# yuz1wan/video_distillation

Hardware: AMD Instinct MI355X
Metric: distillation steps/sec (DM, miniUCF101 IPC=1) (higher is better)
Workload: dtype f16

## Files before the change

### include/vd_hip.h

```cpp
#ifndef VD_HIP_H
#define VD_HIP_H

#include <stdint.h>

#ifdef __cplusplus
extern "C" {
#endif

#define VD_ABI_VERSION 5

#define VD_PREC_BF16   0
#define VD_PREC_F16    1
#define VD_PREC_BF16X3 2
#define VD_PREC_F16X3  3
#define VD_F16X3_WSHIFT 8
#define VD_PREC_F16C8  4

#define VD_EPI_POOL_CL   0
#define VD_EPI_POOL_FEAT 1
#define VD_EPI_ROWS      2
#define VD_EPI_POS_FEAT  3

typedef struct VdConvParams {
    const void* src;
    int64_t src_plane_stride4;
    int64_t src_clip_stride4;
    int64_t src_chunk_stride4;
    const void* wpk;
    int64_t w_plane_stride;
    int64_t w_box_stride;
    const float* bias;
    void* dst;
    int64_t dst_plane_stride;
    uint8_t* argmax;
    const int32_t* col_off;
    const float* out_scale;
    const int32_t* type_desc;
    const int32_t* tables;
    const int32_t* boxes;
    const int32_t* gather;
    int64_t gather_stride;
    const void* zero_slot;
    int32_t nbox, nclips, ncl;
    int32_t CC, S, NT, MW, MTW;
    int32_t epi, pool_t, relu, n_out, n_stride;
    int64_t out_clip_stride;
    int32_t out_chunk_stride, out_t_stride;
    int32_t lds_plane_bytes;
    int32_t prec;
    int32_t dbg;
    int32_t ntypes;
    int32_t tab_ofs[3];
    int32_t atomic;
    int32_t select;
    int32_t src_split_cc;
    int64_t src_split_off4;
    int32_t NTW;
    const int64_t* clip_index;
    int32_t mt_valid;
    int32_t persist;
    uint64_t* stamps;
    int32_t w_set_clips;
    int32_t replica_stride;
    int32_t emit_lo;
    int32_t src_planes, src_rows;
    int32_t pair_flip;
    uint32_t* range_stats;
} VdConvParams;

int vd_abi_version(void);

int vd_conv_mfma(const VdConvParams* params, void* stream);
int vd_conv_mfma_multi(const VdConvParams* const* params, int n, void* stream);

int vd_conv0_breg(const VdConvParams* p, void* stream);

int vd_pack_weights(const float* w, const int32_t* widx, int64_t n, void* out_hi, void* out_lo,
                    int prec, void* stream);

#define VD_PACK_MAX 24
typedef struct {
    const float* w; const int32_t* widx; int64_t n; void* out_hi; void* out_lo; int32_t prec; int32_t first_block;
} VdPackSeg;
typedef struct { int32_t nseg; int32_t reserved; VdPackSeg seg[VD_PACK_MAX]; } VdPackBatch;
int vd_pack_weights_multi(const VdPackBatch* batch, void* stream);
int vd_pack_weights_c8(const float* w, int64_t w_elems, const int32_t* widx, int CC, int S, int NT, void* out_hi, void* out_c8,
                       float* scales6, void* stream);
int vd_pack_weights_dither(const float* w, const int32_t* widx, int64_t n, int groups, void* out, int prec, void* stream);

int vd_round_operand(const float* w, int64_t n, int prec, float* out, void* stream);

int vd_pix2rows(const float* x, const int64_t* clip_index, int64_t nclips, int T, int H, int W,
                void* out_hi, void* out_lo, int prec, void* stream);

int vd_unpool_relu_bwd(const float* g, const uint8_t* argmax, int64_t nclips, int C, int To, int Ho, int Wo,
                       int pool_t, int T, int OH, int OW, int g_layout, void* out_hi, void* out_lo,
                       int prec, const float* scale, void* stream);

int vd_absmax_scale(const float* g, int64_t n, float target, float* out, void* stream);

int vd_dm_loss(const float* feat_real, const float* feat_syn, int nclass, int nreal, int nsyn, int dim,
               float* loss_per_class, float* g_syn, void* stream);

int vd_group_sum(const float* x, int groups, int per, int dim, float scale, float* out, void* stream);

int vd_sgd_momentum(float* x, float* buf, const float* g, int64_t n, float lr, float momentum, int first,
                    void* stream);

int vd_hallucinator_fwd(const float* stat, const float* dyn, const int64_t* sidx, const int64_t* didx,
                        const float* w, const float* b, int n, int T, int H, int W, float* out, void* stream);

int vd_hallucinator_bwd(const float* g_out, const float* stat, const float* dyn, const int64_t* sidx,
                        const int64_t* didx, const float* w, int n, int T, int H, int W,
                        float* g_dyn, float* g_stat, float* g_w, float* g_b, void* stream);

int vd_match_rows_fwd(const float* gr, const float* gs, int64_t rows, int len, float* acc, void* stream);
int vd_match_rows_bwd(const float* gr, const float* gs, int64_t rows, int len, int mode, const float* acc,
                      const float* gout, float* g_gs, void* stream);

#define VD_MATCH_MAX_SEG 16
typedef struct VdMatchSeg {
    const float* gr;
    const float* gs;
    float* g;
    int64_t rows;
    int32_t len;
    int32_t reserved;
} VdMatchSeg;
typedef struct VdMatchBatch {
    int32_t nseg;
    int32_t reserved;
    VdMatchSeg seg[VD_MATCH_MAX_SEG];
} VdMatchBatch;
int vd_match_rows_fwd_multi(const VdMatchBatch* batch, float* acc, void* stream);
int vd_match_rows_bwd_multi(const VdMatchBatch* batch, int mode, const float* acc, const float* gout, void* stream);

int vd_clip_minor_cl(const void* src, int64_t src_plane_slots, int planes, int64_t nclips, int C, int64_t npos,
                     void* dst, int64_t dst_plane_slots, void* stream);
int vd_clip_minor_pix(const float* x, int64_t nclips, int T, int H, int W, void* dst_hi, void* dst_lo, int prec,
                      void* stream);
int vd_pack_dy(const void* dy, int64_t dy_plane_slots, int planes, int64_t nclips, int N, int T, int OH, int OW,
               int nt, int noh, int now, void* dst, int64_t dst_plane_elems, void* stream);
int vd_unpool_relu_bwd_packed(const float* g, const uint8_t* argmax, int64_t nclips, int C, int To, int Ho, int Wo,
                              int pool_t, int T, int OH, int OW, int g_layout, int nt, int noh, int now,
                              void* dst_hi, void* dst_lo, int prec, const float* scale, void* stream);

int vd_bias_grad_pooled(const float* g, const uint8_t* argmax, int64_t nclips, int C, int64_t npos, int g_layout, float* db,
                        void* stream);
int64_t vd_bias_grad_pooled_scratch_floats(int64_t nclips, int C, int64_t npos);
int vd_bias_grad_pooled_ordered(const float* g, const uint8_t* argmax, int64_t nclips, int C, int64_t npos, int g_layout,
                                float* scratch, float* db, void* stream);
int vd_bias_grad(const void* dy, int64_t dy_plane_slots, int planes, int64_t nclips, int N, int64_t npos, int prec,
                 const float* scale_inv, float* db, void* stream);

int vd_head_fwd(const float* feats, const float* w, const float* b, int64_t nclips, int C, int To, int Ho, int Wo,
                int kt, int kh, int kw, int K, float* out, void* stream);

int vd_standardize(const float* x, int64_t n, double* scratch2, float* out, void* stream);
int vd_head_train_fwd(const float* feats, const float* mask, const float* w, const float* b, int64_t nclips, int C, int To,
                      int Ho, int Wo, int kt, int kh, int kw, int K, float* dropped, float* logits, int32_t* amax_t, void* stream);
int vd_ce_loss(const float* logits, const int64_t* labels, int B, int K, float* loss_per_clip, float* dlogits, void* stream);
int vd_head_train_bwd(const float* dlogits, const int32_t* amax_t, const float* dropped, const float* mask, const float* w,
                      int64_t nclips, int C, int To, int Ho, int Wo, int kt, int kh, int kw, int K, float* g_w, float* g_b,
                      float* g_feats, void* stream);
int vd_standardize_ordered(const float* x, int64_t n, double* scratch, float* out, void* stream);
int vd_head_train_bwd_ordered(const float* dlogits, const int32_t* amax_t, const float* dropped, const float* mask, const float* w,
                              int64_t nclips, int C, int To, int Ho, int Wo, int kt, int kh, int kw, int K, float* g_w, float* g_b,
                              float* g_feats, void* stream);
int vd_set_deterministic(int on);
int vd_get_deterministic(void);
int vd_resplit_slots(const void* src_hi, const void* src_lo, int64_t n_elems, int src_prec, void* dst_hi, void* dst_lo,
                     int dst_prec, void* stream);
int vd_split_scaled(const float* src, int64_t n_elems, const float* scale, void* dst_hi, void* dst_lo, int prec, void* stream);
int vd_scale_combine(const float* a, const float* b, int mode, float* out, void* stream);
const char* vd_sources_hash(void);

int vd_head_second_order(const float* logits, const float* dlogits, const int32_t* amax_t, const float* dropped,
                         const float* mask, const float* w, const float* v_w, const float* v_b, const float* gbar_feats,
                         int64_t nclips, int C, int To, int Ho, int Wo, int kt, int kh, int kw, int K, float* abar_feats,
                         float* wbar, float* bbar, float* dlogbar_out, void* stream);
int vd_program_build(int layer, int frames, int height, int width, int prec, int batch_hint, void** blob, int64_t* nbytes);
int vd_program_build_dgrad(int layer, int parity_class, int frames, int height, int width, int batch_hint, void** blob,
                           int64_t* nbytes);
int vd_program_build_wgrad(int layer, int frames, int height, int width, int nclips, int planes, void** blob, int64_t* nbytes,
                           int* block3, int* replicas);
void vd_blob_free(void* blob);

typedef struct VdEmbed VdEmbed;
int vd_embed_create(int frames, int height, int width, int prec, int batch_hint, VdEmbed** out);
int vd_embed_create_ex(int frames, int height, int width, int prec, int prec_bwd, int batch_hint, VdEmbed** out);
int64_t vd_embed_argmax_bytes(const VdEmbed* e, int64_t nclips);
int64_t vd_embed_backward_workspace_bytes(const VdEmbed* e, int64_t nclips);
int vd_embed_forward_keep(VdEmbed* e, const float* clips, const int64_t* clip_index, int64_t nclips, void* workspace,
                          int64_t workspace_bytes, float* features, uint8_t* argmax, void* stream);
int vd_embed_backward(VdEmbed* e, const float* g_features, const uint8_t* argmax, int64_t nclips, void* workspace,
                      int64_t workspace_bytes, float* g_clips, void* stream);
int64_t vd_embed_num_features(const VdEmbed* e);
int64_t vd_embed_workspace_bytes(const VdEmbed* e, int64_t nclips);
int vd_embed_set_weights(VdEmbed* e, const float* w0, const float* b0, const float* w1, const float* b1, const float* w2,
                         const float* b2, void* stream);
int vd_embed_forward(VdEmbed* e, const float* clips, const int64_t* clip_index, int64_t nclips, void* workspace,
                     int64_t workspace_bytes, float* features, void* stream);
void vd_embed_free(VdEmbed* e);

int vd_mfma_peak(int blocks, int iters, int shape, float* out, void* stream);
int vd_sgd_momentum_wd(float* x, float* buf, const float* g, int64_t n, float lr, float momentum, float wd, int first,
                       void* stream);

int vd_replica_sum(float* rep, int replicas, int rows, int cols, float* out, void* stream);

int vd_frames_normalize(const void* src_u8, float* dst, int64_t nframes, int height, int width, const float* mean3,
                        const float* std3, void* stream);

int vd_clips_sample(const void* frames_u8, int64_t store_frames, int src_h, int src_w, const int64_t* frame_row,
                    const int32_t* crop_yx, const uint8_t* flip, int64_t nclips, int T, int out_h, int out_w, float* dst,
                    const float* mean3, const float* std3, void* stream);

typedef struct VdProgram VdProgram;
int vd_program_load(const void* blob, int64_t nbytes, int prec, VdProgram** out);
int vd_program_pack_weights(VdProgram* prog, const float* w, void* stream);
int vd_program_run(VdProgram* prog, const void* src, int64_t src_plane_slots, const float* bias, void* dst,
                   int64_t dst_plane_stride, uint8_t* argmax, const int64_t* clip_index, int nclips, void* stream);
int vd_program_run_scaled(VdProgram* prog, const void* src, int64_t src_plane_slots, const float* bias, void* dst,
                          int64_t dst_plane_stride, uint8_t* argmax, const int64_t* clip_index, int nclips,
                          const float* out_scale, void* stream);
int vd_program_run_wgrad(VdProgram* prog, const void* x_clip_minor, int64_t x_plane_slots, const void* packed_dy,
                         int64_t packed_plane_elems, float* copies, int64_t copy_elems, int cin, const float* out_scale,
                         void* stream);
int64_t vd_program_info(const VdProgram* prog, int what);
void vd_program_free(VdProgram* prog);

typedef struct VdTrain VdTrain;
int vd_train_create(int frames, int height, int width, int num_classes, int prec, int prec_bwd, int64_t nclips, VdTrain** out);
int64_t vd_train_workspace_bytes(const VdTrain* t);
int vd_train_step(VdTrain* t, float* const* params, float* const* momentum, const float* clips, const int64_t* labels,
                  const float* dropout_mask, float lr, float momentum_coef, float weight_decay, int first, void* workspace,
                  int64_t workspace_bytes, float* loss_per_clip, float* logits, void* stream);
void vd_train_free(VdTrain* t);

typedef struct VdComm VdComm;
typedef struct { char internal[128]; } VdCommId;
int vd_comm_unique_id(VdCommId* id);
int vd_comm_create(const VdCommId* id, int nranks, int rank, VdComm** out);
int vd_comm_size(const VdComm* c);
int vd_comm_version(int* version);
int vd_comm_rank(const VdComm* c);
int vd_comm_allreduce_f32(VdComm* c, const float* send, float* recv, int64_t n, void* stream);
int vd_comm_allgather_f32(VdComm* c, const float* send, float* recv, int64_t n_per_rank, void* stream);
void vd_comm_free(VdComm* c);

#define VD_CORESET_HERDING   0
#define VD_CORESET_KCENTER   1
#define VD_CORESET_MAX_COUNT 4096
#define VD_CORESET_MAX_DIM   8192
int64_t vd_coreset_workspace_bytes(int nclass, int max_count);
int vd_coreset_select(const float* feats, int dim, const int64_t* offsets, const int32_t* counts, int nclass, int max_count,
                      int ipc, int method, int64_t* out_idx, void* workspace, int64_t workspace_bytes, void* stream);

#ifdef __cplusplus
}
// ... 3 lines not shown
```

### video_distillation_amd/csrc/aux_kernels.hip

```cpp
#include <hip/hip_runtime.h>
#include <stdint.h>
#include <stdlib.h>

#include "../../include/vd_hip.h"
#include "frame_norm.h"

typedef __bf16 bf16_t;

__device__ __forceinline__ void split16p(int prec, float v, uint16_t& hi, uint16_t& lo) {
    if (prec == VD_PREC_BF16 || prec == VD_PREC_BF16X3) {
        __bf16 h = (__bf16)v;
        __bf16 l = (__bf16)(v - (float)h);
        hi = __builtin_bit_cast(uint16_t, h);
        lo = __builtin_bit_cast(uint16_t, l);
    } else {
        _Float16 h = (_Float16)v;
        _Float16 l = (_Float16)(v - (float)h);
        hi = __builtin_bit_cast(uint16_t, h);
        lo = __builtin_bit_cast(uint16_t, l);
    }
}

__device__ __forceinline__ float wave_sum(float v) {
#pragma unroll
// ... 358 lines not shown
                           reinterpret_cast<hipStream_t>(stream), g, argmax, nwin, C, To, Ho, Wo, pool_t, T, OH, OW,
                           (uint4*)out_hi, (uint4*)out_lo, prec, scale);
        return (int)hipGetLastError();
    }
    hipLaunchKernelGGL(unpool_relu_bwd_kernel, dim3((unsigned)((nslots + bs - 1) / bs)), dim3(bs), 0,
                       reinterpret_cast<hipStream_t>(stream), g, argmax, nslots, C, To, Ho, Wo, pool_t, T, OH, OW,
                       g_layout, (uint4*)out_hi, (uint4*)out_lo, prec, scale);
    return (int)hipGetLastError();
}

__global__ void absmax_kernel(const float* __restrict__ g, int64_t n, unsigned int* __restrict__ bits) {
    __shared__ float red[16];
    float m = 0.f;
    for (int64_t i = (int64_t)blockIdx.x * blockDim.x + threadIdx.x; i < n; i += (int64_t)gridDim.x * blockDim.x)
        m = fmaxf(m, fabsf(g[i]));
#pragma unroll
    for (int o = 32; o > 0; o >>= 1) m = fmaxf(m, __shfl_xor(m, o, 64));
    const int lane = threadIdx.x & 63, w = threadIdx.x >> 6;
    if (lane == 0) red[w] = m;
    __syncthreads();
    if (threadIdx.x == 0) {
        for (int i = 1; i < (int)(blockDim.x >> 6); ++i) m = fmaxf(m, red[i]);
        atomicMax(bits, __float_as_uint(m));
    }
}

__device__ __forceinline__ void float_decompose(unsigned int bits, int& e, unsigned int& mant) {
    e = (int)(bits >> 23);
    mant = bits & 0x7fffffu;
    if (e == 0) {
        const int sh = __clz(mant) - 8;
        mant <<= sh;
        e = 1 - sh;
    } else {
        mant |= 0x800000u;
    }
    e -= 127;
}

__global__ void scale_from_absmax_kernel(const unsigned int* __restrict__ bits, float target, float* __restrict__ out) {
    const unsigned int mb = bits[0], tb = __float_as_uint(target);
    int k = 0;
    if (mb != 0u && mb < 0x7f800000u && tb != 0u && tb < 0x7f800000u) {
        int em, et;
        unsigned int mm, mt;
        float_decompose(mb, em, mm);
        float_decompose(tb, et, mt);
        k = et - em - (mt > mm ? 0 : 1);
        k = k < -126 ? -126 : (k > 126 ? 126 : k);
    }
    out[0] = __uint_as_float((unsigned int)(127 + k) << 23);
    out[1] = __uint_as_float((unsigned int)(127 - k) << 23);
}

extern "C" int vd_absmax_scale(const float* g, int64_t n, float target, float* out, void* stream) {
    hipStream_t st = reinterpret_cast<hipStream_t>(stream);
    unsigned int* bits = reinterpret_cast<unsigned int*>(out + 2);
    hipError_t e = hipMemsetAsync(bits, 0, sizeof(unsigned int), st);
    if (e != hipSuccess) return (int)e;
    if (n > 0) {
        int64_t blocks = (n + 256 * 8 - 1) / (256 * 8);
        if (blocks > 1024) blocks = 1024;
        hipLaunchKernelGGL(absmax_kernel, dim3((unsigned)blocks), dim3(256), 0, st, g, n, bits);
    }
    hipLaunchKernelGGL(scale_from_absmax_kernel, dim3(1), dim3(1), 0, st, bits, target, out);
    return (int)hipGetLastError();
}

__global__ __launch_bounds__(1024) void dm_loss_kernel(const float* __restrict__ fr, const float* __restrict__ fs,
                                                        int nreal, int nsyn, int dim, float* __restrict__ loss,
                                                        float* __restrict__ gsyn) {
    __shared__ float red[16];
    const int c = blockIdx.x;
    const float* r = fr + (int64_t)c * nreal * dim;
    const float* s = fs + (int64_t)c * nsyn * dim;
    const float inv_r = 1.f / (float)nreal, inv_s = 1.f / (float)nsyn;
    float part = 0.f;
    for (int d = threadIdx.x; d < dim; d += blockDim.x) {
        float m[8] = {0.f, 0.f, 0.f, 0.f, 0.f, 0.f, 0.f, 0.f};
        int b = 0;
        for (; b + 8 <= nreal; b += 8) {
#pragma unroll
            for (int k = 0; k < 8; ++k) m[k] += r[(int64_t)(b + k) * dim + d];
        }
        for (; b < nreal; ++b) m[0] += r[(int64_t)b * dim + d];
        const float mr = ((m[0] + m[1]) + (m[2] + m[3])) + ((m[4] + m[5]) + (m[6] + m[7]));
        float ms = 0.f;
        for (int k = 0; k < nsyn; ++k) ms += s[(int64_t)k * dim + d];
        const float diff = mr * inv_r - ms * inv_s;
        part += diff * diff;
        if (gsyn != nullptr) {
            const float gv = -2.f * diff * inv_s;
            for (int k = 0; k < nsyn; ++k) gsyn[((int64_t)c * nsyn + k) * dim + d] = gv;
        }
    }
    const float tot = block_sum(part, red);
    if (threadIdx.x == 0) loss[c] = tot;
}

extern "C" int vd_dm_loss(const float* feat_real, const float* feat_syn, int nclass, int nreal, int nsyn, int dim,
                          float* loss_per_class, float* g_syn, void* stream) {
    if (nclass <= 0) return 0;
    if (nreal <= 0 || nsyn <= 0 || dim <= 0) return -2;
    hipLaunchKernelGGL(dm_loss_kernel, dim3(nclass), dim3(1024), 0, reinterpret_cast<hipStream_t>(stream), feat_real,
                       feat_syn, nreal, nsyn, dim, loss_per_class, g_syn);
    return (int)hipGetLastError();
}

__global__ void group_sum_kernel(const float* __restrict__ x, int per, int dim, float scale, float* __restrict__ out) {
    const int g = blockIdx.y;
    const int d = blockIdx.x * blockDim.x + threadIdx.x;
    if (d >= dim) return;
    const float* r = x + (int64_t)g * per * dim + d;
    float m[4] = {0.f, 0.f, 0.f, 0.f};
    int b = 0;
    for (; b + 4 <= per; b += 4) {
#pragma unroll
        for (int k = 0; k < 4; ++k) m[k] += r[(int64_t)(b + k) * dim];
    }
    for (; b < per; ++b) m[0] += r[(int64_t)b * dim];
    out[(int64_t)g * dim + d] = ((m[0] + m[1]) + (m[2] + m[3])) * scale;
}

extern "C" int vd_group_sum(const float* x, int groups, int per, int dim, float scale, float* out, void* stream) {
    if (groups <= 0 || dim <= 0) return 0;
    if (per <= 0) return -2;
    hipLaunchKernelGGL(group_sum_kernel, dim3((dim + 255) / 256, groups), dim3(256), 0,
                       reinterpret_cast<hipStream_t>(stream), x, per, dim, scale, out);
    return (int)hipGetLastError();
}

__global__ void sgd_momentum_kernel(float* __restrict__ x, float* __restrict__ buf, const float* __restrict__ g,
                                    int64_t n, float lr, float mu, int first) {
    const int64_t stride = (int64_t)gridDim.x * blockDim.x;
    for (int64_t i = (int64_t)blockIdx.x * blockDim.x + threadIdx.x; i < n; i += stride) {
#pragma clang fp contract(off)
        const float gv = g[i];
        const float prev = buf[i] * mu;
        const float b = first ? gv : prev + gv;
        buf[i] = b;
        const float step = lr * b;
        x[i] = x[i] - step;
    }
}

extern "C" int vd_sgd_momentum(float* x, float* buf, const float* g, int64_t n, float lr, float momentum, int first,
                               void* stream) {
    if (n <= 0) return 0;
    const int bs = 256;
    int64_t blocks = (n + bs - 1) / bs;
    if (blocks > 8192) blocks = 8192;
    hipLaunchKernelGGL(sgd_momentum_kernel, dim3((unsigned)blocks), dim3(bs), 0, reinterpret_cast<hipStream_t>(stream),
                       x, buf, g, n, lr, momentum, first);
    return (int)hipGetLastError();
}

#define HAL_W(co, ci, kt, kh, kw) w[(((co) * 4 + (ci)) * 3 + (kt)) * 9 + (kh) * 3 + (kw)]

__global__ __launch_bounds__(256) void hal_fwd_kernel(const float* __restrict__ stat, const float* __restrict__ dyn,
                                                       const int64_t* __restrict__ sidx, const int64_t* __restrict__ didx,
                                                       const float* __restrict__ w, const float* __restrict__ b,
                                                       int n, int T, int H, int W, float* __restrict__ out) {
    const int64_t total = (int64_t)n * H * W;
    const int64_t i = (int64_t)blockIdx.x * blockDim.x + threadIdx.x;
    if (i >= total) return;
    const int x = (int)(i % W);
    const int y = (int)((i / W) % H);
    const int64_t clip = i / ((int64_t)W * H);
    const int64_t si = sidx ? sidx[clip] : clip, di = didx ? didx[clip] : clip;
    const float* sp = stat + si * 3 * H * W;
    const float* dp = dyn + di * (int64_t)T * H * W;
    bool ok[9];
    int off[9];
#pragma unroll
    for (int a = 0; a < 3; ++a)
#pragma unroll
        for (int c = 0; c < 3; ++c) {
            const int yy = y + a - 1, xx = x + c - 1;
            ok[a * 3 + c] = yy >= 0 && yy < H && xx >= 0 && xx < W;
            off[a * 3 + c] = yy * W + xx;
        }
    float S[3][3];
#pragma unroll
    for (int kt = 0; kt < 3; ++kt)
#pragma unroll
        for (int co = 0; co < 3; ++co) S[kt][co] = 0.f;
#pragma unroll
    for (int ci = 0; ci < 3; ++ci)
#pragma unroll
        for (int k = 0; k < 9; ++k) {
            const float v = ok[k] ? sp[(int64_t)ci * H * W + off[k]] : 0.f;
#pragma unroll
            for (int kt = 0; kt < 3; ++kt)
#pragma unroll
                for (int co = 0; co < 3; ++co) S[kt][co] += HAL_W(co, ci, kt, k / 3, k % 3) * v;
        }
    const float b0 = b[0], b1 = b[1], b2 = b[2];
    float d[3][9];
#pragma unroll
    for (int k = 0; k < 9; ++k) { d[0][k] = 0.f; d[1][k] = ok[k] ? dp[off[k]] : 0.f; }
    const int64_t HW = (int64_t)H * W;
    for (int t = 0; t < T; ++t) {
        const bool nxt = t + 1 < T;
#pragma unroll
        for (int k = 0; k < 9; ++k) d[2][k] = (nxt && ok[k]) ? dp[(int64_t)(t + 1) * HW + off[k]] : 0.f;
        float a0 = b0 + S[1][0], a1 = b1 + S[1][1], a2 = b2 + S[1][2];
        if (t > 0) { a0 += S[0][0]; a1 += S[0][1]; a2 += S[0][2]; }
        if (nxt) { a0 += S[2][0]; a1 += S[2][1]; a2 += S[2][2]; }
#pragma unroll
        for (int kt = 0; kt < 3; ++kt)
#pragma unroll
            for (int k = 0; k < 9; ++k) {
                const float v = d[kt][k];
                a0 += HAL_W(0, 3, kt, k / 3, k % 3) * v;
                a1 += HAL_W(1, 3, kt, k / 3, k % 3) * v;
                a2 += HAL_W(2, 3, kt, k / 3, k % 3) * v;
            }
        float* op = out + ((clip * T + t) * 3) * HW + (int64_t)y * W + x;
        op[0] = a0;
        op[HW] = a1;
        op[2 * HW] = a2;
#pragma unroll
        for (int k = 0; k < 9; ++k) { d[0][k] = d[1][k]; d[1][k] = d[2][k]; }
    }
}

extern "C" int vd_hallucinator_fwd(const float* stat, const float* dyn, const int64_t* sidx, const int64_t* didx,
                                   const float* w, const float* b, int n, int T, int H, int W, float* out, void* stream) {
    const int64_t total = (int64_t)n * H * W;
    if (total <= 0 || T <= 0) return 0;
    hipLaunchKernelGGL(hal_fwd_kernel, dim3((unsigned)((total + 255) / 256)), dim3(256), 0,
                       reinterpret_cast<hipStream_t>(stream), stat, dyn, sidx, didx, w, b, n, T, H, W, out);
    return (int)hipGetLastError();
}

__global__ __launch_bounds__(256) void hal_bwd_data_kernel(const float* __restrict__ go, const int64_t* __restrict__ sidx,
                                                            const int64_t* __restrict__ didx, const float* __restrict__ w,
                                                            int n, int T, int H, int W, float* __restrict__ g_dyn,
                                                            float* __restrict__ g_stat) {
    const int64_t total = (int64_t)n * H * W;
    const int64_t i = (int64_t)blockIdx.x * blockDim.x + threadIdx.x;
    if (i >= total) return;
    const int x = (int)(i % W);
    const int y = (int)((i / W) % H);
    const int64_t clip = i / ((int64_t)W * H);
    const int64_t HW = (int64_t)H * W;
    bool ok[9];
    int off[9];
#pragma unroll
    for (int a = 0; a < 3; ++a)
#pragma unroll
        for (int c = 0; c < 3; ++c) {
            const int yy = y + a - 1, xx = x + c - 1;
            ok[a * 3 + c] = yy >= 0 && yy < H && xx >= 0 && xx < W;
            off[a * 3 + c] = yy * W + xx;
        }
    const float* gp = go + clip * (int64_t)T * 3 * HW;
    float nb[3][3][9], sum[3][9], first[3][9];
#pragma unroll
    for (int co = 0; co < 3; ++co)
#pragma unroll
        for (int k = 0; k < 9; ++k) {
            nb[0][co][k] = 0.f;
            const float v = ok[k] ? gp[(int64_t)co * HW + off[k]] : 0.f;
            nb[1][co][k] = v; first[co][k] = v; sum[co][k] = 0.f;
        }
    const int64_t di = didx ? didx[clip] : clip;
    float* gd = g_dyn + di * (int64_t)T * HW + (int64_t)y * W + x;
    for (int t = 0; t < T; ++t) {
        const bool nxt = t + 1 < T;
#pragma unroll
        for (int co = 0; co < 3; ++co)
#pragma unroll
            for (int k = 0; k < 9; ++k) {
                nb[2][co][k] = (nxt && ok[k]) ? gp[((int64_t)(t + 1) * 3 + co) * HW + off[k]] : 0.f;
                sum[co][k] += nb[1][co][k];
            }
        float acc = 0.f;
#pragma unroll
        for (int f = 0; f < 3; ++f)
#pragma unroll
            for (int co = 0; co < 3; ++co)
#pragma unroll
                for (int k = 0; k < 9; ++k) acc += nb[f][co][k] * HAL_W(co, 3, 2 - f, 2 - k / 3, 2 - k % 3);
        atomicAdd(gd + (int64_t)t * HW, acc);
        if (nxt) {
#pragma unroll
            for (int co = 0; co < 3; ++co)
#pragma unroll
                for (int k = 0; k < 9; ++k) { nb[0][co][k] = nb[1][co][k]; nb[1][co][k] = nb[2][co][k]; }
        }
    }
    if (g_stat != nullptr) {
        const int64_t si = sidx ? sidx[clip] : clip;
#pragma unroll
        for (int ci = 0; ci < 3; ++ci) {
            float acc = 0.f;
#pragma unroll
            for (int co = 0; co < 3; ++co)
#pragma unroll
                for (int k = 0; k < 9; ++k) {
                    const int kh = 2 - k / 3, kw = 2 - k % 3;
                    const float sm = sum[co][k];
                    acc += HAL_W(co, ci, 1, kh, kw) * sm + HAL_W(co, ci, 0, kh, kw) * (sm - first[co][k]) +
                           HAL_W(co, ci, 2, kh, kw) * (sm - nb[1][co][k]);
                }
// ... 1672 lines not shown
```

### video_distillation_amd/csrc/conv_mfma.hip

```cpp
#include <hip/hip_runtime.h>
#include <mutex>
#include <stdint.h>
#include <stdlib.h>
#include <string.h>
#include <type_traits>
#include <utility>

#include "../../include/vd_hip.h"

#ifndef VD_DB_X1
#define VD_DB_X1 3
#endif
#ifdef VD_NO_SCHED_BARRIER
#define VD_SCHED_BARRIER()
#else
#define VD_SCHED_BARRIER() __builtin_amdgcn_sched_barrier(0)
#endif
#ifndef VD_NO_SETPRIO_LOOP
#define VD_PRIO_LOOP(x) __builtin_amdgcn_s_setprio(x)
#else
#define VD_PRIO_LOOP(x)
#endif
#ifdef VD_SETPRIO
#define VD_PRIO(x) __builtin_amdgcn_s_setprio(x)
// ... 12 lines not shown
#define VD_C8_SA_LO (127 - VD_C8_ALO_SHIFT)
#define VD_C8_SA_HI (127 + 2)
__device__ __forceinline__ uint32_t vd_c8_hi_byte(uint16_t h16) {
    const _Float16 h = __builtin_bit_cast(_Float16, h16);
    const f16x2 hh = {h, h};
    i16x2 r = {0, 0};
    r = __builtin_amdgcn_cvt_scalef32_pk_fp8_f16(r, hh, 4.0f, false);
    return (uint32_t)__builtin_bit_cast(int, r) & 0xffu;
}
__device__ __forceinline__ void vd_c8_image(const uint4& a, int& w0, int& w1, const float div) {
    i16x2 r0, r1;
#pragma clang diagnostic push
#pragma clang diagnostic ignored "-Wuninitialized"
    r0 = __builtin_amdgcn_cvt_scalef32_pk_fp8_f16(r0, __builtin_bit_cast(f16x2, a.x), div, false);
    r0 = __builtin_amdgcn_cvt_scalef32_pk_fp8_f16(r0, __builtin_bit_cast(f16x2, a.y), div, true);
    r1 = __builtin_amdgcn_cvt_scalef32_pk_fp8_f16(r1, __builtin_bit_cast(f16x2, a.z), div, false);
    r1 = __builtin_amdgcn_cvt_scalef32_pk_fp8_f16(r1, __builtin_bit_cast(f16x2, a.w), div, true);
#pragma clang diagnostic pop
    w0 = __builtin_bit_cast(int, r0); w1 = __builtin_bit_cast(int, r1);
}
__device__ __forceinline__ uint32_t vd_c8_lo_byte(float v) {
    float r = (v - (float)(_Float16)v) * (float)(1 << VD_C8_ALO_SHIFT);
    r = fminf(fmaxf(r, -448.f), 448.f);
    return (uint32_t)__builtin_amdgcn_cvt_pk_fp8_f32(r, r, 0, false) & 0xffu;
}

struct VdDevCache {
    std::mutex mu;
    bool done[64] = {};
    int ncu[64] = {};
};
static int vd_dev_prepare(const void* kern, VdDevCache& c, int& ncu) {
    int dev = 0;
    hipError_t e = hipGetDevice(&dev);
    if (e != hipSuccess) return (int)e;
    if (dev < 0 || dev >= 64) return -4;
    std::lock_guard<std::mutex> lk(c.mu);
    if (!c.done[dev]) {
        e = hipDeviceGetAttribute(&c.ncu[dev], hipDeviceAttributeMultiprocessorCount, dev);
        if (e != hipSuccess || c.ncu[dev] <= 0) return e != hipSuccess ? (int)e : -4;
        e = hipFuncSetAttribute(kern, hipFuncAttributeMaxDynamicSharedMemorySize, 160 * 1024);
        if (e != hipSuccess) return (int)e;
        c.done[dev] = true;
    }
    ncu = c.ncu[dev];
    return 0;
}

template <int PREC>
__device__ __forceinline__ f32x16 mfma16(const uint4& a, const uint4& b, f32x16 c) {
    if constexpr (PREC == VD_PREC_BF16 || PREC == VD_PREC_BF16X3) {
        return __builtin_amdgcn_mfma_f32_32x32x16_bf16(__builtin_bit_cast(bf16x8, a), __builtin_bit_cast(bf16x8, b), c, 0, 0, 0);
    } else {
        return __builtin_amdgcn_mfma_f32_32x32x16_f16(__builtin_bit_cast(f16x8, a), __builtin_bit_cast(f16x8, b), c, 0, 0, 0);
    }
}

typedef uint32_t u32x4 __attribute__((ext_vector_type(4)));
template <int PREC>
__device__ __forceinline__ f32x16 mfma16(const uint4& a, const u32x4& b, f32x16 c) {
    if constexpr (PREC == VD_PREC_BF16 || PREC == VD_PREC_BF16X3) {
        return __builtin_amdgcn_mfma_f32_32x32x16_bf16(__builtin_bit_cast(bf16x8, a), __builtin_bit_cast(bf16x8, b), c, 0, 0, 0);
    } else {
        return __builtin_amdgcn_mfma_f32_32x32x16_f16(__builtin_bit_cast(f16x8, a), __builtin_bit_cast(f16x8, b), c, 0, 0, 0);
    }
}

template <int PREC>
__device__ __forceinline__ void split16(float v, uint16_t& hi, uint16_t& lo) {
    if constexpr (PREC == VD_PREC_BF16 || PREC == VD_PREC_BF16X3) {
        __bf16 h = (__bf16)v;
        __bf16 l = (__bf16)(v - (float)h);
        hi = __builtin_bit_cast(uint16_t, h);
        lo = __builtin_bit_cast(uint16_t, l);
    } else {
        _Float16 h = (_Float16)v;
        _Float16 l = (_Float16)(v - (float)h);
        hi = __builtin_bit_cast(uint16_t, h);
        lo = __builtin_bit_cast(uint16_t, l);
    }
}

#ifndef VD_DBG_HOOKS
#define VD_DBG_HOOKS 0
#endif
#if VD_DBG_HOOKS
#define VD_DBG(p) ((p).dbg)
#else
#define VD_DBG(p) 0
#endif
#ifndef VD_OCC_SMALL
#define VD_OCC_SMALL 2
#endif
#define VD_OCC(PREC, MTW, NTW, BAL) \
    ((((MTW) * (NTW) + (BAL)) <= 4 && ((PREC) == VD_PREC_BF16 || (PREC) == VD_PREC_F16)) ? VD_OCC_SMALL : 2)
template <int I> struct VdIC { static constexpr int v = I; };
template <class F, int... Is>
__device__ __forceinline__ void vd_static_for_impl(F&& f, std::integer_sequence<int, Is...>) { (f(VdIC<Is>{}), ...); }
template <int N, class F>
__device__ __forceinline__ void vd_static_for(F&& f) { vd_static_for_impl(f, std::make_integer_sequence<int, N>{}); }

template <int PREC, int MTW, bool SO = false, int NTW = 1, int BAL = 0, bool SQ = false>
__device__ __forceinline__ void conv_mfma_body(const VdConvParams& p, const int boxes_per_wg, const int total_boxes, const int block_id, const int nblocks) {
    constexpr bool C8 = (PREC == VD_PREC_F16C8);
    constexpr bool X3 = (PREC == VD_PREC_BF16X3 || PREC == VD_PREC_F16X3 || C8);
    static_assert(!C8 || (MTW == 4 && NTW == 1 && BAL == 0 && !SO && !SQ), "VD_PREC_F16C8: the last level's 4 x 1-tile layout only");
    constexpr bool EXT = SO || MTW == 5;
    constexpr bool SEQ = X3 && SQ;
    constexpr int LPL = (X3 && !SEQ) ? 2 : 1;
    constexpr bool ALT = X3 && !C8;
    constexpr int TILES = MTW * NTW + BAL;
    constexpr int MA = MTW + BAL;
    static_assert(BAL == 0 || (NTW == 2 && !X3 && !SO), "balanced layout: single-pass formats, two N tiles per wave");
    constexpr int H0 = (MTW + 1) / 2;
    constexpr int H1 = MTW - H0;
    constexpr int AD = 1;
    constexpr int DB = C8 ? 3 : X3 ? (TILES <= 2 ? 5 : ((SEQ && NTW == 1) ? 3 : 2)) : VD_DB_X1;
    static_assert(X3 || (DB + 1) % (AD + 1) == 0, "ring sizes must divide the unroll factor");
    constexpr int LU = C8 ? 6 : (TILES <= 4) ? 14 : 17;
    extern __shared__ __attribute__((aligned(16))) char smem[];

    const int tid = threadIdx.x;
    const int nthreads = blockDim.x;
    const int lane = tid & 63;
    const int wave = __builtin_amdgcn_readfirstlane(tid >> 6);
    const int ncols = p.NT / NTW;
    const int wn = wave % ncols;
    const int wm = wave / ncols;
    bool short_row = false;
    if constexpr (NTW == 2) short_row = p.mt_valid > 0 && (wm + 1) * MTW > p.mt_valid;
    const int half = lane >> 5;

    int wgid;
    {
        const int nwg = nblocks, q = nwg >> 3, r = nwg & 7;
        const int xcd = block_id & 7, k = block_id >> 3;
        wgid = (xcd < r ? xcd * (q + 1) : r * (q + 1) + (xcd - r) * q) + k;
    }
    unsigned long long t_stamp[8];
    auto stamp = [&](int k) { if (VD_DBG(p) & 8) { unsigned long long t; asm volatile("s_memtime %0\n\ts_waitcnt lgkmcnt(0)" : "=s"(t) :: "memory"); t_stamp[k] = t; } };
    auto finish = [&]() {
        if ((VD_DBG(p) & 8) && tid == 0 && p.stamps != nullptr) {
            stamp(7);
            unsigned long long* o = reinterpret_cast<unsigned long long*>(p.stamps) + (size_t)block_id * 8;
            for (int k = 0; k < 8; ++k) o[k] = t_stamp[k];
        }
    };
    const int ngroups = (int)(p.gather_stride >> 6);
    const int nwaves = nthreads >> 6;
    const int plane_bytes = p.lds_plane_bytes;
    int* lds_tap = reinterpret_cast<int*>(smem + LPL * plane_bytes);
    int* lds_otab = lds_tap + 2 * p.S;
    int* lds_skip = lds_otab + (p.MW * MTW + BAL) * 4;
    const bool one_type = (p.ntypes == 1);
    const uint32_t* zslot = reinterpret_cast<const uint32_t*>(p.zero_slot);
    const uint32_t* src = reinterpret_cast<const uint32_t*>(p.src);
    const uint4* wbase = reinterpret_cast<const uint4*>(p.wpk);
    const int64_t w_lo = p.w_plane_stride >> 3;
    const int wstep = p.NT * 64;
    const int S = p.S;
    int a_off[MA];
    const int mt_tot = p.MW * MTW + BAL;
    auto tile_of = [&](int i) { return (BAL && i == MTW) ? p.MW * MTW : wm * MTW + i; };
    if (one_type) {
        const int32_t* a_tab0 = p.tables + p.tab_ofs[0];
        const int32_t* o_tab0 = p.tables + p.tab_ofs[1];
        const int32_t* t_tab0 = p.tables + p.tab_ofs[2];
        for (int k = tid; k < 2 * p.S; k += nthreads) lds_tap[k] = t_tab0[k];
        if constexpr (C8)
            for (int k = tid; k < (p.S >> 2); k += nthreads) lds_skip[k] = t_tab0[2 * p.S + k];
        if (p.epi != VD_EPI_ROWS)
            for (int k = tid; k < mt_tot * 4; k += nthreads) lds_otab[k] = o_tab0[k];
#pragma unroll
        for (int i = 0; i < MA; ++i) a_off[i] = a_tab0[tile_of(i) * 32 + (lane & 31)];
    }

  constexpr bool LOOPED = (TILES <= 4);
  const int nbit = LOOPED ? boxes_per_wg : 1;
  for (int bit = 0; bit < nbit; ++bit) {
    const int bid = wgid * nbit + bit;
    if (bid >= total_boxes) break;
    stamp(0);
    int grp = bid / p.nbox;
    int bi = bid - grp * p.nbox;
    if constexpr (EXT) {
        if (p.w_box_stride != 0) {
            const int ngrp = total_boxes / p.nbox;
            bi = bid / ngrp;
            grp = bid - bi * ngrp;
        }
    }
    if constexpr (C8) {
        if (p.persist & 0x80000) {
            const int ngrp = total_boxes / p.nbox;
            bi = bid / ngrp;
            grp = bid - bi * ngrp;
        }
    }
    const int clip0 = grp * p.ncl;

    const int32_t* gtab = p.gather + (int64_t)bi * p.gather_stride;
    constexpr bool HOIST = (TILES < 8);
#ifndef VD_C8_HOIST
#define VD_C8_HOIST 1
#endif
    const bool hoist = HOIST && (!C8 || (VD_C8_HOIST && ngroups <= nwaves * LU));
    uint32_t goff[HOIST ? LU : 1];
#pragma unroll
    for (int u = 0; u < (HOIST ? LU : 1); ++u) {
        const int gi = wave + u * nwaves;
        const int e = gtab[((gi < ngroups) ? gi : ngroups - 1) * 64 + lane];
        const int ci = e >> 24;
        const bool ok = (e >= 0) && (clip0 + ci < p.nclips);
        goff[u] = ok ? ((uint32_t)ci * (uint32_t)p.src_clip_stride4 + (uint32_t)(e & 0xFFFFFF)) : 0xFFFFFFFFu;
    }
    const int32_t* box = p.boxes + bi * 8;
    const int32_t* o_tab = p.tables + (one_type ? p.tab_ofs[1] : box[1]);
    const int out_rel = box[3];
    if (!one_type) {
        const int32_t* a_tab = p.tables + box[0];
        const int32_t* t_tab = p.tables + box[2];
        __syncthreads();
        for (int k = tid; k < 2 * p.S; k += nthreads) lds_tap[k] = t_tab[k];
        if constexpr (C8)
            for (int k = tid; k < (p.S >> 2); k += nthreads) lds_skip[k] = t_tab[2 * p.S + k];
        if (p.epi != VD_EPI_ROWS)
            for (int k = tid; k < mt_tot * 4; k += nthreads) lds_otab[k] = o_tab[k];
#pragma unroll
        for (int i = 0; i < MA; ++i) a_off[i] = a_tab[tile_of(i) * 32 + (lane & 31)];
    }
#pragma unroll
    for (int u = 0; u < (HOIST ? LU : 1); ++u) asm volatile("" : "+v"(goff[u]));

    f32x16 acc[TILES];
#pragma unroll
    for (int i = 0; i < TILES; ++i)
#pragma unroll
        for (int k = 0; k < 16; ++k) acc[i][k] = 0.f;

    for (int cc = 0; cc < p.CC; ++cc) {
      vd_static_for<SEQ ? 2 : 1>([&](auto PHC) __attribute__((always_inline)) {
        constexpr int ph = decltype(PHC)::v;
        __syncthreads();
        const bool alt_on = ALT && !(p.persist & 0x100000);
        if constexpr (ALT) {
            if (alt_on && ph == 0 && cc > 0) {
#pragma unroll
                for (int i = 0; i < TILES; ++i)
#pragma unroll
                    for (int k = 0; k < 16; ++k) acc[i][k] = -acc[i][k];
            }
        }
        const uint32_t bsgn = (alt_on && (cc & 1)) ? 0x80008000u : 0u;
        const int64_t wset = (!X3 && !EXT && p.w_set_clips > 0) ? (int64_t)(clip0 / p.w_set_clips) * w_lo : (int64_t)0;
        const uint4* wp = wbase + wset + ((EXT || C8) ? (((int64_t)bi * p.w_box_stride) >> 3) : (int64_t)0) + ((int64_t)cc * S * p.NT + wn * NTW) * 64 + lane;
        auto load_b = [&](int s, uint4* bh, uint4* bl) {
            const int sc = (VD_DBG(p) & 16) ? 0 : ((s < S) ? s : S - 1);
#pragma unroll
            for (int j = 0; j < NTW; ++j) {
                bh[j] = wp[(int64_t)sc * wstep + j * 64];
                if constexpr (X3 && !C8 && (!SEQ || ph == 0)) bl[j] = wp[(int64_t)sc * wstep + j * 64 + w_lo];
            }
        };
        uint4 bqh[DB + 1][NTW], bql[DB + 1][NTW];
#pragma unroll
        for (int u = 0; u <= DB; ++u)
#pragma unroll
            for (int j = 0; j < NTW; ++j) bql[u][j] = make_uint4(0, 0, 0, 0);
#pragma unroll
        for (int u = 0; u < DB; ++u) load_b(u, bqh[u], bql[u]);
        const uint32_t* csrc = src + (int64_t)clip0 * p.src_clip_stride4 + (int64_t)cc * p.src_chunk_stride4;
        if constexpr (TILES <= 4) {
            if (p.clip_index != nullptr) csrc = src + p.clip_index[clip0] * (int64_t)p.src_clip_stride4;
        }
        if constexpr (SO) {
            if (p.src_split_cc > 0 && cc >= p.src_split_cc)
                csrc = src + (int64_t)clip0 * p.src_clip_stride4 + p.src_split_off4 +
                       (int64_t)(cc - p.src_split_cc) * p.src_chunk_stride4;
        }
        if (cc == 0 && ph == 0) stamp(1);
        if (hoist && !(VD_DBG(p) & 4)) {
            int gi = wave;
#pragma unroll
            for (int u = 0; u < LU; ++u) {
                asm volatile("" : "+s"(gi));
                if (gi < ngroups) {
                    const bool ok = goff[HOIST ? u : 0] != 0xFFFFFFFFu;
                    const uint32_t* gp = ok ? csrc + goff[HOIST ? u : 0] + (ph ? p.src_plane_stride4 : (int64_t)0) : zslot;
                    char* dst = smem + gi * 1024;
                    __builtin_amdgcn_global_load_lds((const __attribute__((address_space(1))) void*)gp,
                                                     (__attribute__((address_space(3))) void*)dst, 16, 0, 0);
                    if constexpr (X3 && !SEQ) {
                        const uint32_t* gl = ok ? csrc + goff[HOIST ? u : 0] + p.src_plane_stride4 : zslot;
                        __builtin_amdgcn_global_load_lds((const __attribute__((address_space(1))) void*)gl,
                                                         (__attribute__((address_space(3))) void*)(dst + plane_bytes), 16, 0, 0);
                    }
                }
                gi += nwaves;
            }
        }
        if (!hoist && !(VD_DBG(p) & 4)) {
            constexpr int LB = 8;
            for (int g0 = wave; g0 < ngroups; g0 += nwaves * LB) {
                uint32_t off[LB];
#pragma unroll
                for (int u = 0; u < LB; ++u) {
                    const int gi = g0 + u * nwaves;
                    const int e = gtab[((gi < ngroups) ? gi : ngroups - 1) * 64 + lane];
                    const int ci = e >> 24;
                    const bool ok = (e >= 0) && (clip0 + ci < p.nclips);
                    off[u] = ok ? ((uint32_t)ci * (uint32_t)p.src_clip_stride4 + (uint32_t)(e & 0xFFFFFF)) : 0xFFFFFFFFu;
                }
#pragma unroll
                for (int u = 0; u < LB; ++u) asm volatile("" : "+v"(off[u]));
                int gi = g0;
#pragma unroll
                for (int u = 0; u < LB; ++u) {
                    asm volatile("" : "+s"(gi));
                    if (gi < ngroups) {
                        const bool ok = off[u] != 0xFFFFFFFFu;
                        const uint32_t* gp = ok ? csrc + off[u] + (ph ? p.src_plane_stride4 : (int64_t)0) : zslot;
                        char* dst = smem + gi * 1024;
                        __builtin_amdgcn_global_load_lds((const __attribute__((address_space(1))) void*)gp,
                                                         (__attribute__((address_space(3))) void*)dst, 16, 0, 0);
                        if constexpr (X3 && !SEQ) {
                            const uint32_t* gl = ok ? csrc + off[u] + p.src_plane_stride4 : zslot;
                            __builtin_amdgcn_global_load_lds((const __attribute__((address_space(1))) void*)gl,
                                                             (__attribute__((address_space(3))) void*)(dst + plane_bytes), 16, 0, 0);
                        }
                    }
                    gi += nwaves;
                }
            }
        }
        if (cc == 0 && ph == 0) stamp(2);
        __syncthreads();
        if (cc == 0 && ph == 0) stamp(3);
        if (VD_DBG(p) & 2) return;
        if constexpr (!X3) {
            auto tap_of = [&](int st) {
                const int sc = (VD_DBG(p) & 32) ? 0 : ((st < S) ? st : S - 1);
                return lds_tap[2 * sc + half];
            };
            static_assert(AD == 1, "the refill scheme below is written for two register sets");
            uint4 A[AD + 1][MA];
#pragma unroll
            for (int d = 0; d <= AD; ++d) {
                const int tp = tap_of(d);
#pragma unroll
                for (int i = 0; i < MA; ++i) A[d][i] = *reinterpret_cast<const uint4*>(smem + a_off[i] + tp);
            }
            int tp = tap_of(AD + 1);
            VD_PRIO_LOOP(2);
            auto k_step = [&](const int u, const int s_abs) {
                load_b(s_abs + DB, bqh[(u + DB) % (DB + 1)], bql[(u + DB) % (DB + 1)]);
                const int tp_next = tap_of(s_abs + AD + 2);
                VD_SCHED_BARRIER();
                VD_PRIO(1);
#pragma unroll
                for (int i = 0; i < MTW; ++i) {
                    if (NTW == 2 && BAL == 0 && i == MTW - 1 && short_row) continue;
#pragma unroll
                    for (int j = 0; j < NTW; ++j)
                        acc[j * MTW + i] = mfma16<PREC>(A[u % (AD + 1)][i], bqh[u][j], acc[j * MTW + i]);
                    VD_SCHED_BARRIER();
                    if (i > 0 && (VD_DBG(p) & 64)) A[u % (AD + 1)][i] = A[u % (AD + 1)][0];
                    else A[u % (AD + 1)][i] = *reinterpret_cast<const uint4*>(smem + a_off[i] + tp);
                    VD_SCHED_BARRIER();
                }
                if constexpr (BAL) {
                    uint4 bx = bqh[u][0];
                    if (wm) bx = bqh[u][1];
                    acc[MTW * NTW] = mfma16<PREC>(A[u % (AD + 1)][MTW], bx, acc[MTW * NTW]);
                    VD_SCHED_BARRIER();
                    A[u % (AD + 1)][MTW] = *reinterpret_cast<const uint4*>(smem + a_off[MTW] + tp);
                }
                VD_PRIO(0);
                VD_SCHED_BARRIER();
                tp = tp_next;
            };
            int s = 0;
            for (; s + DB < S; s += DB + 1) {
#pragma unroll
                for (int u = 0; u <= DB; ++u) k_step(u, s + u);
            }
            if (s < S) {
#pragma unroll
                for (int u = 0; u <= DB; ++u) {
                    if (s + u >= S) break;
                    k_step(u, s + u);
                }
            }
            VD_PRIO_LOOP(0);
        } else if constexpr (C8) {
            const int* sc8 = reinterpret_cast<const int*>(p.out_scale);
            const int sb_hi = sc8[0], sb_lo = sc8[1];
            auto skip_of = [&](int st) { return __builtin_amdgcn_readfirstlane(lds_skip[((st < S) ? st : S - 4) >> 2]); };
            const int* tapv = lds_tap + half;
            auto taps_of = [&](int st, int* t4) {
                const int sc = (st < S) ? st : S - 4;
#pragma unroll
                for (int q = 0; q < 4; ++q) t4[q] = tapv[2 * (sc + q)];
            };
            auto rdA = [&](int i, int tap) { return *reinterpret_cast<const uint4*>(smem + a_off[i] + tap); };
            const uint4* wq = wp;
            auto piece = [&](int st) { return wq[(int64_t)st * wstep + w_lo]; };
            int skip = skip_of(0);
            int tq[4];
            taps_of(0, tq);
            uint4 Ah[MTW];
#pragma unroll
            for (int i = 0; i < MTW; ++i) {
                Ah[i] = make_uint4(0, 0, 0, 0);
                if (!((skip >> i) & 1)) Ah[i] = rdA(i, tq[0]);
            }
            const float w_div = p.out_scale[3];
            uint4 b8_2, b8_3;
            i32x8 B8hi;
            auto img_b = [&](auto UC) __attribute__((always_inline)) {
                constexpr int u = decltype(UC)::v;
                int w0, w1;
                vd_c8_image(bqh[u][0], w0, w1, w_div);
                B8hi[2 * u] = w0; B8hi[2 * u + 1] = w1;
            };
            i32x8 a8lo[2], a8hi[2];
            auto corr_lo = [&](auto IC, auto RC) __attribute__((always_inline)) {
// ... 112 lines not shown
                    corr_lo(VdIC<T1>{}, VdIC<1>{});
                    corr_hi(VdIC<0>{}, VdIC<0>{}, B8lo);
                    corr_hi(VdIC<T1>{}, VdIC<1>{}, B8lo);
                } else if constexpr (P1) {
                    rd_planes(VdIC<0>{}, VdIC<0>{}, VdIC<0>{});
                    prefetch_next();
                    __builtin_amdgcn_sched_barrier(0);
                    corr_lo(VdIC<0>{}, VdIC<0>{});
                    corr_hi(VdIC<0>{}, VdIC<0>{}, B8lo);
                } else {
                    vd_static_for<MTW>([&](auto IC) __attribute__((always_inline)) {
                        constexpr int i = decltype(IC)::v;
                        if (!((skip >> i) & 1)) {
                            rd_planes(IC, VdIC<i & 1>{}, VdIC<i & 1>{});
                            corr_lo(IC, VdIC<i & 1>{});
                            corr_hi(IC, VdIC<i & 1>{}, B8lo);
                        }
                    });
                    prefetch_next();
                }
                __builtin_amdgcn_sched_barrier(0);
            };
            int s = 0;
            auto run = [&](auto MC) __attribute__((always_inline)) {
                constexpr int MK = decltype(MC)::v;
                const int skip_n = skip_of(s + 4);
                const int tqn0 = tapv[2 * ((s + 4 < S) ? s + 4 : S - 4)];
                if (MK >= 0 || skip != 0xF) group(MC, skip_n, tqn0);
                else {
#pragma unroll
                    for (int u = 0; u < 4; ++u) bqh[(u + DB) % (DB + 1)][0] = wq[(int64_t)(u + DB) * wstep];
#pragma unroll
                    for (int i = 0; i < MTW; ++i)
                        if (!((skip_n >> i) & 1)) Ah[i] = rdA(i, tqn0);
                }
                wq += (int64_t)4 * wstep;
                skip = skip_n;
                s += 4;
                taps_of(s, tq);
            };
            while (s < S) {
                while (s < S && skip == 0) run(VdIC<0>{});
                while (s < S && skip == 0xA) run(VdIC<0xA>{});
                while (s < S && skip == 0xC) run(VdIC<0xC>{});
                while (s < S && skip == 0xE) run(VdIC<0xE>{});
                if (s < S && skip != 0 && skip != 0xA && skip != 0xC && skip != 0xE) run(VdIC<-1>{});
            }
        } else if constexpr (SEQ) {
            {
                constexpr int PH = ph;
                int tap_next = lds_tap[2 * ((1 < S) ? 1 : 0) + half];
                uint4 Ax[MTW];
                {
                    const int tap0 = lds_tap[half];
#pragma unroll
                    for (int i = 0; i < MTW; ++i) Ax[i] = *reinterpret_cast<const uint4*>(smem + a_off[i] + tap0);
                }
                for (int s = 0; s < S; s += DB + 1) {
#pragma unroll
                    for (int u = 0; u <= DB; ++u) {
                        if (s + u >= S) break;
                        load_b(s + u + DB, bqh[(u + DB) % (DB + 1)], bql[(u + DB) % (DB + 1)]);
                        uint4 bh[NTW], bl[NTW];
#pragma unroll
                        for (int j = 0; j < NTW; ++j) {
                            bh[j] = bqh[u][j]; bl[j] = bql[u][j];
                            bh[j].x ^= bsgn; bh[j].y ^= bsgn; bh[j].z ^= bsgn; bh[j].w ^= bsgn;
                            if constexpr (PH == 0) { bl[j].x ^= bsgn; bl[j].y ^= bsgn; bl[j].z ^= bsgn; bl[j].w ^= bsgn; }
                        }
                        const int sn2 = (s + u + 2 < S) ? s + u + 2 : S - 1;
                        const int tap_next2 = lds_tap[2 * sn2 + half];
                        __builtin_amdgcn_sched_barrier(0);
#pragma unroll
                        for (int i = 0; i < MTW; ++i) {
                            if (NTW == 2 && BAL == 0 && i == MTW - 1 && short_row) continue;
#pragma unroll
                            for (int j = 0; j < NTW; ++j) {
                                if constexpr (PH == 0) {
                                    acc[j * MTW + i] = mfma16<PREC>(Ax[i], bl[j], acc[j * MTW + i]);
                                    acc[j * MTW + i] = mfma16<PREC>(Ax[i], bh[j], acc[j * MTW + i]);
                                } else {
                                    acc[j * MTW + i] = mfma16<PREC>(Ax[i], bh[j], acc[j * MTW + i]);
                                }
                            }
                            __builtin_amdgcn_sched_barrier(0);
                            Ax[i] = *reinterpret_cast<const uint4*>(smem + a_off[i] + tap_next);
                            __builtin_amdgcn_sched_barrier(0);
                        }
                        tap_next = tap_next2;
                    }
                }
            }
        } else {
            int tap_next = lds_tap[2 * ((1 < S) ? 1 : 0) + half];
            uint4 Ah[MTW], Al[MTW];
            {
                const int tap0 = lds_tap[half];
#pragma unroll
                for (int i = 0; i < MTW; ++i) {
                    Ah[i] = *reinterpret_cast<const uint4*>(smem + a_off[i] + tap0);
                    Al[i] = *reinterpret_cast<const uint4*>(smem + plane_bytes + a_off[i] + tap0);
                }
            }
            for (int s = 0; s < S; s += DB + 1) {
#pragma unroll
                for (int u = 0; u <= DB; ++u) {
                    if (s + u >= S) break;
                    load_b(s + u + DB, bqh[(u + DB) % (DB + 1)], bql[(u + DB) % (DB + 1)]);
                    uint4 bh[NTW], bl[NTW];
#pragma unroll
                    for (int j = 0; j < NTW; ++j) {
                        bh[j] = bqh[u][j]; bl[j] = bql[u][j];
                        bh[j].x ^= bsgn; bh[j].y ^= bsgn; bh[j].z ^= bsgn; bh[j].w ^= bsgn;
                        bl[j].x ^= bsgn; bl[j].y ^= bsgn; bl[j].z ^= bsgn; bl[j].w ^= bsgn;
                    }
                    const int sn2 = (s + u + 2 < S) ? s + u + 2 : S - 1;
                    const int tap_next2 = lds_tap[2 * sn2 + half];
                    __builtin_amdgcn_sched_barrier(0);
#pragma unroll
                    for (int i = 0; i < MTW; ++i) {
                        if (NTW == 2 && BAL == 0 && i == MTW - 1 && short_row) continue;
#pragma unroll
                        for (int j = 0; j < NTW; ++j) {
                            acc[j * MTW + i] = mfma16<PREC>(Al[i], bh[j], acc[j * MTW + i]);
                            acc[j * MTW + i] = mfma16<PREC>(Ah[i], bl[j], acc[j * MTW + i]);
                            acc[j * MTW + i] = mfma16<PREC>(Ah[i], bh[j], acc[j * MTW + i]);
                        }
                        __builtin_amdgcn_sched_barrier(0);
                        Ah[i] = *reinterpret_cast<const uint4*>(smem + a_off[i] + tap_next);
                        Al[i] = *reinterpret_cast<const uint4*>(smem + plane_bytes + a_off[i] + tap_next);
                        __builtin_amdgcn_sched_barrier(0);
                    }
                    tap_next = tap_next2;
                }
            }
        }
      });
    }

    if constexpr (ALT) {
        if (!(p.persist & 0x100000) && !(p.CC & 1)) {
#pragma unroll
            for (int i = 0; i < TILES; ++i)
#pragma unroll
                for (int k = 0; k < 16; ++k) acc[i][k] = -acc[i][k];
        }
    }
    stamp(4);
    if (VD_DBG(p) & 1) { if (acc[0][0] == 123.456f) reinterpret_cast<float*>(p.dst)[0] = 1.f; continue; }
    const int64_t out_total = (int64_t)p.nclips * p.out_clip_stride;
    const int64_t out_base = (int64_t)clip0 * p.out_clip_stride + out_rel;
    const float asc = (PREC == VD_PREC_F16X3 && p.w_box_stride == 0) ? 1.f / (float)(1 << VD_F16X3_WSHIFT) : 1.f;

    if (p.epi == VD_EPI_ROWS) {
        float* dst = reinterpret_cast<float*>(p.dst);
        if constexpr (EXT) { if (p.atomic) dst += (int64_t)box[5] * p.replica_stride; }
        const float osc = ((p.out_scale != nullptr) ? p.out_scale[0] : 1.f) * asc;
#pragma unroll
      for (int j = 0; j < NTW + BAL; ++j) {
        const bool ex = BAL && j == NTW;
        const int n = (wn * NTW + (ex ? wm : j)) * 32 + (lane & 31);
        const bool n_ok = n < p.n_out;
        const float bias = (p.bias != nullptr && n_ok) ? p.bias[n] : 0.f;
        const int64_t coff = (p.col_off != nullptr) ? (int64_t)p.col_off[n & 31] : (int64_t)n * p.n_stride;
#pragma unroll
        for (int i = 0; i < MTW; ++i) {
            if (ex && i > 0) continue;
            const int gi = ex ? p.MW * MTW : wm * MTW + i;
            const f32x16& at = acc[ex ? MTW * NTW : j * MTW + i];
#pragma unroll
            for (int k = 0; k < 16; ++k) {
                const int row = (k & 3) + 8 * (k >> 2) + 4 * half;
                const int o = o_tab[gi * 32 + row];
                const int64_t idx = out_base + o;
                float v = at[k] * osc + bias;
                if (p.relu) v = fmaxf(v, 0.f);
                if (o >= 0 && n_ok && idx < out_total) {
                    if (EXT && p.atomic) atomicAdd(&dst[idx + coff], v);
                    else dst[idx + coff] = v;
                }
            }
        }
      }
        finish();
        continue;
    }

    if constexpr (C8) {
        if (p.epi == VD_EPI_POS_FEAT) {
            float* dstf = reinterpret_cast<float*>(p.dst);
            const int n = wn * 32 + (lane & 31);
            const bool n_ok = n < p.n_out;
            const float bias = (p.bias != nullptr && n_ok) ? p.bias[n] : 0.f;
#pragma unroll
            for (int k = 0; k < 16; k += 2) {
                float m = fmaxf(acc[0][k], acc[0][k + 1]);
#pragma unroll
                for (int i = 1; i < MTW; ++i) m = fmaxf(m, fmaxf(acc[i][k], acc[i][k + 1]));
                m += bias;
                if (p.relu) m = fmaxf(m, 0.f);
                const int row = (k & 3) + 8 * (k >> 2) + 4 * half;
                const int o = lds_otab[row >> 1];
                const int64_t idx = out_base + o + (int64_t)n * p.n_stride;
                if (o >= 0 && n_ok && idx < out_total) dstf[idx] = m;
            }
            finish();
            continue;
        }
    }

    const int64_t lim64 = out_total - out_base;
    const int lim = (int)(lim64 > 0x7fffffff ? 0x7fffffff : (lim64 < 0 ? 0 : lim64));
    const bool feat = (p.epi == VD_EPI_POOL_FEAT);
    float* dstf = reinterpret_cast<float*>(p.dst) + out_base;
    uint16_t* dst16 = reinterpret_cast<uint16_t*>(p.dst) + out_base * 8;
    uint8_t* amx = p.argmax ? p.argmax + (feat ? out_base : out_base * 8) : nullptr;
    const int nsets = (p.pool_t == 2) ? 1 : 2;
    const bool staged = !feat && amx == nullptr;
    const bool lo_out = X3 || (!EXT && p.emit_lo != 0);
    const int NCH = p.NT * 32;
    const int Q = mt_tot * 4 * nsets;
    uint16_t* stg = reinterpret_cast<uint16_t*>(smem);
    if (staged) __syncthreads();
    stamp(5);
    float rs_amax = 0.f;
    int rs_sat = 0;
#pragma unroll
  for (int j = 0; j < NTW + BAL; ++j) {
    const bool ex = BAL && j == NTW;
    const int n = (wn * NTW + (ex ? wm : j)) * 32 + (lane & 31);
    const bool n_ok = n < p.n_out;
    const float bias = (p.bias != nullptr && n_ok) ? p.bias[n] : 0.f;
    const uint32_t chan = feat ? (uint32_t)n * (uint32_t)p.n_stride
                               : (uint32_t)(n >> 3) * (uint32_t)p.out_chunk_stride * 8u + (uint32_t)(n & 7);
#pragma unroll
    for (int i = 0; i < MTW; ++i) {
        if (ex && i > 0) continue;
        const int gi = ex ? p.MW * MTW : wm * MTW + i;
        const f32x16& at = acc[ex ? MTW * NTW : j * MTW + i];
#pragma unroll
        for (int qh = 0; qh < 2; ++qh) {
            const int r0 = 8 * qh;
            if (staged) {
                float m0 = fmaxf(fmaxf(at[r0], at[r0 + 1]), fmaxf(at[r0 + 2], at[r0 + 3]));
                float m1 = fmaxf(fmaxf(at[r0 + 4], at[r0 + 5]), fmaxf(at[r0 + 6], at[r0 + 7]));
                if (p.pool_t == 2) m0 = fmaxf(m0, m1);
                if constexpr (PREC == VD_PREC_F16X3) { m0 *= asc; m1 *= asc; }
                m0 += bias; m1 += bias;
                if (p.relu) { m0 = fmaxf(m0, 0.f); m1 = fmaxf(m1, 0.f); }
                if (!X3 && !EXT && p.emit_lo == 2) {
                    const float a0 = fabsf(m0), a1 = (p.pool_t == 2) ? 0.f : fabsf(m1);
                    rs_amax = fmaxf(rs_amax, fmaxf(a0, a1));
                    rs_sat += (!(a0 <= 1792.f) ? 1 : 0) + (!(a1 <= 1792.f) ? 1 : 0);
                    m0 = fminf(fmaxf(m0, -1792.f), 1792.f); m1 = fminf(fmaxf(m1, -1792.f), 1792.f);
                }
                const int q = (gi * 4 + half + 2 * qh) * nsets;
                uint16_t hi, lo;
                split16<PREC>(m0, hi, lo);
                stg[q * NCH + n] = hi;
                const bool lo8 = !X3 && !EXT && p.emit_lo == 2;
                uint8_t* stg8 = reinterpret_cast<uint8_t*>(stg);
                const int b8 = (n >> 3) * 16 + (n & 7);
                if (lo8) { stg8[(Q + q) * NCH * 2 + b8] = (uint8_t)vd_c8_lo_byte(m0); stg8[(Q + q) * NCH * 2 + b8 + 8] = (uint8_t)vd_c8_hi_byte(hi); }
                else if (lo_out) stg[(Q + q) * NCH + n] = lo;
                if (p.pool_t != 2) {
                    split16<PREC>(m1, hi, lo);
                    stg[(q + 1) * NCH + n] = hi;
                    if (lo8) { stg8[(Q + q + 1) * NCH * 2 + b8] = (uint8_t)vd_c8_lo_byte(m1); stg8[(Q + q + 1) * NCH * 2 + b8 + 8] = (uint8_t)vd_c8_hi_byte(hi); }
                    else if (lo_out) stg[(Q + q + 1) * NCH + n] = lo;
                }
                continue;
            }
            const int o = lds_otab[gi * 4 + half + 2 * qh];
            if (o < 0 || !n_ok) continue;
            if (SO && p.select) {
                const float osc_sel = ((p.out_scale != nullptr) ? p.out_scale[0] : 1.f) * asc;
#pragma unroll
                for (int st = 0; st < 2; ++st) {
                    if (st == 1 && p.pool_t == 2) continue;
                    const int base = o + st * (((p.pair_flip >> (half + 2 * qh)) & 1) ? -p.out_t_stride : p.out_t_stride);
                    if (base >= lim) continue;
                    const uint32_t idx = feat ? (uint32_t)base + chan : (uint32_t)base * 8u + chan;
                    const int ab = amx[idx];
                    const int jsel = (p.pool_t == 2) ? (ab & 7) : (4 * st + (ab & 3));
                    float v = 0.f;
#pragma unroll
                    for (int j = 0; j < 8; ++j) v = (j == jsel) ? at[r0 + j] : v;
                    v = (ab & 0x80) ? 0.f : v * osc_sel + bias;
                    if (feat) {
                        dstf[idx] = v;
                    } else if (p.select == 2) {
                        reinterpret_cast<float*>(p.dst)[out_base * 8 + idx] = v;
                    } else {
                        uint16_t hi, lo;
                        split16<PREC>(v, hi, lo);
                        dst16[idx] = hi;
                        if constexpr (X3) dst16[idx + p.dst_plane_stride * 8] = lo;
                    }
                }
                continue;
            }
            float mv[2]; int av[2];
#pragma unroll
            for (int st = 0; st < 2; ++st) {
                float mx = at[r0 + 4 * st];
                int am = 0;
#pragma unroll
                for (int j = 1; j < 4; ++j) {
                    const float v = at[r0 + 4 * st + j];
                    if (v > mx) { mx = v; am = j; }
                }
                mv[st] = mx; av[st] = am;
            }
            if (p.pool_t == 2 && mv[1] > mv[0]) { mv[0] = mv[1]; av[0] = 4 + av[1]; }
#pragma unroll
            for (int st = 0; st < 2; ++st) {
                if (st == 1 && p.pool_t == 2) continue;
                float mx = mv[st];
                if constexpr (PREC == VD_PREC_F16X3) mx *= asc;
                mx += bias;
                if (p.relu) mx = fmaxf(mx, 0.f);
                const int base = o + st * (((p.pair_flip >> (half + 2 * qh)) & 1) ? -p.out_t_stride : p.out_t_stride);
                if (base >= lim) continue;
                const uint8_t ab = (uint8_t)(av[st] | (mx > 0.f ? 0 : 0x80));
                if (feat) {
                    const uint32_t idx = (uint32_t)base + chan;
                    dstf[idx] = mx;
                    if (amx) amx[idx] = ab;
                } else {
                    const uint32_t idx = (uint32_t)base * 8u + chan;
                    uint16_t hi, lo;
                    split16<PREC>(mx, hi, lo);
                    dst16[idx] = hi;
                    if constexpr (X3) dst16[idx + p.dst_plane_stride * 8] = lo;
                    if (amx) amx[idx] = ab;
                }
            }
        }
    }
  }
    if constexpr (!X3 && !EXT) {
        if (staged && p.emit_lo == 2 && p.range_stats != nullptr) {
#pragma unroll
            for (int o = 32; o > 0; o >>= 1) {
                rs_amax = fmaxf(rs_amax, __shfl_xor(rs_amax, o));
                rs_sat += __shfl_xor(rs_sat, o);
            }
            if (lane == 0) {
                const uint32_t bits = __float_as_uint(rs_amax);
                if (bits > __builtin_nontemporal_load(p.range_stats + 1)) atomicMax(p.range_stats + 1, bits);
                if (rs_sat) atomicAdd(p.range_stats, (uint32_t)rs_sat);
            }
        }
    }
    if (staged) {
        __syncthreads();
        stamp(6);
        const int cpq_sh = __builtin_ctz(NCH >> 3);
        const int ns_sh = nsets - 1;
        uint4* dslots = reinterpret_cast<uint4*>(p.dst) + out_base;
        for (int item = tid; item < ((Q << cpq_sh)); item += nthreads) {
            const int q = item >> cpq_sh, cc = item & ((1 << cpq_sh) - 1);
            const int g = q >> ns_sh, st = q & ns_sh;
            const int o = lds_otab[g];
            const int base = o + st * (((p.pair_flip >> (g & 3)) & 1) ? -p.out_t_stride : p.out_t_stride);
            if (o < 0 || base >= lim) continue;
            const uint32_t slot = (uint32_t)base + (uint32_t)cc * (uint32_t)p.out_chunk_stride;
            dslots[slot] = *reinterpret_cast<const uint4*>(stg + q * NCH + cc * 8);
            if (lo_out) dslots[slot + p.dst_plane_stride] = *reinterpret_cast<const uint4*>(stg + (Q + q) * NCH + cc * 8);
        }
    }
    finish();
  }
}

template <int PREC, int MTW, bool SO = false, int NTW = 1, int BAL = 0, bool SQ = false>
__global__ __launch_bounds__(256, VD_OCC(PREC, MTW, NTW, BAL)) void conv_mfma_kernel(const VdConvParams p, const int boxes_per_wg, const int total_boxes) {
    conv_mfma_body<PREC, MTW, SO, NTW, BAL, SQ>(p, boxes_per_wg, total_boxes, (int)blockIdx.x, (int)gridDim.x);
}

#define VD_MULTI_MAX 4
struct VdConvMulti {
    VdConvParams p[VD_MULTI_MAX];
    int first[VD_MULTI_MAX + 1];
    int total[VD_MULTI_MAX];
};
template <int PREC, int MTW, bool SO = false, int NTW = 1, int BAL = 0>
__global__ __launch_bounds__(256, VD_OCC(PREC, MTW, NTW, BAL)) void conv_mfma_multi_kernel(const VdConvMulti m) {
    const int b = (int)blockIdx.x;
    int k = 0;
#pragma unroll
    for (int i = 1; i < VD_MULTI_MAX; ++i) k += (b >= m.first[i]) ? 1 : 0;
    conv_mfma_body<PREC, MTW, SO, NTW, BAL>(m.p[k], 1, m.total[k], b - m.first[k], m.first[k + 1] - m.first[k]);
}

#ifndef VD_L0_D
#define VD_L0_D 6
#endif
#ifndef VD_L0_PRIO
#define VD_L0_PRIO 1
#endif
#ifndef VD_L0_TOUCH
#define VD_L0_TOUCH 0
#endif
#define VD_LDS_BARRIER() asm volatile("s_waitcnt lgkmcnt(0)\n\ts_barrier" ::: "memory")

template <int PREC, bool FS>
__global__ __launch_bounds__(512, 1) void conv0_breg_kernel(const VdConvParams p, const int boxes_per_wg) {
    constexpr int MTW = 4, S = 32, NI = 3;
    constexpr int PH = 9, PF = 189;
    extern __shared__ __attribute__((aligned(16))) char smem[];
    const int tid = threadIdx.x;
    const int lane = tid & 63;
    const int wave = __builtin_amdgcn_readfirstlane(tid >> 6);
    const int grp = wave >> 2, tg = tid & 255;
    const int wn = wave & 1, wm = (wave >> 1) & 1;
    const int half = lane >> 5;
    const int32_t* a_tab = p.tables + p.tab_ofs[0];
    const int32_t* o_tab = p.tables + p.tab_ofs[1];
    const int32_t* t_tab = p.tables + p.tab_ofs[2];
    const int plane_bytes = p.lds_plane_bytes;
    const uint32_t* src = reinterpret_cast<const uint32_t*>(p.src);
    char* patch = smem + grp * plane_bytes;
    int* lds_tap = reinterpret_cast<int*>(smem + 2 * plane_bytes);
    uint16_t* stg16 = reinterpret_cast<uint16_t*>(smem + 2 * plane_bytes + 512 + wave * 2048);
    for (int k = tid; k < 2 * S; k += 512) lds_tap[k] = t_tab[k];
    int a_off[FS ? 1 : MTW];
#pragma unroll
    for (int i = 0; i < (FS ? 1 : MTW); ++i) a_off[i] = a_tab[(wm * MTW + i) * 32 + (lane & 31)];
    int o_reg[2];
#pragma unroll
    for (int k = 0; k < 2; ++k) {
        const int ql = (lane + 64 * k) >> 2, g = ql >> 1;
        const int o = o_tab[wm * 16 + g];
        const int step = ((p.pair_flip >> (g & 3)) & 1) ? -p.out_t_stride : p.out_t_stride;
        o_reg[k] = o < 0 ? -1 : o + (ql & 1) * step;
    }
    const int ph = p.type_desc[1], pitch_h = FS ? PH : p.type_desc[3], pitch_f = FS ? PF : p.type_desc[4], nitems = 2 * p.type_desc[0] * ph;
    const int ph_magic = (65536 + ph - 1) / ph;
    const int row4 = (int)(p.src_chunk_stride4 / ((int64_t)p.src_planes * p.src_rows));
    u32x4 breg[S];
    auto load_breg = [&](int set) {
        const char* wbase = reinterpret_cast<const char*>(reinterpret_cast<const uint4*>(p.wpk) + (int64_t)set * (p.w_plane_stride >> 3) + (int64_t)wn * 64);
        uint32_t voff = (uint32_t)lane * 16u;
#define VD_L0_LD(k) "global_load_dwordx4 %" #k ", %16, %17\n\tv_add_u32 %16, 0x800, %16\n\t"
#define VD_L0_LD16 VD_L0_LD(0) VD_L0_LD(1) VD_L0_LD(2) VD_L0_LD(3) VD_L0_LD(4) VD_L0_LD(5) VD_L0_LD(6) VD_L0_LD(7) \
                   VD_L0_LD(8) VD_L0_LD(9) VD_L0_LD(10) VD_L0_LD(11) VD_L0_LD(12) VD_L0_LD(13) VD_L0_LD(14) VD_L0_LD(15)
#pragma unroll
        for (int h = 0; h < 2; ++h) {
            u32x4* b = breg + 16 * h;
            asm volatile(VD_L0_LD16 "s_waitcnt vmcnt(0)"
                         : "=&v"(b[0]), "=&v"(b[1]), "=&v"(b[2]), "=&v"(b[3]), "=&v"(b[4]), "=&v"(b[5]), "=&v"(b[6]), "=&v"(b[7]),
                           "=&v"(b[8]), "=&v"(b[9]), "=&v"(b[10]), "=&v"(b[11]), "=&v"(b[12]), "=&v"(b[13]), "=&v"(b[14]), "=&v"(b[15]),
                           "+v"(voff)
                         : "s"(wbase)
                         : "memory");
        }
#undef VD_L0_LD16
#undef VD_L0_LD
        __builtin_amdgcn_sched_barrier(0);
    };
    int cur_set = -1;
    const int n = wn * 32 + (lane & 31);
    const float bias = (p.bias != nullptr) ? p.bias[n] : 0.f;
    const int64_t out_total = (int64_t)p.nclips * p.out_clip_stride;
    const int total = p.nclips * p.nbox;
    int wgid;
    {
        const int nwg = gridDim.x, q = nwg >> 3, r = nwg & 7;
        const int xcd = blockIdx.x & 7, k = blockIdx.x >> 3;
        wgid = (xcd < r ? xcd * (q + 1) : r * (q + 1) + (xcd - r) * q) + k;
    }
    const int b_lo = wgid * boxes_per_wg;
    const int b_hi = (b_lo + boxes_per_wg < total) ? b_lo + boxes_per_wg : total;
    if (b_lo >= b_hi) return;
    const int nmine = (b_hi - b_lo + 1 - grp) >> 1;
    uint4 raw[NI][2];
    const char* rs_base = nullptr;
    int rs_f0 = 0, rs_h0 = 0, rs_w0 = 0;
    int64_t ep_base = 0;
    typedef const int32_t __attribute__((address_space(4))) * cint_p;
    typedef const int64_t __attribute__((address_space(4))) * clong_p;
    const cint_p c_boxes = (cint_p)(uintptr_t)p.boxes;
    const clong_p c_index = (clong_p)(uintptr_t)p.clip_index;
    auto prep_rows = [&](int b) {
        const int clip0 = b / p.nbox, bi = b - clip0 * p.nbox;
        const cint_p box = c_boxes + bi * 8;
        const int b6 = box[6], b7 = box[7];
        const int64_t ci = p.clip_index != nullptr ? c_index[clip0] : (int64_t)clip0;
        rs_f0 = b6 >> 16; rs_h0 = (int)(int16_t)(b6 & 0xFFFF); rs_w0 = b7;
        rs_base = reinterpret_cast<const char*>(src + ci * p.src_clip_stride4 + ((int64_t)rs_f0 * p.src_rows + rs_h0) * row4 + rs_w0);
    };
    auto prep_out = [&](int b) {
        const int clip0 = b / p.nbox, bi = b - clip0 * p.nbox;
        ep_base = (int64_t)clip0 * p.out_clip_stride + c_boxes[bi * 8 + 3];
    };
    auto load_raw = [&]() {
        const int f0 = rs_f0, h0 = rs_h0, w0 = rs_w0;
        const char* base = rs_base;
        int tv = tg;
        asm volatile("" : "+v"(tv));
        const uint32_t off_valid = (uint32_t)((((f0 < 0 ? -f0 : 0) * p.src_rows + (h0 < 0 ? -h0 : 0)) * row4) * 4);
        const uint32_t hf16 = (uint32_t)(tv & 1) * 16u;
        const bool in_row = (w0 + 4 * (tv & 1) + 8 <= row4);
#pragma unroll
        for (int k = 0; k < NI; ++k) {
            const int it = tv + 256 * k, r = it >> 1;
            const int pl = (r * ph_magic) >> 16, h = r - pl * ph;
            const bool ok = it < nitems && (unsigned)(f0 + pl) < (unsigned)p.src_planes && (unsigned)(h0 + h) < (unsigned)p.src_rows;
            const uint32_t o1 = (ok ? (uint32_t)((pl * p.src_rows + h) * row4 * 4) : off_valid) + hf16;
            const uint32_t o2 = (ok && in_row) ? o1 + 16u : o1;
            const uint4 v0 = *reinterpret_cast<const uint4*>(base + o1);
            const uint4 v1 = *reinterpret_cast<const uint4*>(base + o2);
            const uint32_t m0 = ok ? 0xffffffffu : 0u, m1 = (ok && in_row) ? 0xffffffffu : 0u;
            raw[k][0] = make_uint4(v0.x & m0, v0.y & m0, v0.z & m0, v0.w & m0);
            raw[k][1] = make_uint4(v1.x & m1, v1.y & m1, v1.z & m1, v1.w & m1);
        }
    };
    uint32_t sink = 0;
    auto touch_rows = [&]() {
        const int f0 = rs_f0, h0 = rs_h0;
        const char* base = rs_base;
        int tv = tg;
        asm volatile("" : "+v"(tv));
        const uint32_t off_valid = (uint32_t)((((f0 < 0 ? -f0 : 0) * p.src_rows + (h0 < 0 ? -h0 : 0)) * row4) * 4);
        const uint32_t hf16 = (uint32_t)(tv & 1) * 16u;
#pragma unroll
        for (int k = 0; k < NI; ++k) {
            const int it = tv + 256 * k, r = it >> 1;
            const int pl = (r * ph_magic) >> 16, h = r - pl * ph;
            const bool ok = it < nitems && (unsigned)(f0 + pl) < (unsigned)p.src_planes && (unsigned)(h0 + h) < (unsigned)p.src_rows;
            const uint32_t o1 = (ok ? (uint32_t)((pl * p.src_rows + h) * row4 * 4) : off_valid) + hf16;
            asm volatile("global_load_dword %0, %1, %2" : "+v"(sink) : "v"(o1), "s"(base) : "memory");
        }
    };
    auto expand = [&]() {
        int tv = tg;
        asm volatile("" : "+v"(tv));
#pragma unroll
        for (int k = 0; k < NI; ++k) {
            const int it = tv + 256 * k, r = it >> 1;
            if (it >= nitems) continue;
            const int pl = (r * ph_magic) >> 16, h = r - pl * ph;
            const uint4 a = raw[k][0], c = raw[k][1];
            uint4* dst = reinterpret_cast<uint4*>(patch + (pl * pitch_f + h * pitch_h + 4 * (tv & 1)) * 16);
            dst[0] = a;
            dst[1] = make_uint4(a.y, a.z, a.w, c.x);
            dst[2] = make_uint4(a.z, a.w, c.x, c.y);
            dst[3] = make_uint4(a.w, c.x, c.y, c.z);
        }
    };
    f32x16 acc[MTW];
    unsigned long long t_sum[6] = {0, 0, 0, 0, 0, 0}, t_last = 0, t_first = 0;
    auto tick = [&](int k) {
        if (VD_DBG(p) & 8) {
            unsigned long long t;
            asm volatile("s_memtime %0\n\ts_waitcnt lgkmcnt(0)" : "=s"(t) :: "memory");
            if (k >= 0) t_sum[k] += t - t_last;
            else if (k == -2) t_first = t;
            t_last = t;
        }
    };
    const int b_first = (b_lo + grp < b_hi) ? b_lo + grp : b_hi - 1;
    prep_rows(b_first);
    load_raw();
    if (grp == 0) {
        expand();
        if (FS) prep_rows(b_first + 2 < b_hi ? b_first + 2 : b_first);
    }
    {
        const int set = (p.w_set_clips > 0) ? (b_first / p.nbox) / p.w_set_clips : 0;
        cur_set = set; load_breg(set);
    }
    __syncthreads();
    tick(-2);
    const int n0 = (b_hi - b_lo + 1) >> 1;
    for (int q = 0; q <= 2 * n0; ++q) {
        const int j = (q - grp) >> 1;
        const bool k_phase = ((q + grp) & 1) == 0;
        if (k_phase) {
            if (j >= 0 && j < nmine) {
                const int b = b_lo + grp + 2 * j;
                if (p.w_set_clips > 0) {
                    const int set = (b / p.nbox) / p.w_set_clips;
                    if (set != cur_set) { cur_set = set; load_breg(set); }
                }
                prep_out(b);
                if constexpr (!FS) prep_rows(j + 1 < nmine ? b + 2 : b);
                tick(0);
#pragma unroll
                for (int i = 0; i < MTW; ++i)
#pragma unroll
                    for (int k = 0; k < 16; ++k) acc[i][k] = 0.f;
                if constexpr (FS) {
                    constexpr int D = VD_L0_D, NR = 68;
                    constexpr int FSTRIDE = 3 * PF * 16;
                    uint4 R[D];
                    const char* pa = patch + a_off[0] + half * (PH * 16);
                    const char* pb = patch + a_off[0] + half * ((PF - 6 * PH) * 16);
                    const char* pl0 = patch + a_off[0] + half * FSTRIDE;
                    const char* pl1 = patch + a_off[0];
                    auto tapq = [](int qq) constexpr { return ((qq / 7) * PF + (qq % 7) * PH) * 16; };
                    auto rd = [&](auto rc) -> uint4 {
                        constexpr int r = decltype(rc)::v;
                        if constexpr (r < 60) {
                            constexpr int jj = r / 6, f = r % 6;
                            return *reinterpret_cast<const uint4*>((jj == 3 ? pb : pa) + f * FSTRIDE + tapq(2 * jj));
                        } else {
                            constexpr int i = (r - 60) & 3, st = (r - 60) >> 2;
                            return *reinterpret_cast<const uint4*>((st ? pl1 : pl0) + (i + 2 * st) * FSTRIDE + tapq(20));
                        }
                    };
                    vd_static_for<D>([&](auto rc) { R[decltype(rc)::v] = rd(rc); });
                    if (VD_L0_PRIO) __builtin_amdgcn_s_setprio(3);
                    vd_static_for<NR>([&](auto rc) {
                        constexpr int r = decltype(rc)::v;
                        if constexpr (r < 60) {
                            constexpr int jj = r / 6, f = r % 6;
                            vd_static_for<3>([&](auto kc) {
                                constexpr int kt = decltype(kc)::v, i = f - kt;
                                if constexpr (i >= 0 && i < MTW) {
                                    acc[i] = mfma16<PREC>(R[r % D], breg[3 * jj + kt], acc[i]);
                                    __builtin_amdgcn_sched_barrier(0);
                                }
                            });
                        } else {
                            acc[(r - 60) & 3] = mfma16<PREC>(R[r % D], breg[30 + ((r - 60) >> 2)], acc[(r - 60) & 3]);
                            __builtin_amdgcn_sched_barrier(0);
                        }
                        if constexpr (r + D < NR) {
                            R[r % D] = rd(VdIC<r + D>{});
                            __builtin_amdgcn_sched_barrier(0);
                        }
                        if constexpr (r == 5 && VD_L0_TOUCH) { touch_rows(); __builtin_amdgcn_sched_barrier(0); }
                    });
                    if (VD_L0_PRIO) __builtin_amdgcn_s_setprio(0);
                } else {
                    uint4 A[2][MTW];
                    const int tp0 = lds_tap[half], tp1 = lds_tap[2 + half];
#pragma unroll
                    for (int i = 0; i < MTW; ++i) A[0][i] = *reinterpret_cast<const uint4*>(patch + a_off[i] + tp0);
#pragma unroll
                    for (int i = 0; i < MTW; ++i) A[1][i] = *reinterpret_cast<const uint4*>(patch + a_off[i] + tp1);
                    int tp2 = lds_tap[4 + half];
#pragma unroll
                    for (int s = 0; s < S; ++s) {
                        const int tp3 = lds_tap[2 * ((s + 3 < S) ? s + 3 : S - 1) + half];
#pragma unroll
                        for (int i = 0; i < MTW; ++i) {
                            acc[i] = mfma16<PREC>(A[s & 1][i], breg[s], acc[i]);
                            __builtin_amdgcn_sched_barrier(0);
                            if (s + 2 < S) A[s & 1][i] = *reinterpret_cast<const uint4*>(patch + a_off[i] + tp2);
                            __builtin_amdgcn_sched_barrier(0);
                        }
                        tp2 = tp3;
                    }
                }
                tick(1);
            }
        } else {
            const int jn = (q + 1 - grp) >> 1;
            const bool have_prev = jn - 1 >= 0 && jn - 1 < nmine;
            load_raw();
            __builtin_amdgcn_sched_barrier(0);
            if (have_prev) {
#pragma unroll
                for (int i = 0; i < MTW; ++i) {
#pragma unroll
                    for (int qh = 0; qh < 2; ++qh) {
                        const int r0 = 8 * qh;
                        float m0 = fmaxf(fmaxf(acc[i][r0], acc[i][r0 + 1]), fmaxf(acc[i][r0 + 2], acc[i][r0 + 3]));
                        float m1 = fmaxf(fmaxf(acc[i][r0 + 4], acc[i][r0 + 5]), fmaxf(acc[i][r0 + 6], acc[i][r0 + 7]));
                        m0 = fmaxf(m0 + bias, 0.f); m1 = fmaxf(m1 + bias, 0.f);
                        const int ql = (i * 4 + half + 2 * qh) * 2;
                        uint16_t hi, lo;
                        split16<PREC>(m0, hi, lo);
                        stg16[ql * 32 + (lane & 31)] = hi;
                        split16<PREC>(m1, hi, lo);
                        stg16[(ql + 1) * 32 + (lane & 31)] = hi;
                    }
                }
            }
            __builtin_amdgcn_sched_barrier(0);
            tick(3);
            expand();
            __builtin_amdgcn_sched_barrier(0);
            tick(4);
            if (have_prev) {
                const int64_t out_base = ep_base;
                const int64_t lim64 = out_total - out_base;
                const int lim = (int)(lim64 > 0x7fffffff ? 0x7fffffff : (lim64 < 0 ? 0 : lim64));
                uint4* dslots = reinterpret_cast<uint4*>(p.dst) + out_base;
                const uint4* stg4 = reinterpret_cast<const uint4*>(stg16);
#pragma unroll
                for (int k = 0; k < 2; ++k) {
                    const int item = lane + 64 * k;
                    const int ch = item & 3;
                    const uint4 v = stg4[item];
                    const int base = o_reg[k];
                    if (base >= 0 && base < lim)
                        dslots[(uint32_t)base + (uint32_t)(wn * 4 + ch) * (uint32_t)p.out_chunk_stride] = v;
                }
            }
            if constexpr (FS) {
                const int bn = b_lo + grp + 2 * (jn + 1 < nmine ? jn + 1 : (jn < nmine ? jn : (nmine > 0 ? nmine - 1 : 0)));
                prep_rows(bn < b_hi ? bn : b_hi - 1);
            }
        }
        tick(k_phase ? -1 : 5);
        VD_LDS_BARRIER();
        tick(k_phase ? 2 : 5);
    }
    if ((VD_DBG(p) & 8) && p.stamps != nullptr && (tid & 255) == 0) {
        unsigned long long* o = reinterpret_cast<unsigned long long*>(p.stamps) + ((size_t)wgid * 2 + grp) * 8;
        for (int k = 0; k < 6; ++k) o[k] = t_sum[k];
        o[6] = (unsigned long long)nmine;
        o[7] = t_last - t_first;
    }
    asm volatile("s_waitcnt vmcnt(0)" :: "v"(sink) : "memory");
}

template <int PREC, bool FS>
static int launch_conv0_breg(const VdConvParams& p, hipStream_t st) {
    const int64_t total = (int64_t)p.nclips * p.nbox;
    if (total <= 0) return 0;
    auto kern = conv0_breg_kernel<PREC, FS>;
    static VdDevCache cache;
    int ncu = 0;
    if (int rc = vd_dev_prepare(reinterpret_cast<const void*>(kern), cache, ncu)) return rc;
    const size_t lds = (size_t)2 * p.lds_plane_bytes + 512 + 8 * 2048;
    if (lds > 160 * 1024) return -3;
    const int64_t slots = (int64_t)ncu;
    const int gens = p.persist > 0 ? p.persist : 4;
    int per = (int)((total + slots * gens - 1) / (slots * gens));
    if (per < 2) per = 2;
    per += per & 1;
    const int64_t grid = (total + per - 1) / per;
    hipLaunchKernelGGL(kern, dim3((unsigned)grid), dim3(512), lds, st, p, per);
    return (int)hipGetLastError();
}

extern "C" int vd_conv0_breg(const VdConvParams* pp, void* stream) {
    if (pp == nullptr) return -1;
    const VdConvParams& p = *pp;
    if (p.NT != 2 || p.MW != 2 || p.MTW != 4 || (p.NTW != 0 && p.NTW != 1) || p.S != 32 || p.CC != 1 || p.ncl != 1 ||
        p.ntypes != 1 || p.epi != VD_EPI_POOL_CL || p.pool_t != 1 || p.argmax != nullptr || !p.relu ||
        8 * 1024 > p.lds_plane_bytes || p.src_planes <= 0 || p.src_rows <= 0 || p.type_desc == nullptr)
        return -2;
    hipStream_t st = reinterpret_cast<hipStream_t>(stream);
    VdConvParams q = p;
    q.persist = p.persist & 0xFFFF;
    const bool fs = (p.pair_flip & 0xF) != 0 && (p.pair_flip >> 8) == (9 | (189 << 8)) && !(p.persist & 0x80000);
    if (p.prec == VD_PREC_F16) return fs ? launch_conv0_breg<VD_PREC_F16, true>(q, st) : launch_conv0_breg<VD_PREC_F16, false>(q, st);
    if (p.prec == VD_PREC_BF16) return fs ? launch_conv0_breg<VD_PREC_BF16, true>(q, st) : launch_conv0_breg<VD_PREC_BF16, false>(q, st);
    return -2;
}

template <int PREC, int MTW, bool SO = false, int NTW = 1, int BAL = 0, bool SQ = false>
static int launch(const VdConvParams& p, hipStream_t st) {
    constexpr bool X3 = (PREC == VD_PREC_BF16X3 || PREC == VD_PREC_F16X3 || PREC == VD_PREC_F16C8);
    const int groups = (p.nclips + p.ncl - 1) / p.ncl;
    const int64_t total = (int64_t)groups * p.nbox;
    if (total <= 0) return 0;
    size_t lds = (size_t)((X3 && !SQ) ? 2 : 1) * p.lds_plane_bytes +
                 (size_t)(2 * p.S + (p.MW * MTW + BAL) * 4 + (PREC == VD_PREC_F16C8 ? p.S / 4 : 0)) * sizeof(int) + 16;
    if (lds > 160 * 1024) return -3;
    if ((p.dbg & 0x100) && lds < 100 * 1024) lds = 100 * 1024;
    auto kern = conv_mfma_kernel<PREC, MTW, SO, NTW, BAL, SQ>;
    if (p.NT % NTW != 0) return -2;
    const int ncols = p.NT / NTW;
    static VdDevCache cache;
    int ncu = 0;
    if (int rc = vd_dev_prepare(reinterpret_cast<const void*>(kern), cache, ncu)) return rc;
    int occ = (int)((160 * 1024) / lds);
    const int waves_per_simd = VD_OCC(PREC, MTW, NTW, BAL);
    const int wg_waves = ncols * p.MW;
    const int by_regs = (waves_per_simd * 4) / wg_waves;
    if (occ > by_regs) occ = by_regs;
    if (occ < 1) occ = 1;
    const int64_t slots = (int64_t)ncu * occ;
    const int gens = p.persist & 0xFFFF;
    int per = (gens > 0 && MTW * NTW <= 4) ? (int)((total + slots * gens - 1) / (slots * gens)) : 1;
    if (per < 1) per = 1;
    const int64_t grid = (total + per - 1) / per;
    hipLaunchKernelGGL(kern, dim3((unsigned)grid), dim3(64 * ncols * p.MW), lds, st, p, per, (int)total);
    return (int)hipGetLastError();
}

static bool vd_first_level_seq_enabled() {
    static const bool on = [] { const char* e = getenv("VD_X3_SEQ"); return !(e && e[0] == '0'); }();
    return on;
}

extern "C" int vd_conv_mfma(const VdConvParams* pp, void* stream) {
    if (pp == nullptr) return -1;
    const VdConvParams& p = *pp;
    hipStream_t st = reinterpret_cast<hipStream_t>(stream);
    const int ntw = p.NTW > 0 ? p.NTW : 1;
    if (p.NT % ntw != 0) return -2;
    const int wgw = (p.NT / ntw) * p.MW;
    if (wgw < 1 || wgw > 4 || p.lds_plane_bytes % 16 != 0) return -2;
    if (p.ncl * 65536 <= 0 || p.S <= 0 || p.CC <= 0) return -2;
    if (p.MTW * ntw < 8 && (p.gather_stride >> 6) > (int64_t)wgw * (p.MTW * ntw <= 4 ? 14 : 17)) return -2;
    if (p.clip_index != nullptr && (p.ncl != 1 || p.CC != 1 || p.MTW * ntw > 4)) return -2;
    if (p.prec == VD_PREC_F16C8) {
        if (ntw != 1 || p.MTW != 4 || p.S % 4 != 0 || (p.epi != VD_EPI_POOL_FEAT && p.epi != VD_EPI_POS_FEAT) || p.out_scale == nullptr ||
            p.select || p.atomic || p.src_split_cc > 0 || p.emit_lo != 0)
            return -2;
        if (p.epi == VD_EPI_POS_FEAT && (p.MW != 1 || p.NT != 4 || p.pool_t != 2 || p.argmax != nullptr || p.w_box_stride <= 0)) return -2;
        if (p.epi != VD_EPI_POS_FEAT && p.w_box_stride != 0) return -2;
        return launch<VD_PREC_F16C8, 4>(p, st);
    }
    if (p.emit_lo != 0) {
        const int mt_tot = p.MW * p.MTW + ((ntw == 2 && p.MTW == 3) ? 1 : 0);
        if (p.prec > VD_PREC_F16 || p.epi != VD_EPI_POOL_CL || p.argmax != nullptr || p.dst_plane_stride <= 0 ||
            (int64_t)2 * mt_tot * 4 * (p.pool_t == 2 ? 1 : 2) * p.NT * 32 * 2 > p.lds_plane_bytes)
            return -2;
    }
    if (ntw == 2 && p.MTW == 3) {
        if (p.MW != 2 || p.NT != 4 || p.select || p.src_split_cc > 0 || p.atomic || p.w_box_stride != 0) return -2;
        if ((p.gather_stride >> 6) > (int64_t)4 * 17) return -2;
        if (p.prec == VD_PREC_F16) return launch<VD_PREC_F16, 3, false, 2, 1>(p, st);
        if (p.prec == VD_PREC_BF16) return launch<VD_PREC_BF16, 3, false, 2, 1>(p, st);
        return -2;
    }
    if (ntw == 2) {
        if ((p.MTW != 4 && p.MTW != 2) || p.select || p.src_split_cc > 0 || p.atomic || p.w_box_stride != 0) return -2;
        switch (p.prec) {
            case VD_PREC_BF16: return p.MTW == 4 ? launch<VD_PREC_BF16, 4, false, 2>(p, st) : launch<VD_PREC_BF16, 2, false, 2>(p, st);
            case VD_PREC_F16: return p.MTW == 4 ? launch<VD_PREC_F16, 4, false, 2>(p, st) : launch<VD_PREC_F16, 2, false, 2>(p, st);
            case VD_PREC_BF16X3: return p.MTW == 4 ? launch<VD_PREC_BF16X3, 4, false, 2>(p, st) : launch<VD_PREC_BF16X3, 2, false, 2>(p, st);
            case VD_PREC_F16X3: return p.MTW == 4 ? launch<VD_PREC_F16X3, 4, false, 2>(p, st) : launch<VD_PREC_F16X3, 2, false, 2>(p, st);
            default: return -2;
        }
    }
    if (ntw != 1) return -2;
    if (p.MTW != 5 && (p.atomic || p.w_box_stride != 0 || p.select || p.src_split_cc > 0)) {
        if (p.select == 2 && (p.epi != VD_EPI_POOL_CL || p.argmax == nullptr)) return -2;
        if (p.prec == VD_PREC_F16X3) {
            if (p.MTW == 2) return launch<VD_PREC_F16X3, 2, true>(p, st);
            if (p.MTW == 4) return launch<VD_PREC_F16X3, 4, true>(p, st);
            if (p.MTW == 7) return launch<VD_PREC_F16X3, 7, true>(p, st);
            if (p.MTW == 8) return launch<VD_PREC_F16X3, 8, true>(p, st);
            return -2;
        }
        if (p.prec != VD_PREC_BF16X3) return -2;
        if (p.MTW == 2) return launch<VD_PREC_BF16X3, 2, true>(p, st);
        if (p.MTW == 4) return launch<VD_PREC_BF16X3, 4, true>(p, st);
        if (p.MTW == 7) return launch<VD_PREC_BF16X3, 7, true>(p, st);
        if (p.MTW == 8) return launch<VD_PREC_BF16X3, 8, true>(p, st);
        return -2;
    }
    const int64_t sq_stage = (p.epi == VD_EPI_POOL_CL && p.argmax == nullptr)
        ? (int64_t)2 * p.MW * p.MTW * 4 * (p.pool_t == 2 ? 1 : 2) * p.NT * 32 * 2 : 0;
    if (p.MTW == 4 && p.CC == 1 && p.ncl == 1 && sq_stage <= p.lds_plane_bytes && vd_first_level_seq_enabled()) {
        if (p.prec == VD_PREC_BF16X3) return launch<VD_PREC_BF16X3, 4, false, 1, 0, true>(p, st);
        if (p.prec == VD_PREC_F16X3) return launch<VD_PREC_F16X3, 4, false, 1, 0, true>(p, st);
    }
#define VD_DISPATCH(PR)                                                   \
    case PR:                                                              \
        if (p.MTW == 2) return launch<PR, 2>(p, st);                      \
        if (p.MTW == 4) return launch<PR, 4>(p, st);                      \
        if (p.MTW == 5) return launch<PR, 5>(p, st);                      \
        if (p.MTW == 7) return launch<PR, 7>(p, st);                      \
        if (p.MTW == 8) return launch<PR, 8>(p, st);                      \
        return -2;
    switch (p.prec) {
        VD_DISPATCH(VD_PREC_BF16)
        VD_DISPATCH(VD_PREC_F16)
        VD_DISPATCH(VD_PREC_BF16X3)
        VD_DISPATCH(VD_PREC_F16X3)
        default: return -2;
    }
#undef VD_DISPATCH
}

template <int PREC, int MTW, bool SO = false>
static int launch_multi(const VdConvParams* const* pp, int n, hipStream_t st) {
    constexpr bool X3 = (PREC == VD_PREC_BF16X3 || PREC == VD_PREC_F16X3);
    VdConvMulti m;
    ::memset(&m, 0, sizeof(m));
    size_t lds = 0;
    int64_t grid = 0;
    int used = 0;
    const int threads = 64 * pp[0]->NT * pp[0]->MW;
    for (int k = 0; k < n; ++k) {
        const VdConvParams& p = *pp[k];
        const int groups = (p.nclips + p.ncl - 1) / p.ncl;
        const int64_t total = (int64_t)groups * p.nbox;
        if (total <= 0) continue;
        if (total > 0x3fffffff) return -2;
        const size_t l = (size_t)(X3 ? 2 : 1) * p.lds_plane_bytes + (size_t)(2 * p.S + p.MW * MTW * 4) * sizeof(int) + 16;
        if (l > lds) lds = l;
        m.p[used] = p;
        m.first[used] = (int)grid;
        m.total[used] = (int)total;
        grid += (total + 7) & ~(int64_t)7;
        ++used;
    }
    if (used == 0) return 0;
    if (lds > 160 * 1024 || grid > 0x7fffffff) return -3;
    for (int k = used; k <= VD_MULTI_MAX; ++k) m.first[k] = (int)grid;
    auto kern = conv_mfma_multi_kernel<PREC, MTW, SO>;
    static VdDevCache cache;
    int ncu = 0;
    if (int rc = vd_dev_prepare(reinterpret_cast<const void*>(kern), cache, ncu)) return rc;
    hipLaunchKernelGGL(kern, dim3((unsigned)grid), dim3(threads), lds, st, m);
    return (int)hipGetLastError();
}

extern "C" int vd_conv_mfma_multi(const VdConvParams* const* pp, int n, void* stream) {
    if (pp == nullptr || n < 1 || n > VD_MULTI_MAX) return -1;
    for (int k = 0; k < n; ++k)
        if (pp[k] == nullptr) return -1;
    if (n == 1) return vd_conv_mfma(pp[0], stream);
    hipStream_t st = reinterpret_cast<hipStream_t>(stream);
    const VdConvParams& a = *pp[0];
    bool so = false;
    const bool so0 = a.atomic || a.select || a.src_split_cc > 0;
    for (int k = 0; k < n; ++k) {
        const VdConvParams& p = *pp[k];
        if ((p.atomic || p.select || p.src_split_cc > 0) != so0) return -2;
        if (p.prec != a.prec || p.MTW != a.MTW || p.NT != a.NT || p.MW != a.MW || (p.NTW != 0 && p.NTW != 1)) return -2;
        const int wgw = p.NT * p.MW;
        if (wgw < 1 || wgw > 4 || p.lds_plane_bytes % 16 != 0 || p.ncl * 65536 <= 0 || p.S <= 0 || p.CC <= 0) return -2;
        if (p.MTW < 8 && (p.gather_stride >> 6) > (int64_t)wgw * (p.MTW <= 4 ? 14 : 17)) return -2;
        if (p.clip_index != nullptr || p.emit_lo != 0 || p.w_box_stride != 0 || p.MTW == 5) return -2;
        so = so || p.atomic || p.select || p.src_split_cc > 0;
    }
    if (so) {
        if (a.prec == VD_PREC_F16X3) {
            if (a.MTW == 2) return launch_multi<VD_PREC_F16X3, 2, true>(pp, n, st);
            if (a.MTW == 4) return launch_multi<VD_PREC_F16X3, 4, true>(pp, n, st);
            if (a.MTW == 7) return launch_multi<VD_PREC_F16X3, 7, true>(pp, n, st);
            if (a.MTW == 8) return launch_multi<VD_PREC_F16X3, 8, true>(pp, n, st);
            return -2;
        }
        if (a.prec != VD_PREC_BF16X3) return -2;
        if (a.MTW == 2) return launch_multi<VD_PREC_BF16X3, 2, true>(pp, n, st);
        if (a.MTW == 4) return launch_multi<VD_PREC_BF16X3, 4, true>(pp, n, st);
        if (a.MTW == 7) return launch_multi<VD_PREC_BF16X3, 7, true>(pp, n, st);
        if (a.MTW == 8) return launch_multi<VD_PREC_BF16X3, 8, true>(pp, n, st);
        return -2;
    }
#define VD_DISPATCH_MULTI(PR)                                                \
    case PR:                                                                 \
        if (a.MTW == 2) return launch_multi<PR, 2>(pp, n, st);               \
        if (a.MTW == 4) return launch_multi<PR, 4>(pp, n, st);               \
        if (a.MTW == 7) return launch_multi<PR, 7>(pp, n, st);               \
        if (a.MTW == 8) return launch_multi<PR, 8>(pp, n, st);               \
        return -2;
    switch (a.prec) {
        VD_DISPATCH_MULTI(VD_PREC_BF16)
        VD_DISPATCH_MULTI(VD_PREC_F16)
        VD_DISPATCH_MULTI(VD_PREC_BF16X3)
        VD_DISPATCH_MULTI(VD_PREC_F16X3)
        default: return -2;
    }
#undef VD_DISPATCH_MULTI
}
```

### video_distillation_amd/distill.py

```python
from __future__ import annotations

import ctypes
import math
import collections
import os
from typing import Dict, List, Optional, Sequence, Tuple

import numpy as np
import torch

from . import plan as P

PARAM_SHAPES = ((64, 3, 3, 7, 7), (64,), (128, 64, 3, 7, 7), (128,), (128, 128, 3, 7, 7), (128,))


COLLECTIVE_CALLS = {"all_reduce": 0, "all_gather": 0, "bytes": 0, "control_all_reduce": 0}


def _all_reduce(t: torch.Tensor) -> None:
    import torch.distributed as dist
    COLLECTIVE_CALLS["all_reduce"] += 1
    COLLECTIVE_CALLS["bytes"] += t.numel() * t.element_size()
    dist.all_reduce(t, op=dist.ReduceOp.SUM)

# ... 105 lines not shown
        if self.two_streams:
            pr, ps = (int(v) for v in os.environ.get("VD_STREAM_PRIO", "0,-1").split(","))
            self.s_real = torch.cuda.Stream(device=self.device, priority=pr)
            self.s_syn = torch.cuda.Stream(device=self.device, priority=ps)
        self._ev_real = None
        self.s_prep = None
        self._real_done: Dict[int, "torch.cuda.Event"] = {}
        self._prep_slot: Optional[int] = None
        self.weight_format = prec_real if (prec_real in ("f16", "bf16") and prec_syn == prec_real + "x3"
                                           and os.environ.get("VD_VALUE_PASS", "1") == "1") else None
        self.prec_real = prec_real
        self.dither_enabled = True
        self._dither = 0
        self.resident_rows = os.environ.get("VD_RESIDENT_ROWS", "1") == "1"
        self._pool_rows = None

    def new_network(self, seed: int):
        return fresh_network_weights(seed, self.device)

    def embed_syn(self, x: torch.Tensor, weights):
        eng = self.eng_syn
        eng.set_weights(weights)
        feats, handle = eng.forward(x, keep=True)
        if self.weight_format is not None and not self._dither:
            eng.set_weights(weights, quantize=self.weight_format, quantize_levels=(0, 1) if self.real_last in ("x3", "c8") else (0, 1, 2))
            feats = eng.forward(x)
        return feats, handle

    def set_weights(self, weights, per_class: int = 0) -> None:
        self.set_real_weights(weights, per_class)
        if self.eng_syn is not self.eng_real:
            self.eng_syn.set_weights(weights)

    def set_real_weights(self, weights, per_class: int = 0, slot: Optional[int] = None) -> None:
        from . import engine
        self._dither = engine.dither_groups(int(per_class), self.prec_real) if (self.dither_enabled and self.eng_syn is not self.eng_real) else 0
        self.eng_real.set_weights(weights, dither=self._dither, slot=slot)

    def prepare_real_weights(self, weights, per_class: int, step: int, nclips: Optional[int] = None) -> None:
        if not self.two_streams or os.environ.get("VD_PREP_STREAM", "1") != "1" or \
                (nclips is not None and nclips < int(os.environ.get("VD_PREP_MIN_CLIPS", "1600"))):
            self._prep_slot = None
            return self.set_real_weights(weights, per_class)
        if self.s_prep is None:
            self.s_prep = torch.cuda.Stream(device=self.device, priority=-1)
        k = step % 2
        cur = torch.cuda.current_stream(self.device)
        self.s_prep.wait_stream(torch.cuda.default_stream(self.device))
        prev = self._real_done.get(k)
        if prev is not None:
            self.s_prep.wait_event(prev)
        for w in weights:
            w.record_stream(self.s_prep)
        with torch.cuda.stream(self.s_prep):
            self.set_real_weights(weights, per_class, slot=k)
            ev = torch.cuda.Event()
            ev.record(self.s_prep)
        cur.wait_event(ev)
        self._prep_slot = k

    def real_launches_done(self) -> None:
        if self.s_prep is not None and self._prep_slot is not None:
            ev = torch.cuda.Event()
            ev.record(torch.cuda.current_stream(self.device))
            self._real_done[self._prep_slot] = ev

    def fork(self):
        if self.two_streams:
            cur = torch.cuda.current_stream(self.device)
            self.s_real.wait_stream(cur)
            self.s_syn.wait_stream(cur)

    def on_real(self):
        return torch.cuda.stream(self.s_real) if self.two_streams else _NullCtx()

    def on_syn(self):
        return torch.cuda.stream(self.s_syn) if self.two_streams else _NullCtx()

    def real_to_syn(self, *tensors):
        if self.two_streams:
            self.s_syn.wait_stream(self.s_real)
            for t in tensors:
                t.record_stream(self.s_syn)

    C8_MIN_ABSMAX = 0.25

    def real_range(self, reset: bool = True) -> Optional[dict]:
        st = getattr(self.eng_real.fwd[1], "range_stats", None) if self.real_last == "c8" else None
        if st is None:
            return None
        sat, bits = (int(v) for v in st.cpu().numpy().view(np.uint32))
        if reset:
            st.zero_()
        return {"saturated": sat, "absmax": float(np.array([bits], dtype=np.uint32).view(np.float32)[0])}

    def check_real_range(self, force_fallback: bool = False) -> Optional[dict]:
        r = self.real_range()
        if r is None or not (self.range_is_bad(r) or force_fallback):
            return r
        return self.fall_back_to_hi_lo(r)

    def range_is_bad(self, r: Optional[dict]) -> bool:
        return r is not None and (r["saturated"] > 0 or not np.isfinite(r["absmax"]) or (0.0 < r["absmax"] < self.C8_MIN_ABSMAX))

    def fall_back_to_hi_lo(self, r: Optional[dict] = None) -> dict:
        r = dict(r or {"saturated": 0, "absmax": 0.0})
        import warnings
        warnings.warn("fp8-corrected last level outside its validated activation range (%d outputs of level 1 saturated at 1792, "
                      "max |output| %.3g): the real side's last level runs in fp16 hi+lo pairs from now on" % (r["saturated"], r["absmax"]))
        from . import engine
        old = self.eng_real
        self.eng_real = engine.EmbedEngine(self.geo, prec=old.prec_name, device=self.device, chunk=old.chunk, last_hilo=True)
        self.real_last = "x3"
        self._pool_rows = None
        self._prep_slot = None
        self._real_done = {}
        r["fallback"] = "x3"
        return r

    def join(self, *tensors):
        if self.two_streams:
            cur = torch.cuda.current_stream(self.device)
            cur.wait_stream(self.s_real)
            cur.wait_stream(self.s_syn)
            for t in tensors:
                t.record_stream(cur)

    def embed_pool(self, pool: torch.Tensor, index: torch.Tensor, per_class: int = 0) -> torch.Tensor:
        segs = [(index.numel() // per_class, per_class)] if (per_class and index.numel() % per_class == 0) else None
        return self.embed_pool_segments(pool, index, segs)

    def embed_pool_segments(self, pool: torch.Tensor, index: torch.Tensor, segments) -> torch.Tensor:
        rows = None
        if self.resident_rows:
            key = (pool.data_ptr(), tuple(pool.shape))
            if self._pool_rows is None or self._pool_rows[0] != key:
                self._pool_rows = (key, self.eng_real.pool_rows(pool))
            rows = self._pool_rows[1]
        G = self._dither
        if G and segments and all(per % G == 0 for _, per in segments) and sum(n * per for n, per in segments) == index.numel():
            key = (tuple(segments), G, str(index.device))
            perm = self._seg_perm.get(key) if hasattr(self, "_seg_perm") else None
            if perm is None:
                pos, parts = 0, [[] for _ in range(G)]
                for n, per in segments:
                    blk = torch.arange(pos, pos + n * per).view(n, per // G, G)
                    for g in range(G):
                        parts[g].append(blk[:, :, g].reshape(-1))
                    pos += n * per
                perm = torch.cat([torch.cat(pg) for pg in parts]).to(index.device)
                if not hasattr(self, "_seg_perm"):
                    self._seg_perm = {}
                self._seg_perm[key] = perm
            f = self.eng_real.forward_sets(pool, index[perm], rows=rows)
            out = torch.empty_like(f)
            out[perm] = f
            return out
        return self.eng_real.forward(pool, index=index, rows=rows)

    def embed_keep(self, x: torch.Tensor):
        return self.eng_syn.forward(x, keep=True)

    def embed_backward(self, handle, g: torch.Tensor) -> torch.Tensor:
        return self.eng_syn.backward(handle, g)

    def dm_loss(self, f_real: torch.Tensor, f_syn: torch.Tensor, nclass: int):
        nreal, nsyn, dim = f_real.shape[0] // max(nclass, 1), f_syn.shape[0] // max(nclass, 1), self.num_feat
        loss = torch.empty(nclass, dtype=torch.float32, device=self.device)
        g = torch.empty_like(f_syn)
        hip = self.hip
        hip.check(hip.lib().vd_dm_loss(hip.ptr(f_real), hip.ptr(f_syn), nclass, nreal, nsyn, dim, hip.ptr(loss),
                                       hip.ptr(g), hip.stream_ptr(self.device)), "vd_dm_loss")
        return loss, g

    def group_sum(self, x: torch.Tensor, groups: int, per: int, scale: float) -> torch.Tensor:
        hip = self.hip
        out = torch.empty((groups, x.shape[1]), dtype=torch.float32, device=self.device)
        hip.check(hip.lib().vd_group_sum(hip.ptr(x), groups, per, x.shape[1], ctypes.c_float(scale), hip.ptr(out),
                                         hip.stream_ptr(self.device)), "vd_group_sum")
        return out

    def sgd(self, x: torch.Tensor, buf: torch.Tensor, g: torch.Tensor, lr: float, mu: float, first: bool) -> None:
        hip = self.hip
        hip.check(hip.lib().vd_sgd_momentum(hip.ptr(x), hip.ptr(buf), hip.ptr(g), ctypes.c_int64(x.numel()),
                                            ctypes.c_float(lr), ctypes.c_float(mu), int(first),
                                            hip.stream_ptr(self.device)), "vd_sgd_momentum")

    def hallucinate(self, static, dynamic, sidx, didx, w, b):
        hip = self.hip
        n, T, H, W = int(sidx.numel()), dynamic.shape[-4], dynamic.shape[-2], dynamic.shape[-1]
        out = torch.empty((n, T, 3, H, W), dtype=torch.float32, device=self.device)
        hip.check(hip.lib().vd_hallucinator_fwd(hip.ptr(static), hip.ptr(dynamic), hip.ptr(sidx), hip.ptr(didx),
                                                hip.ptr(w), hip.ptr(b), n, T, H, W, hip.ptr(out),
                                                hip.stream_ptr(self.device)), "vd_hallucinator_fwd")
        return out

    def hallucinate_backward(self, g_out, static, dynamic, sidx, didx, w, need_static: bool):
        hip = self.hip
        n, T, H, W = int(sidx.numel()), dynamic.shape[-4], dynamic.shape[-2], dynamic.shape[-1]
        g_dyn = torch.zeros_like(dynamic)
        g_stat = torch.zeros_like(static) if need_static else None
        g_w = torch.zeros(324, dtype=torch.float32, device=self.device)
        g_b = torch.zeros(3, dtype=torch.float32, device=self.device)
        hip.check(hip.lib().vd_hallucinator_bwd(hip.ptr(g_out), hip.ptr(static), hip.ptr(dynamic), hip.ptr(sidx),
                                                hip.ptr(didx), hip.ptr(w), n, T, H, W, hip.ptr(g_dyn),
                                                hip.ptr(g_stat), hip.ptr(g_w), hip.ptr(g_b),
                                                hip.stream_ptr(self.device)), "vd_hallucinator_bwd")
        return g_dyn, g_stat, g_w.view(3, 4, 3, 3, 3), g_b


class RealPool:

    def __init__(self, clips: torch.Tensor, counts: Sequence[int], offsets: Sequence[int]):
        self.clips, self.counts, self.offsets = clips, list(counts), list(offsets)

    @staticmethod
    def synthetic(num_classes: int, classes: Sequence[int], per_class: int, geo: P.NetGeometry, device, seed: int = 1234,
                  kind: str = "randn", noise: float = 2.0):
        assert kind in ("randn", "templates")
        n = len(classes) * per_class
        clips = torch.empty((n, geo.frames, 3, geo.height, geo.width), dtype=torch.float32, device=device)
        counts = [per_class] * num_classes
        offsets = [0] * num_classes
        for k, c in enumerate(classes):
            gen = torch.Generator(device=device)
            gen.manual_seed(int(seed) * 1000003 + int(c))
            blk = clips[k * per_class:(k + 1) * per_class]
            blk.normal_(generator=gen)
            if kind == "templates":
                t = torch.randn((geo.frames * 3, 1, geo.height, geo.width), dtype=torch.float32, device=device, generator=gen)
                t = torch.nn.functional.avg_pool2d(t, 9, 1, 4).view(1, geo.frames, 3, geo.height, geo.width) * 6.0
                blk.mul_(float(noise)).add_(t)
            mean = blk.mean(dim=(0, 1, 3, 4), keepdim=True)
            std = blk.std(dim=(0, 1, 3, 4), keepdim=True)
            blk.sub_(mean).div_(std)
            offsets[c] = k * per_class
        return RealPool(clips, counts, offsets)

    @staticmethod
    def from_dataset(dataset, num_classes: int, classes: Sequence[int], device, workers: int = 8):
        from . import dataset as D
        per_class = D.indices_class(dataset.labels, num_classes)
        order = [i for c in classes for i in per_class[c]]
        clips, _ = D.preload(dataset, device, indices=order, workers=workers)
        counts = [len(per_class[c]) for c in range(num_classes)]
        offsets, o = [0] * num_classes, 0
        for c in classes:
            offsets[c] = o
            o += counts[c]
        return RealPool(clips, counts, offsets)


def check_real_range(trainer) -> None:
    be = trainer.be
    every = int(os.environ.get("VD_RANGE_CHECK_EVERY", "1"))
    if every <= 0 or not hasattr(be, "check_real_range") or getattr(be, "real_last", None) != "c8":
        return
    trainer._range_calls = getattr(trainer, "_range_calls", 0) + 1
    if trainer._range_calls % every:
        return
    torch.cuda.synchronize(be.device)
    force = False
    if collectives_on(getattr(trainer, "world", 1)):
        flag = torch.tensor([1.0 if be.range_is_bad(be.real_range(reset=False)) else 0.0], device=be.device)
        _all_reduce_max(flag)
        force = bool(flag.item() > 0)
    r = be.check_real_range(force_fallback=force)
    if r is not None and r.get("fallback"):
        r["fallback_at_sync"] = trainer._range_calls
        r["fallback_decided_by"] = "max over ranks" if force else "this rank"
    if r is not None and (r["absmax"] > 0.0 or r["saturated"] > 0 or getattr(trainer, "real_range", None) is None):
        trainer.real_range = r


class DMTrainer:

    def __init__(self, backend, pool: RealPool, num_classes: int, ipc: int, batch_real: int, lr_img: float,
                 momentum: float = 0.5, rank: int = 0, world: int = 1, image_syn: Optional[torch.Tensor] = None,
                 shard: str = "class", exchange: str = "owner", comm=None):
        assert shard in ("class", "batch", "hybrid")
        self.shard = shard if (world > 1 or os.environ.get("VD_FORCE_BATCH_SHARD") == "1") else "class"
        if self.shard in ("batch", "hybrid") and batch_real % world != 0:
            raise ValueError("shard=%r needs batch_real (%d) divisible by the number of ranks (%d): every rank embeds the same share of a "
                             "split class batch; use shard='class' (distill.choose_shard falls back to it)" % (self.shard, batch_real, world))
        self.be, self.pool = backend, pool
        self.num_classes, self.ipc, self.batch_real = num_classes, ipc, batch_real
        self.lr_img, self.momentum = float(lr_img), float(momentum)
        self.rank, self.world = rank, world
        self.c_lo, self.c_hi = class_range(num_classes, rank, world)
        self.classes = list(range(self.c_lo, self.c_hi))
        if self.shard == "hybrid":
            self.block, self.split, self.split_owned = hybrid_partition(num_classes, rank, world)
            self.classes = self.block + self.split_owned
        if image_syn is None:
            idx = np.concatenate([pool.offsets[c] + np.arange(ipc) % pool.counts[c] for c in self.classes]) \
                if self.classes else np.zeros(0, dtype=np.int64)
            image_syn = pool.clips[torch.as_tensor(idx, device=pool.clips.device, dtype=torch.int64)].clone()
        self.image_syn = image_syn.contiguous()
        self.buf = torch.zeros_like(self.image_syn)
        self.steps_done = 0
        assert exchange in ("owner", "allreduce")
        self.exchange, self.comm = exchange, comm
        self.exchange_events = collections.deque(maxlen=512)
        self._g_full = None
        self._pending = None
        self.defer_backward = os.environ.get("VD_DEFER_BWD", "1" if getattr(backend, "real_last", None) == "c8" else "0") == "1"

    def _allreduce_pixel_grad(self, grad: torch.Tensor) -> torch.Tensor:
        if self.world == 1 and self.comm is None:
            return grad
        if self._g_full is None:
            self._g_full = torch.empty((self.num_classes * self.ipc,) + tuple(grad.shape[1:]), dtype=grad.dtype, device=grad.device)
            own = self.owned_classes()
            self._g_rows = (torch.as_tensor(own, device=grad.device, dtype=torch.int64).view(-1, 1) * self.ipc
                            + torch.arange(self.ipc, device=grad.device)).view(-1)
        full = self._g_full
        full.zero_()
        full.index_copy_(0, self._g_rows, grad)
        timed = full.is_cuda
        if timed:
            e0, e1 = torch.cuda.Event(enable_timing=True), torch.cuda.Event(enable_timing=True)
            e0.record()
        if self.comm is not None:
            COLLECTIVE_CALLS["all_reduce"] += 1
            COLLECTIVE_CALLS["bytes"] += full.numel() * full.element_size()
            self.comm.all_reduce(full)
        else:
            import torch.distributed as dist
            if dist.is_available() and dist.is_initialized():
                _all_reduce(full)
        if timed:
            e1.record()
            self.exchange_events.append((e0, e1))
        return full.index_select(0, self._g_rows)

    def owned_classes(self, rank: Optional[int] = None) -> List[int]:
        rank = self.rank if rank is None else rank
        if self.shard == "hybrid":
            block, _, owned = hybrid_partition(self.num_classes, rank, self.world)
            return block + owned
        lo, hi = class_range(self.num_classes, rank, self.world)
        return list(range(lo, hi))

    def step(self, it: int, overlap: bool = False) -> torch.Tensor:
        be, ncls = self.be, len(self.classes)
        if self.shard == "batch":
            per = self.batch_real // self.world
            idx = sample_real_indices(it, self.pool.counts, self.pool.offsets, self.batch_real, range(self.num_classes))
            idx = idx.reshape(self.num_classes, self.batch_real)[:, self.rank * per:(self.rank + 1) * per].reshape(-1)
        elif self.shard == "hybrid":
            per = self.batch_real // self.world
            idx_s = sample_real_indices(it, self.pool.counts, self.pool.offsets, self.batch_real, self.split)
            idx_s = idx_s.reshape(len(self.split), self.batch_real)[:, self.rank * per:(self.rank + 1) * per].reshape(-1)
            idx = np.concatenate([sample_real_indices(it, self.pool.counts, self.pool.offsets, self.batch_real, self.block), idx_s])
        else:
            idx = sample_real_indices(it, self.pool.counts, self.pool.offsets, self.batch_real, self.classes)
        dev = self.image_syn.device
        idx_t = torch.as_tensor(idx, device=dev)
        weights = be.new_network(seed=it)
        fork, on_real, on_syn = getattr(be, "fork", None), getattr(be, "on_real", _NullCtx), getattr(be, "on_syn", _NullCtx)
        if fork:
            fork()
        if getattr(be, "two_streams", False):
            idx_t.record_stream(be.s_real)
            for w in weights:
                w.record_stream(be.s_real)
                w.record_stream(be.s_syn)
            defer = overlap and self.defer_backward
            ev_l0 = None
            with on_real():
                if hasattr(be, "prepare_real_weights"):
                    be.prepare_real_weights(weights, self._per_class(), self.steps_done, nclips=int(idx.size))
                else:
                    be.set_real_weights(weights, self._per_class())
                if defer:
                    ev_l0 = torch.cuda.Event()
                    be.eng_real.after_first_level = lambda: ev_l0.record(be.s_real)
                try:
                    f_real = self._real_features(idx_t)
                finally:
                    be.eng_real.after_first_level = None
                if hasattr(be, "real_launches_done"):
                    be.real_launches_done()
            with on_syn():
                self._flush_backward(ev_l0 if defer else None)
                f_syn, handle = be.embed_syn(self.image_syn, weights)
                be.real_to_syn(f_real)
                f_real = self._exchange(f_real)
                loss_c, g_syn = be.dm_loss(f_real, f_syn, ncls)
                self._pending = (handle, g_syn, self.steps_done == 0)
                if not defer:
                    self._flush_backward(None)
                loss = loss_c.sum()
            if not overlap:
                be.join(loss)
            self.steps_done += 1
            return loss
        self._flush_backward(None)
        if hasattr(be, "set_real_weights"):
            be.set_weights(weights, self._per_class())
        else:
            be.set_weights(weights)
        f_real = self._exchange(self._real_features(idx_t))
        f_syn, handle = be.embed_syn(self.image_syn, weights) if hasattr(be, "embed_syn") else be.embed_keep(self.image_syn)
        loss_c, g_syn = be.dm_loss(f_real, f_syn, ncls)
        grad = be.embed_backward(handle, g_syn)
        if self.exchange == "allreduce":
            grad = self._allreduce_pixel_grad(grad)
        be.sgd(self.image_syn, self.buf, grad, self.lr_img, self.momentum, first=(self.steps_done == 0))
        self.steps_done += 1
        return loss_c.sum()

    def _flush_backward(self, after: Optional["torch.cuda.Event"]) -> None:
        if self._pending is None:
            return
        handle, g_syn, first = self._pending
        self._pending = None
        be = self.be
        if after is not None:
            torch.cuda.current_stream(self.image_syn.device).wait_event(after)
        grad = be.embed_backward(handle, g_syn)
        if self.exchange == "allreduce":
            grad = self._allreduce_pixel_grad(grad)
        be.sgd(self.image_syn, self.buf, grad, self.lr_img, self.momentum, first=first)

    def _real_features(self, idx_t: torch.Tensor) -> torch.Tensor:
        be = self.be
        if self.shard == "hybrid":
            nb, ns, per = len(self.block), len(self.split), self.batch_real // self.world
            if hasattr(be, "embed_pool_segments"):
                f = be.embed_pool_segments(self.pool.clips, idx_t, [(n, p) for n, p in ((nb, self.batch_real), (ns, per)) if n])
            else:
                f = be.embed_pool(self.pool.clips, idx_t)
            parts = []
            if nb:
                parts.append(be.group_sum(f[:nb * self.batch_real].contiguous(), nb, self.batch_real, 1.0 / self.batch_real))
            if ns:
                parts.append(be.group_sum(f[nb * self.batch_real:].contiguous(), ns, per, 1.0 / self.batch_real))
            return torch.cat(parts, 0)
        f = be.embed_pool(self.pool.clips, idx_t, self._per_class()) if hasattr(be, "set_real_weights") else \
            be.embed_pool(self.pool.clips, idx_t)
        if self.shard != "batch":
            return f
        return be.group_sum(f, self.num_classes, self.batch_real // self.world, 1.0 / self.batch_real)

    def _per_class(self) -> int:
        return self.batch_real // self.world if self.shard in ("batch", "hybrid") else self.batch_real

    def _exchange(self, x: torch.Tensor) -> torch.Tensor:
        if self.shard == "class":
            return x
        import torch.distributed as dist
        live = dist.is_available() and dist.is_initialized()
        if self.shard == "hybrid":
            nb = len(self.block)
            if not self.split:
                return x
            part = x[nb:].contiguous()
            if live:
                _all_reduce(part)
            if not self.split_owned:
                return x[:nb].contiguous()
            if getattr(self, "_own_idx", None) is None or self._own_idx.device != x.device:
                self._own_idx = torch.as_tensor([self.split.index(c) for c in self.split_owned], dtype=torch.int64, device=x.device)
            return torch.cat([x[:nb], part.index_select(0, self._own_idx)], 0)
        if live:
            _all_reduce(x)
        return x[self.c_lo:self.c_hi].contiguous()

    def global_loss(self, local_loss: torch.Tensor) -> torch.Tensor:
        be = self.be
        ctx = be.on_syn() if getattr(be, "two_streams", False) else _NullCtx()
        with ctx:
            if collectives_on(self.world):
                import torch.distributed as dist
                local_loss = local_loss.clone()
                _all_reduce(local_loss)
        return local_loss

    def sync(self) -> None:
        if getattr(self.be, "two_streams", False):
            if getattr(self, "_pending", None) is not None:
                with self.be.on_syn():
                    self._flush_backward(None)
            self.be.join()
        check_real_range(self)

    def mark(self):
        ev = torch.cuda.Event(enable_timing=True)
        ev.record(self.be.s_syn if getattr(self.be, "two_streams", False) else torch.cuda.current_stream(self.image_syn.device))
        return ev

    def gather_syn(self) -> torch.Tensor:
        if hasattr(self, "sync"):
            self.sync()
        if not collectives_on(self.world):
            return self.image_syn
        import torch.distributed as dist
        owners = [self.owned_classes(r) if hasattr(self, "owned_classes") else
                  list(range(*class_range(self.num_classes, r, self.world))) for r in range(self.world)]
        sizes = [len(o) * self.ipc for o in owners]
        mx = max(sizes)
        pad = torch.zeros((mx,) + tuple(self.image_syn.shape[1:]), dtype=self.image_syn.dtype, device=self.image_syn.device)
        pad[:self.image_syn.shape[0]] = self.image_syn
        parts = [torch.empty_like(pad) for _ in range(self.world)]
        _all_gather(parts, pad)
        out = torch.cat([p[:s] for p, s in zip(parts, sizes)], dim=0)
        order = [c for o in owners for c in o]
        if order != sorted(order):
            pos = torch.as_tensor(np.argsort(order), device=out.device)
            out = out.view(len(order), self.ipc, *out.shape[1:])[pos].reshape(out.shape)
        return out


class S2DTrainer:

    def __init__(self, backend, pool: RealPool, num_classes: int, vpc: int, spc: int, dpc: int, batch_real: int,
                 static_syn: torch.Tensor, dynamic_syn: torch.Tensor, hal_w: torch.Tensor, hal_b: torch.Tensor,
                 lr_dynamic: float, lr_hal: float, lr_static: float = 0.0, train_static: bool = False,
                 momentum: float = 0.95, rank: int = 0, world: int = 1):
        self.be, self.pool = backend, pool
        self.num_classes, self.vpc, self.spc, self.dpc, self.batch_real = num_classes, vpc, spc, dpc, batch_real
        self.rank, self.world = rank, world
        self.c_lo, self.c_hi = class_range(num_classes, rank, world)
        self.classes = list(range(self.c_lo, self.c_hi))
        self.static = static_syn[self.c_lo * spc:self.c_hi * spc].contiguous()
        self.dynamic = dynamic_syn[self.c_lo:self.c_hi].reshape((-1,) + tuple(dynamic_syn.shape[2:])).contiguous()
        self.hal_w, self.hal_b = hal_w.clone().contiguous(), hal_b.clone().contiguous()
        self.lr_dynamic, self.lr_hal, self.lr_static = float(lr_dynamic), float(lr_hal), float(lr_static)
        self.train_static, self.momentum = train_static, float(momentum)
        self.buf_d = torch.zeros_like(self.dynamic)
        self.buf_w, self.buf_b = torch.zeros_like(self.hal_w), torch.zeros_like(self.hal_b)
        self.buf_s = torch.zeros_like(self.static) if train_static else None
        self.steps_done = 0
        self._pending = None
        self.last_grads = None
        self.defer_backward = os.environ.get("VD_DEFER_BWD", "1" if getattr(backend, "real_last", None) == "c8" else "0") == "1"

    def indices(self, it: int, draws: Optional[Tuple[np.ndarray, np.ndarray]] = None):
        ncls = len(self.classes)
        label = np.repeat(np.arange(ncls), self.vpc)
        idx = np.tile(np.arange(self.vpc), ncls)
        if draws is None:
            dd = np.concatenate([np.random.default_rng([it, c, 1]).integers(0, 2, self.vpc) for c in self.classes]) if ncls else idx
            ds = np.concatenate([np.random.default_rng([it, c, 2]).integers(0, 2, self.vpc) for c in self.classes]) if ncls else idx
        else:
            dd, ds = draws[0][self.c_lo * self.vpc:self.c_hi * self.vpc], draws[1][self.c_lo * self.vpc:self.c_hi * self.vpc]
        dynamic_idx = label * self.dpc + 2 * idx + dd
        static_idx = self.spc * label + 2 * idx + ds
        return static_idx.astype(np.int64), dynamic_idx.astype(np.int64)

    def step(self, it: int, draws=None, overlap: bool = False) -> torch.Tensor:
        be, ncls = self.be, len(self.classes)
        dev = self.dynamic.device
        weights = be.new_network(seed=it)
        sidx_np, didx_np = self.indices(it, draws)
        sidx, didx = torch.as_tensor(sidx_np, device=dev), torch.as_tensor(didx_np, device=dev)
        idx = sample_real_indices(it, self.pool.counts, self.pool.offsets, self.batch_real, self.classes)
        idx_t = torch.as_tensor(idx, device=dev)
        two = getattr(be, "two_streams", False)
        on_real, on_syn = (be.on_real, be.on_syn) if two else (_NullCtx, _NullCtx)
        if two:
            be.fork()
            idx_t.record_stream(be.s_real)
            for t in (sidx, didx):
                t.record_stream(be.s_syn)
            for w in weights:
                w.record_stream(be.s_real)
                w.record_stream(be.s_syn)
            defer = overlap and self.defer_backward
            ev_l0 = None
            with on_real():
                be.prepare_real_weights(weights, self.batch_real, self.steps_done, nclips=int(idx.size))
                if defer:
                    ev_l0 = torch.cuda.Event()
                    be.eng_real.after_first_level = lambda: ev_l0.record(be.s_real)
                try:
# ... 491 lines not shown
```

### video_distillation_amd/engine.py

```python
from __future__ import annotations

import ctypes
import threading
import os
from typing import Dict, List, Optional, Sequence, Tuple

import numpy as np
import torch

from . import hip
from . import plan as P


LAUNCH_PROFILE: Optional[list] = None


class _DevPlan:

    def __init__(self, plan: P.ConvPlan, device, prec: int):
        self.plan = plan
        desc, tables = plan.flat_tables()
        self.type_desc = torch.from_numpy(desc.copy()).to(device)
        self.tables = torch.from_numpy(tables.copy()).to(device)
        self.boxes = torch.from_numpy(plan.device_boxes().copy()).to(device)
        self.widx = torch.from_numpy(plan.widx.reshape(-1).copy()).to(device)
        gt = plan.gather_table()
        self.gather = torch.from_numpy(gt.copy()).to(device)
        self.n_w = int(self.widx.numel())
        planes = 2 if hip.is_x3(prec) else 1
        self.prec = prec
        self.wpk = self._new_wpk(planes, device)
        self.wpk_d: Optional[torch.Tensor] = None
        self.range_stats: Optional[torch.Tensor] = None
        self._slots: Dict[int, tuple] = {}
        self._slot = 0
        p = hip.VdConvParams()
        p.type_desc = self.type_desc.data_ptr(); p.tables = self.tables.data_ptr(); p.boxes = self.boxes.data_ptr()
        p.gather = self.gather.data_ptr(); p.gather_stride = int(gt.shape[1])
        p.nbox = plan.nbox; p.ncl = plan.ncl
        p.CC, p.S = plan.CC, plan.S
        p.src_clip_stride4, p.src_chunk_stride4 = plan.clip_stride4, plan.chunk_stride4
        p.NT, p.MW, p.MTW, p.NTW = plan.NT, plan.MW, plan.MTW, plan.NTW
        mt_max = max(t.mt for t in plan.types)
        p.mt_valid = mt_max if (plan.NTW == 2 and mt_max < plan.MW * plan.MTW and os.environ.get("VD_SKIP_PAD", "1") == "1") else 0
        p.epi, p.pool_t, p.relu = plan.epi, plan.pool_t, int(plan.relu)
        p.n_out, p.n_stride = plan.n_out, plan.n_stride
        p.out_clip_stride = plan.out_clip_stride
        p.out_chunk_stride, p.out_t_stride = plan.out_chunk_stride, plan.out_t_stride
        p.pair_flip = plan.pair_flip
        p.lds_plane_bytes = int(gt.shape[1]) * 16
        p.ntypes = len(plan.types)
        p.persist = int(os.environ.get("VD_PERSIST", str(P.BOX_WALK_GENERATIONS)))
        if os.environ.get("VD_NO_ALT") == "1":
            p.persist |= 0x100000
        p.tab_ofs[0], p.tab_ofs[1], p.tab_ofs[2] = int(desc[0][7]), int(desc[0][8]), int(desc[0][9])
        self.zero = torch.zeros(64, dtype=torch.uint8, device=device)
        p.zero_slot = self.zero.data_ptr()
        p.prec = prec
        p.wpk = self.wpk.data_ptr(); p.w_plane_stride = self.n_w
        p.w_box_stride = plan.w_box_stride; p.atomic = int(plan.atomic)
        self.col_off = None if plan.col_off is None else torch.from_numpy(plan.col_off.copy()).to(device)
        p.col_off = 0 if self.col_off is None else self.col_off.data_ptr()
        self.params = p
        self.breg_variant = int(os.environ.get("VD_L0_BREG", "5"))
        self.breg_ok = bool(self.breg_variant in (4, 5) and not hip.is_x3(prec)
                            and plan.epi == P.EPI_POOL_CL and plan.pool_t == 1 and plan.CC == 1 and plan.ncl == 1 and plan.NTW == 1
                            and (plan.NT, plan.MW, plan.MTW, plan.S) == (2, 2, 4, 32) and len(plan.types) == 1
                            and plan.relu and plan.row_source()[1] > 0)
        if plan.row_source()[1] > 0:
            p.src_planes, p.src_rows = plan.row_source()

    def _new_wpk(self, planes: int, device) -> torch.Tensor:
        slack = 16384 if self.prec == hip.PREC["f16c8"] else 0
        flat = torch.zeros(planes * self.n_w + slack, dtype=torch.int16, device=device) if slack else \
            torch.empty(planes * self.n_w, dtype=torch.int16, device=device)
        return flat[:planes * self.n_w].view(planes, self.n_w)

    def use_slot(self, k: int) -> None:
        self._slots[self._slot] = (self.wpk, self.wpk_d)
        if k not in self._slots:
            self._slots[k] = (self._new_wpk(self.wpk.shape[0], self.wpk.device), None)
        self.wpk, self.wpk_d = self._slots[k]
        self._slot = k

    def pack(self, w: torch.Tensor) -> None:
        assert w.dtype == torch.float32 and w.is_contiguous()
        lo = self.wpk[1] if self.wpk.shape[0] == 2 else None
        if _PACK.queue is not None and self.n_w > 0:
            _PACK.queue.append((w, self.widx, self.n_w, self.wpk[0], lo, self.prec))
            return
        hip.check(hip.lib().vd_pack_weights(hip.ptr(w), hip.ptr(self.widx), ctypes.c_int64(self.n_w),
                                            hip.ptr(self.wpk[0]), hip.ptr(lo), self.prec, hip.stream_ptr(w.device)),
                  "vd_pack_weights")

    def pack_c8(self, w: torch.Tensor, scales: torch.Tensor) -> None:
        assert w.dtype == torch.float32 and w.is_contiguous() and self.wpk.shape[0] == 2
        pl = self.plan
        sets = self.n_w // (pl.CC * pl.S * pl.NT * 512)
        hip.check(hip.lib().vd_pack_weights_c8(hip.ptr(w), ctypes.c_int64(w.numel()), hip.ptr(self.widx), sets * pl.CC, pl.S, pl.NT,
                                               hip.ptr(self.wpk[0]), hip.ptr(self.wpk[1]), hip.ptr(scales), hip.stream_ptr(w.device)),
                  "vd_pack_weights_c8")

    def pack_dither(self, w: torch.Tensor, groups: int) -> None:
        assert w.dtype == torch.float32 and w.is_contiguous() and self.wpk.shape[0] == 1
        if self.wpk_d is None or self.wpk_d.shape[0] != groups:
            self.wpk_d = torch.empty((groups, self.n_w), dtype=torch.int16, device=w.device)
        hip.check(hip.lib().vd_pack_weights_dither(hip.ptr(w), hip.ptr(self.widx), ctypes.c_int64(self.n_w), int(groups),
                                                   hip.ptr(self.wpk_d), self.prec, hip.stream_ptr(w.device)), "vd_pack_weights_dither")

    def run(self, src: torch.Tensor, src_plane_slots: int, bias: Optional[torch.Tensor], dst_ptr: int,
            dst_plane_stride: int, argmax: Optional[torch.Tensor], nclips: int, out_scale: Optional[torch.Tensor] = None,
            wpk: Optional[torch.Tensor] = None, w_plane_elems: int = 0, clip_index: Optional[torch.Tensor] = None,
            group: Optional[int] = None, set_clips: int = 0, emit_lo: bool = False, launch: bool = True) -> None:
        p = self.params
        p.emit_lo = int(emit_lo)
        if int(emit_lo) == 2 and _RANGE_MONITOR:
            if self.range_stats is None:
                self.range_stats = torch.zeros(2, dtype=torch.int32, device=src.device)
            p.range_stats = self.range_stats.data_ptr()
        else:
            p.range_stats = 0
        p.clip_index = 0 if clip_index is None else clip_index.data_ptr()
        p.out_scale = 0 if out_scale is None else out_scale.data_ptr()
        p.w_set_clips = 0
        if wpk is not None:
            p.wpk = wpk.data_ptr(); p.w_plane_stride = w_plane_elems
        elif group is not None:
            p.wpk = self.wpk_d[group].data_ptr(); p.w_plane_stride = self.n_w
        elif set_clips > 0:
            assert set_clips % self.plan.ncl == 0
            p.wpk = self.wpk_d.data_ptr(); p.w_plane_stride = self.n_w; p.w_set_clips = int(set_clips)
        else:
            p.wpk = self.wpk.data_ptr(); p.w_plane_stride = self.n_w
        p.src = src.data_ptr(); p.src_plane_stride4 = src_plane_slots * 4
        p.bias = 0 if bias is None else bias.data_ptr()
        p.dst = dst_ptr; p.dst_plane_stride = dst_plane_stride
        p.argmax = 0 if argmax is None else argmax.data_ptr()
        p.nclips = nclips
        if not launch:
            return
        prof = LAUNCH_PROFILE
        if prof is not None:
            e0, e1 = torch.cuda.Event(enable_timing=True), torch.cuda.Event(enable_timing=True)
            e0.record()
        if self.breg_ok and argmax is None and (not p.dbg or os.environ.get("VD_BREG_DBG") == "1"):
            persist = p.persist
            if self.breg_variant == 4:
                p.persist = persist | 0x80000
            try:
                hip.check(hip.lib().vd_conv0_breg(ctypes.byref(p), hip.stream_ptr(src.device)), "vd_conv0_breg(%s)" % self.plan.name)
            finally:
                p.persist = persist
        else:
            hip.check(hip.lib().vd_conv_mfma(ctypes.byref(p), hip.stream_ptr(src.device)), "vd_conv_mfma(%s)" % self.plan.name)
        if prof is not None:
            e1.record()
            prof.append((self.plan.name, self.prec, 2.0 * self.plan.meta.get("macs_per_unit", 0) * nclips, e0, e1))


def GRAD_TARGET() -> float:
    return float(os.environ.get("VD_GRAD_TARGET", "1024"))


_RANGE_MONITOR = os.environ.get("VD_RANGE_MONITOR", "1") == "1"


class _PackState(threading.local):
    queue: Optional[list] = None


_PACK = _PackState()


class batched_packs:

    def __enter__(self):
        self.outer = _PACK.queue is not None or os.environ.get("VD_PACK_BATCH", "1") != "1"
        if not self.outer:
            _PACK.queue = []
        return self

    def __exit__(self, *exc):
        if self.outer:
            return False
        q, _PACK.queue = _PACK.queue, None
        if exc[0] is None:
            flush_packs(q)
        return False


def flush_packs(q) -> None:
    for i in range(0, len(q), hip.VD_PACK_MAX):
        part = q[i:i + hip.VD_PACK_MAX]
        b = hip.VdPackBatch()
        b.nseg = len(part)
        for k, (w, widx, n, hi, lo, prec) in enumerate(part):
            sg = b.seg[k]
            sg.w, sg.widx, sg.n = w.data_ptr(), widx.data_ptr(), int(n)
            sg.out_hi, sg.out_lo, sg.prec = hi.data_ptr(), (0 if lo is None else lo.data_ptr()), int(prec)
        hip.check(hip.lib().vd_pack_weights_multi(ctypes.byref(b), hip.stream_ptr(part[0][0].device)), "vd_pack_weights_multi")


def run_together(plans: Sequence["_DevPlan"], *args, **kwargs) -> None:
    plans = list(plans)
    if len(plans) < 2 or os.environ.get("VD_MULTI_LAUNCH", "1") != "1":
        for dp in plans:
            dp.run(*args, **kwargs)
        return
    groups: Dict[tuple, list] = {}
    for dp in plans:
        pl, p = dp.plan, dp.params
        so = bool(p.atomic or p.select or p.src_split_cc > 0)
        plain = pl.NTW in (0, 1) and pl.MTW in (2, 4, 7, 8) and not p.w_box_stride and not p.dbg and (not so or hip.is_x3(dp.prec))
        key = (dp.prec, pl.MTW, pl.NT, pl.MW, so) if plain else ("single", id(dp))
        groups.setdefault(key, []).append(dp)
    for key, grp in groups.items():
        for i in range(0, len(grp), 4):
            part = grp[i:i + 4]
            if len(part) == 1 or key[0] == "single":
                for dp in part:
                    dp.run(*args, **kwargs)
                continue
            for dp in part:
                dp.run(*args, launch=False, **kwargs)
            arr = (ctypes.POINTER(hip.VdConvParams) * len(part))(*[ctypes.pointer(dp.params) for dp in part])
            prof = LAUNCH_PROFILE
            if prof is not None:
                e0, e1 = torch.cuda.Event(enable_timing=True), torch.cuda.Event(enable_timing=True)
                e0.record()
            dev = part[0].tables.device
            hip.check(hip.lib().vd_conv_mfma_multi(arr, len(part), hip.stream_ptr(dev)),
                      "vd_conv_mfma_multi(%s)" % ",".join(dp.plan.name for dp in part))
            if prof is not None:
                e1.record()
                nclips = int(part[0].params.nclips)
                name = os.path.commonprefix([dp.plan.name for dp in part]).rstrip("_") + "_x%d" % len(part)
                prof.append((name, part[0].prec, sum(2.0 * dp.plan.meta.get("macs_per_unit", 0) * nclips for dp in part), e0, e1))


def dither_groups(n: int, prec: str) -> int:
    want = int(os.environ.get("VD_REAL_DITHER", "8"))
    if prec not in ("f16", "bf16") or want < 4 or n < 4:
        return 0
    g = 1
    while g * 2 <= min(want, n) and n % (g * 2) == 0:
        g *= 2
    return g if g >= 4 else 0


def round_weights(params: Sequence[torch.Tensor], prec: str, levels: Sequence[int] = (0, 1, 2)) -> List[torch.Tensor]:
    out, L = [], hip.lib()
    for i, p in enumerate(params):
        if i % 2 == 0 and p.dim() == 5 and i < 6 and (i // 2) in levels:
            p = p.detach().to(torch.float32).contiguous()
            q = torch.empty_like(p)
            hip.check(L.vd_round_operand(hip.ptr(p), ctypes.c_int64(p.numel()), hip.PREC[prec], hip.ptr(q),
                                         hip.stream_ptr(p.device)), "vd_round_operand")
            out.append(q)
        else:
            out.append(p)
    return out


class EmbedEngine:
    def __init__(self, geo: P.NetGeometry, prec: str = "bf16x3", device="cuda:0", chunk: int = 256,
                 prec_bwd: Optional[str] = None, ntw0: Optional[int] = None, batch_hint: Optional[int] = None,
                 last_hilo: bool = False, bwd0_small: bool = False):
        if not torch.cuda.is_available():
            raise RuntimeError("EmbedEngine needs a HIP device (no CPU fallback)")
        hip.lib()
        self.geo = geo
        self.prec_name = prec
        self.prec = hip.PREC[prec]
        self.planes = 2 if hip.is_x3(self.prec) else 1
        self.device = torch.device(device)
        self.chunk = int(chunk)
        self.ntw = int(os.environ.get("VD_NTW", "2"))
        if ntw0 is None:
            breg = os.environ.get("VD_L0_BREG", "5") in ("4", "5")
            ntw0 = int(os.environ.get("VD_NTW0", "1" if (hip.is_x3(self.prec) or self.ntw != 2 or breg) else "2"))
        bal = (self.ntw == 2 and not hip.is_x3(self.prec) and os.environ.get("VD_BALANCED", "1") == "1")
        self.batch_hint = batch_hint
        net = P.plan_network(geo, ntw=self.ntw, ntw0=ntw0, balanced=bal, batch_hint=batch_hint, bwd0_small=bwd0_small)
        self.dims = net["dims"]
        self.fwd = [_DevPlan(pl, self.device, self.prec) for pl in net["fwd"]]
        self.fwd2x = None
        self.last_c8 = False
        self._c8_scale_slots: Dict[int, torch.Tensor] = {}
        if last_hilo:
            if hip.is_x3(self.prec):
                raise ValueError("last_hilo is an option of the single-pass formats (%s already carries hi+lo planes)" % prec)
            import dataclasses
            pl2 = net["fwd"][2]
            if os.environ.get("VD_L2X_PLAN", "small") == "small" and pl2.NTW == 2 and pl2.MTW == 4 and pl2.ncl % 2 == 0:
                d2 = self.dims[2]
                try:
                    alt = P.plan_forward_cl("fwd2", d2[0], d2[1], d2[2], d2[3], d2[4], d2[11], feat_out=True, ntw=1, mtw_options=(4,),
                                            step_multiple=4 if last_hilo == "c8" else 1)
                    if alt.rows_total <= pl2.rows_total and 2 * alt.gather_table().shape[1] * 16 <= 72 * 1024:
                        pl2 = alt
                except ValueError:
                    pass
            self.last_c8 = (last_hilo == "c8")
            if self.last_c8:
                d2 = self.dims[2]
                pos = None
                if prec == "f16" and os.environ.get("VD_C8_POS", "1") == "1":
                    try:
                        pos = P.plan_forward_pos("fwd2_pos", d2[0], d2[1], d2[2], d2[3], d2[4], d2[11])
                    except (ValueError, AssertionError):
                        pos = None
                if pos is not None:
                    pl2 = pos
                elif prec == "f16" and pl2.NTW == 1 and pl2.MTW == 4 and pl2.S % 4 == 0:
                    pl2 = P.with_skip_table(dataclasses.replace(pl2, types=[dataclasses.replace(t) for t in pl2.types]))
                else:
                    raise ValueError("last_hilo='c8' needs the f16 format and either position tiles (frames dividing 32) or the one-clip "
                                     "4 x 1-tile last-level program (geometry %s)" % (geo,))
            self.fwd2x = _DevPlan(dataclasses.replace(pl2, name="fwd2_c8" if self.last_c8 else "fwd2_hilo"), self.device,
                                  hip.PREC["f16c8"] if self.last_c8 else hip.PREC[prec + "x3"])
            if self.last_c8:
                self.c8_scales = torch.zeros(8, dtype=torch.float32, device=self.device)
                if pl2.epi == P.EPI_POS_FEAT and os.environ.get("VD_C8_BOXMAJOR", "0") == "1":
                    self.fwd2x.params.persist |= 0x80000
        self.prec_bwd = hip.PREC[prec_bwd] if prec_bwd else self.prec
        self.planes_bwd = 2 if hip.is_x3(self.prec_bwd) else 1
        self.bwd = [[_DevPlan(pl, self.device, self.prec_bwd) for pl in layer] for layer in net["bwd"]]
        self.num_feat = geo.num_feat
        self._weights: Optional[List[torch.Tensor]] = None
        self._bwd_packed = False
        self._ws: Dict[str, torch.Tensor] = {}
        self.profile = None

    def _buf(self, name: str, shape, dtype) -> torch.Tensor:
        t = self._ws.get(name)
        n = int(np.prod(shape))
        if t is None or t.numel() < n or t.dtype != dtype:
            t = torch.empty(n, dtype=dtype, device=self.device)
            self._ws[name] = t
        return t[:n].view(*shape)

    def set_weights(self, params: Sequence[torch.Tensor], quantize: Optional[str] = None, dither: int = 0,
                    quantize_levels: Sequence[int] = (0, 1, 2), slot: Optional[int] = None) -> None:
        ws = [p.detach().to(self.device, torch.float32).contiguous() for p in params[:6]]
        if quantize is not None:
            ws = round_weights(ws, quantize, quantize_levels)
        self._weights = ws
        if slot is not None:
            for dp in self.fwd + ([self.fwd2x] if self.fwd2x is not None else []):
                dp.use_slot(slot)
            if self.last_c8:
                if slot not in self._c8_scale_slots:
                    self._c8_scale_slots[slot] = torch.zeros(8, dtype=torch.float32, device=self.device)
                self.c8_scales = self._c8_scale_slots[slot]
        with batched_packs():
            for li in range(3):
                if li == 2 and self.fwd2x is not None:
                    if self.last_c8:
                        self.fwd2x.pack_c8(ws[4], self.c8_scales)
                    else:
                        self.fwd2x.pack(ws[4])
                    continue
                self.fwd[li].pack(ws[2 * li])
                if dither >= 2:
                    self.fwd[li].pack_dither(ws[2 * li], dither)
        self._dither = int(dither) if dither >= 2 else 0
        self._bwd_packed = False

    def _pack_bwd(self) -> None:
        if not self._bwd_packed:
            with batched_packs():
                for li in range(3):
                    for dp in self.bwd[li]:
                        dp.pack(self._weights[2 * li])
            if os.environ.get("VD_BWD_X2_SIM") == "w":
                if _PACK.queue:
                    flush_packs(_PACK.queue)
                    del _PACK.queue[:]
                for li in range(3):
                    for dp in self.bwd[li]:
                        if dp.wpk.shape[0] == 2:
                            dp.wpk[1].zero_()
            self._bwd_packed = True

    def pool_rows(self, pool: torch.Tensor, step: int = 256) -> torch.Tensor:
        g = self.geo
        N = int(pool.shape[0])
        rowp = P.pix_row_pitch(g.width)
        per = g.frames * 3 * g.height * (rowp // 8)
        rows = torch.empty((self.planes, N * per, 8), dtype=torch.int16, device=self.device)
        L, st = hip.lib(), hip.stream_ptr(self.device)
        for i in range(0, N, step):
            nb = min(step, N - i)
            lo = rows[1, i * per:] if self.planes == 2 else None
            hip.check(L.vd_pix2rows(hip.ptr(pool[i:]), hip.ptr(None), ctypes.c_int64(nb), g.frames, g.height, g.width,
                                     hip.ptr(rows[0, i * per:]), hip.ptr(lo), self.prec, st), "vd_pix2rows")
        return rows

    def forward(self, x: torch.Tensor, keep: bool = False, index: Optional[torch.Tensor] = None,
                rows: Optional[torch.Tensor] = None, group: Optional[int] = None):
        assert self._weights is not None, "set_weights() first"
        assert group is None or 0 <= group < getattr(self, "_dither", 0), "set_weights(dither=G) first"
        g = self.geo
        assert x.dim() == 5 and tuple(x.shape[1:]) == (g.frames, g.channel, g.height, g.width), x.shape
        x = x.detach().to(torch.float32).contiguous()
        B = x.shape[0] if index is None else int(index.numel())
        if index is not None:
            index = index.to(self.device, torch.int64).contiguous()
        feats = torch.empty((B, self.num_feat), dtype=torch.float32, device=self.device)
        saved = []
        L = hip.lib()
        st = hip.stream_ptr(self.device)
        rowp = P.pix_row_pitch(g.width)
        per1 = int(np.prod(self.fwd[0].plan.out_shape[:-1]))
        per2 = int(np.prod(self.fwd[1].plan.out_shape[:-1]))
        for c0 in range(0, B, self.chunk):
            nb = min(self.chunk, B - c0)
            n_slots0 = nb * g.frames * 3 * g.height * (rowp // 8)
            cidx = None
            if rows is not None:
                assert index is not None and rows.shape[0] == self.planes
                slots0, n_slots0, cidx = rows, int(rows.shape[1]), index[c0:]
            else:
                slots0 = self._buf("slots0", (self.planes, n_slots0, 8), torch.int16)
                lo = slots0[1] if self.planes == 2 else None
                xin = x[c0:] if index is None else x
                hip.check(L.vd_pix2rows(hip.ptr(xin), hip.ptr(None if index is None else index[c0:]),
                                         ctypes.c_int64(nb), g.frames, g.height, g.width,
                                         hip.ptr(slots0[0]), hip.ptr(lo), self.prec, st), "vd_pix2rows")
            n1, n2 = nb * per1, nb * per2
            hilo = self.fwd2x is not None
            assert not (hilo and keep), "last_hilo engines have no kept-arg-max forward"
            act1 = self._buf("act1", (self.planes, n1, 8), torch.int16)
            act2 = self._buf("act2", (2 if hilo else self.planes, n2, 8), torch.int16)
            am0 = am1 = am2 = None
            if keep:
                am0 = torch.empty(n1 * 8, dtype=torch.uint8, device=self.device)
                am1 = torch.empty(n2 * 8, dtype=torch.uint8, device=self.device)
                am2 = torch.empty(nb * self.num_feat, dtype=torch.uint8, device=self.device)
            w = self._weights
            prof = self.profile
            ev = [torch.cuda.Event(enable_timing=True) for _ in range(4)] if prof is not None else None
            if ev: ev[0].record()
            self.fwd[0].run(slots0, n_slots0, w[1], act1.data_ptr(), n1, am0, nb, clip_index=cidx, group=group)
            if ev: ev[1].record()
            self.fwd[1].run(act1, n1, w[3], act2.data_ptr(), n2, am1, nb, group=group, emit_lo=(2 if self.last_c8 else 1) if hilo else 0)
            if ev: ev[2].record()
            if hilo:
                self.fwd2x.run(act2, n2, w[5], feats[c0:].data_ptr(), 0, None, nb, out_scale=self.c8_scales if self.last_c8 else None)
            else:
                self.fwd[2].run(act2, n2, w[5], feats[c0:].data_ptr(), 0, am2, nb, group=group)
            if ev:
                ev[3].record()
                prof += [("fwd0", nb, ev[0], ev[1]), ("fwd1", nb, ev[1], ev[2]), ("fwd2", nb, ev[2], ev[3])]
            if keep:
                saved.append((c0, nb, am0, am1, am2))
        if keep:
            return feats, saved
        return feats

    def forward_sets(self, x: torch.Tensor, index: torch.Tensor, rows: Optional[torch.Tensor] = None) -> torch.Tensor:
        G = getattr(self, "_dither", 0)
        B = int(index.numel())
        assert G >= 2 and B % G == 0 and self.planes == 1, "set_weights(dither=G) on a single-pass engine first"
        g = self.geo
        per = B // G
        index = index.to(self.device, torch.int64).contiguous()
        feats = torch.empty((B, self.num_feat), dtype=torch.float32, device=self.device)
        rowp = P.pix_row_pitch(g.width)
        per1 = int(np.prod(self.fwd[0].plan.out_shape[:-1]))
        per2 = int(np.prod(self.fwd[1].plan.out_shape[:-1]))
        n1, n2 = B * per1, B * per2
        hilo = self.fwd2x is not None
        act1 = self._buf("act1", (1, n1, 8), torch.int16)
        act2 = self._buf("act2", (2 if hilo else 1, n2, 8), torch.int16)
        w = self._weights
        if rows is None:
            n_slots0 = B * g.frames * 3 * g.height * (rowp // 8)
            slots0 = self._buf("slots0", (1, n_slots0, 8), torch.int16)
            hip.check(hip.lib().vd_pix2rows(hip.ptr(x.detach().to(torch.float32).contiguous()), hip.ptr(index), ctypes.c_int64(B),
                                            g.frames, g.height, g.width, hip.ptr(slots0[0]), hip.ptr(None), self.prec,
                                            hip.stream_ptr(self.device)), "vd_pix2rows")
        if self.fwd[0].breg_ok:
            if rows is not None:
                self.fwd[0].run(rows, int(rows.shape[1]), w[1], act1.data_ptr(), n1, None, B, clip_index=index, set_clips=per)
            else:
                self.fwd[0].run(slots0, n_slots0, w[1], act1.data_ptr(), n1, None, B, set_clips=per)
        else:
            for s in range(G):
                if rows is not None:
                    self.fwd[0].run(rows, int(rows.shape[1]), w[1], act1.data_ptr() + s * per * per1 * 16, n1, None, per,
                                    clip_index=index[s * per:], group=s)
                else:
                    per0 = g.frames * 3 * g.height * (rowp // 8)
                    self.fwd[0].run(slots0[:, s * per * per0:], n_slots0, w[1], act1.data_ptr() + s * per * per1 * 16, n1, None, per, group=s)
        if getattr(self, "after_first_level", None) is not None:
            self.after_first_level()
        for li, (src, n_src, per_src, dst_ptr, n_dst, per_dst_bytes) in enumerate((
                (act1, n1, per1, act2.data_ptr(), n2, per2 * 16), (act2, n2, per2, feats.data_ptr(), 0, self.num_feat * 4)), start=1):
            if li == 2 and hilo:
                if os.environ.get("VD_L2_X2_SIM") == "act":
                    src[1].zero_()
                self.fwd2x.run(src, n_src, w[5], dst_ptr, 0, None, B, out_scale=self.c8_scales if self.last_c8 else None)
            elif per % self.fwd[li].plan.ncl == 0:
                self.fwd[li].run(src, n_src, w[2 * li + 1], dst_ptr, n_dst, None, B, set_clips=per,
                                 emit_lo=(2 if self.last_c8 else 1) if (li == 1 and hilo) else 0)
            else:
                for s in range(G):
                    self.fwd[li].run(src[:, s * per * per_src:], n_src, w[2 * li + 1], dst_ptr + s * per * per_dst_bytes, n_dst, None,
                                     per, group=s, emit_lo=(2 if self.last_c8 else 1) if (li == 1 and hilo) else 0)
        return feats

    def backward(self, saved, g_feat: torch.Tensor) -> torch.Tensor:
        self._pack_bwd()
        g = self.geo
        g_feat = g_feat.detach().to(torch.float32).contiguous()
        B = g_feat.shape[0]
        dx = torch.empty((B, g.frames, g.channel, g.height, g.width), dtype=torch.float32, device=self.device)
        L = hip.lib()
        st = hip.stream_ptr(self.device)
        for c0, nb, am0, am1, am2 in saved:
            grad = g_feat[c0:c0 + nb]
            layout = 0
            for li, am in ((2, am2), (1, am1), (0, am0)):
                cin, cout, t, h, w, T, OH, OW, To, Ho, Wo, pt = self.dims[li]
                nslots = nb * (cout // 8) * T * OH * OW
                dy = self._buf("dy%d" % li, (self.planes_bwd, nslots, 8), torch.int16)
                lo = dy[1] if self.planes_bwd == 2 else None
                sc = inv = None
                if self.prec_bwd in (hip.PREC["f16"], hip.PREC["f16x3"]):
                    scb = self._buf("gscale%d" % li, (4,), torch.float32)
                    hip.check(L.vd_absmax_scale(hip.ptr(grad), ctypes.c_int64(grad.numel()), ctypes.c_float(GRAD_TARGET()),
                                                hip.ptr(scb), st), "vd_absmax_scale")
                    sc, inv = scb, scb[1:]
                hip.check(L.vd_unpool_relu_bwd(hip.ptr(grad), hip.ptr(am), ctypes.c_int64(nb), cout, To, Ho, Wo, pt,
                                               T, OH, OW, layout, hip.ptr(dy[0]), hip.ptr(lo), self.prec_bwd, hip.ptr(sc), st),
                          "vd_unpool_relu_bwd")
                if lo is not None and os.environ.get("VD_BWD_X2_SIM") == "g":
                    lo.zero_()
                if li == 0:
                    out = dx[c0:c0 + nb]
                else:
                    out = self._buf("dx%d" % li, (nb, t, h, w, cin), torch.float32)
                run_together(self.bwd[li], dy, nslots, None, out.data_ptr(), 0, None, nb, out_scale=inv)
                grad = out
                layout = 1
        return dx


class WgradOp:

    def __init__(self, cin: int, cout: int, t: int, h: int, w: int, nclips: int, prec: str, device, ordered: bool = False):
        self.cin, self.cout, self.t, self.h, self.w, self.nclips = cin, cout, t, h, w, nclips
        self.ordered = bool(ordered)
        self.prec = hip.PREC[prec]
        self.planes = 2 if hip.is_x3(self.prec) else 1
        self.device = torch.device(device)
        blk = os.environ.get("VD_WG_BLOCK")
        self.plan = P.plan_wgrad("wgrad%dx%d" % (cin, cout), cin, cout, t, h, w, nclips, block=tuple(int(v) for v in blk.split(",")) if blk else None,
                                 planes=self.planes, ordered=self.ordered)
        self.dp = _DevPlan(self.plan, self.device, self.prec)
        self.T, self.OH, self.OW = self.plan.meta["grid"]
        self.CCb = self.plan.CC
        self.npos_in = t * h * w
        self.xT = torch.empty((self.planes, cin * self.CCb * self.npos_in, 8), dtype=torch.int16, device=self.device)
        self.bp_elems = self.plan.nbox * self.plan.w_box_stride
        self.bp = torch.empty((self.planes, self.bp_elems), dtype=torch.int16, device=self.device)
        self.replicas = int(self.plan.meta["replicas"])
        self.rep = torch.empty((self.replicas, cin * 147, cout), dtype=torch.float32, device=self.device)

    def _stage_x(self, x_src: torch.Tensor, x_is_pixels: bool, x_plane_slots: int) -> None:
        L, st = hip.lib(), hip.stream_ptr(self.device)
        nb = self.nclips
        if x_is_pixels:
            lo = self.xT[1] if self.planes == 2 else None
            hip.check(L.vd_clip_minor_pix(hip.ptr(x_src), ctypes.c_int64(nb), self.t, self.h, self.w, hip.ptr(self.xT[0]),
                                          hip.ptr(lo), self.prec, st), "vd_clip_minor_pix")
        else:
            hip.check(L.vd_clip_minor_cl(hip.ptr(x_src), ctypes.c_int64(x_plane_slots), self.planes, ctypes.c_int64(nb), self.cin,
                                         ctypes.c_int64(self.npos_in), hip.ptr(self.xT), ctypes.c_int64(self.xT.shape[1]), st),
                      "vd_clip_minor_cl")

    def _accumulate(self, dw_out: torch.Tensor, out_scale: Optional[torch.Tensor]) -> None:
        L, st = hip.lib(), hip.stream_ptr(self.device)
        self.rep.zero_()
        self.dp.params.replica_stride = dw_out.numel()
        self.dp.run(self.xT, self.xT.shape[1], None, self.rep.data_ptr(), 0, None, self.cin, out_scale=out_scale, wpk=self.bp,
                    w_plane_elems=self.bp_elems)
        hip.check(L.vd_replica_sum(hip.ptr(self.rep), self.replicas, self.cin * 147, self.cout, hip.ptr(dw_out), st), "vd_replica_sum")

    def run(self, x_src: torch.Tensor, x_is_pixels: bool, x_plane_slots: int, dy: torch.Tensor, dy_plane_slots: int,
            dw_out: torch.Tensor, out_scale: Optional[torch.Tensor] = None) -> None:
        L, st = hip.lib(), hip.stream_ptr(self.device)
        self._stage_x(x_src, x_is_pixels, x_plane_slots)
        nt, noh, now = self.plan.meta["box"]
        hip.check(L.vd_pack_dy(hip.ptr(dy), ctypes.c_int64(dy_plane_slots), self.planes, ctypes.c_int64(self.nclips), self.cout, self.T,
                               self.OH, self.OW, nt, noh, now, hip.ptr(self.bp), ctypes.c_int64(self.bp_elems), st), "vd_pack_dy")
        self._accumulate(dw_out, out_scale)

    def run_pooled(self, x_src: torch.Tensor, x_is_pixels: bool, x_plane_slots: int, g_pooled: torch.Tensor, argmax: torch.Tensor,
                   g_layout: int, pooled: Tuple[int, int, int, int], scale: Optional[torch.Tensor], dw_out: torch.Tensor,
                   out_scale: Optional[torch.Tensor] = None) -> None:
        L, st = hip.lib(), hip.stream_ptr(self.device)
        self._stage_x(x_src, x_is_pixels, x_plane_slots)
        nt, noh, now = self.plan.meta["box"]
        To, Ho, Wo, pt = pooled
        lo = self.bp[1] if self.planes == 2 else None
        hip.check(L.vd_unpool_relu_bwd_packed(hip.ptr(g_pooled), hip.ptr(argmax), ctypes.c_int64(self.nclips), self.cout, To, Ho, Wo, pt,
                                              self.T, self.OH, self.OW, g_layout, nt, noh, now, hip.ptr(self.bp[0]), hip.ptr(lo),
                                              self.prec, hip.ptr(scale), st), "vd_unpool_relu_bwd_packed")
        self._accumulate(dw_out, out_scale)
```

### video_distillation_amd/hip.py

```python
from __future__ import annotations

import ctypes
import os
import subprocess
from typing import Optional

import torch

_HERE = os.path.dirname(os.path.abspath(__file__))
LIB_PATH = os.path.join(_HERE, "libvd_hip.so")
SOURCES = [os.path.join(_HERE, "csrc", f) for f in ("conv_mfma.hip", "aux_kernels.hip", "program.hip", "planner.cpp", "comm.cpp",
                                                         "coreset.hip", "clips_sample.hip")]
CSRC_HEADERS = [os.path.join(_HERE, "csrc", "frame_norm.h")]
STAMP_SOURCE = os.path.join(_HERE, "csrc", "stamp.cpp")
HEADER = os.path.join(_HERE, "..", "include", "vd_hip.h")

CORESET_METHOD = {"herding": 0, "k-center": 1}
PREC = {"bf16": 0, "f16": 1, "bf16x3": 2, "f16x3": 3, "f16c8": 4}
EXPORTS = ("vd_abi_version", "vd_conv_mfma", "vd_conv_mfma_multi", "vd_conv0_breg", "vd_pack_weights", "vd_round_operand", "vd_pix2rows", "vd_unpool_relu_bwd", "vd_absmax_scale", "vd_dm_loss",
           "vd_group_sum", "vd_sgd_momentum", "vd_hallucinator_fwd", "vd_hallucinator_bwd", "vd_match_rows_fwd", "vd_match_rows_bwd", "vd_match_rows_fwd_multi", "vd_match_rows_bwd_multi", "vd_head_fwd", "vd_clip_minor_cl", "vd_clip_minor_pix", "vd_pack_dy", "vd_bias_grad", "vd_bias_grad_pooled", "vd_standardize", "vd_head_train_fwd", "vd_ce_loss", "vd_head_train_bwd", "vd_head_second_order", "vd_resplit_slots", "vd_program_load", "vd_program_pack_weights",
           "vd_program_run", "vd_program_info", "vd_program_free",
           "vd_sgd_momentum_wd", "vd_frames_normalize", "vd_replica_sum", "vd_pack_weights_dither", "vd_unpool_relu_bwd_packed", "vd_mfma_peak", "vd_program_build", "vd_program_build_dgrad", "vd_program_build_wgrad", "vd_program_run_wgrad", "vd_train_create", "vd_train_workspace_bytes", "vd_train_step", "vd_train_free", "vd_blob_free", "vd_embed_create", "vd_embed_create_ex", "vd_embed_argmax_bytes", "vd_embed_backward_workspace_bytes",
           "vd_embed_forward_keep", "vd_embed_backward", "vd_program_run_scaled", "vd_embed_num_features",
           "vd_embed_workspace_bytes", "vd_embed_set_weights", "vd_embed_forward", "vd_embed_free",
           "vd_comm_unique_id", "vd_comm_create", "vd_comm_size", "vd_comm_version", "vd_comm_rank", "vd_comm_allreduce_f32", "vd_comm_allgather_f32",
           "vd_comm_free",
           "vd_bias_grad_pooled_scratch_floats", "vd_bias_grad_pooled_ordered", "vd_standardize_ordered", "vd_head_train_bwd_ordered",
           "vd_set_deterministic", "vd_get_deterministic", "vd_pack_weights_c8", "vd_pack_weights_multi",
           "vd_split_scaled", "vd_scale_combine", "vd_sources_hash", "vd_coreset_workspace_bytes", "vd_coreset_select",
           "vd_clips_sample")
F16X3_WSHIFT = 8


class VdConvParams(ctypes.Structure):
    _fields_ = [
        ("src", ctypes.c_void_p), ("src_plane_stride4", ctypes.c_int64),
        ("src_clip_stride4", ctypes.c_int64), ("src_chunk_stride4", ctypes.c_int64),
        ("wpk", ctypes.c_void_p), ("w_plane_stride", ctypes.c_int64), ("w_box_stride", ctypes.c_int64),
        ("bias", ctypes.c_void_p),
        ("dst", ctypes.c_void_p), ("dst_plane_stride", ctypes.c_int64),
        ("argmax", ctypes.c_void_p), ("col_off", ctypes.c_void_p), ("out_scale", ctypes.c_void_p),
        ("type_desc", ctypes.c_void_p), ("tables", ctypes.c_void_p), ("boxes", ctypes.c_void_p),
        ("gather", ctypes.c_void_p), ("gather_stride", ctypes.c_int64), ("zero_slot", ctypes.c_void_p),
        ("nbox", ctypes.c_int32), ("nclips", ctypes.c_int32), ("ncl", ctypes.c_int32),
        ("CC", ctypes.c_int32), ("S", ctypes.c_int32), ("NT", ctypes.c_int32), ("MW", ctypes.c_int32), ("MTW", ctypes.c_int32),
        ("epi", ctypes.c_int32), ("pool_t", ctypes.c_int32), ("relu", ctypes.c_int32),
        ("n_out", ctypes.c_int32), ("n_stride", ctypes.c_int32),
        ("out_clip_stride", ctypes.c_int64),
        ("out_chunk_stride", ctypes.c_int32), ("out_t_stride", ctypes.c_int32),
        ("lds_plane_bytes", ctypes.c_int32), ("prec", ctypes.c_int32), ("dbg", ctypes.c_int32), ("ntypes", ctypes.c_int32), ("tab_ofs", ctypes.c_int32 * 3), ("atomic", ctypes.c_int32), ("select", ctypes.c_int32), ("src_split_cc", ctypes.c_int32), ("src_split_off4", ctypes.c_int64), ("NTW", ctypes.c_int32), ("clip_index", ctypes.c_void_p), ("mt_valid", ctypes.c_int32), ("persist", ctypes.c_int32), ("stamps", ctypes.c_void_p),
        ("w_set_clips", ctypes.c_int32), ("replica_stride", ctypes.c_int32), ("emit_lo", ctypes.c_int32), ("src_planes", ctypes.c_int32), ("src_rows", ctypes.c_int32), ("pair_flip", ctypes.c_int32), ("range_stats", ctypes.c_void_p),
    ]


class VdMatchSeg(ctypes.Structure):
    _fields_ = [("gr", ctypes.c_void_p), ("gs", ctypes.c_void_p), ("g", ctypes.c_void_p), ("rows", ctypes.c_int64),
                ("len", ctypes.c_int32), ("reserved", ctypes.c_int32)]


VD_PACK_MAX = 24


class VdPackSeg(ctypes.Structure):
    _fields_ = [("w", ctypes.c_void_p), ("widx", ctypes.c_void_p), ("n", ctypes.c_int64), ("out_hi", ctypes.c_void_p),
                ("out_lo", ctypes.c_void_p), ("prec", ctypes.c_int32), ("first_block", ctypes.c_int32)]


class VdPackBatch(ctypes.Structure):
    _fields_ = [("nseg", ctypes.c_int32), ("reserved", ctypes.c_int32), ("seg", VdPackSeg * VD_PACK_MAX)]


class VdMatchBatch(ctypes.Structure):
    _fields_ = [("nseg", ctypes.c_int32), ("reserved", ctypes.c_int32), ("seg", VdMatchSeg * 16)]


def build(force: bool = False, verbose: bool = False, debug_hooks: bool = False) -> str:
    out = LIB_PATH.replace(".so", "_dbg.so") if debug_hooks else LIB_PATH
    if not force and library_stamp(out) == sources_hash():
        return out
    hipcc = os.environ.get("HIPCC", "/opt/rocm/bin/hipcc")
    objdir = os.path.join(_HERE, "csrc", "build_dbg" if debug_hooks else "build")
    os.makedirs(objdir, exist_ok=True)
    import fcntl
    lock = open(os.path.join(objdir, ".lock"), "w")
    fcntl.flock(lock, fcntl.LOCK_EX)
    try:
        return _build_locked(out, objdir, hipcc, force, verbose, debug_hooks)
    finally:
        fcntl.flock(lock, fcntl.LOCK_UN)
        lock.close()


def _file_hash(*paths: str) -> str:
    import hashlib
    h = hashlib.sha256()
    for path in paths:
        with open(path, "rb") as f:
            h.update(f.read())
    return h.hexdigest()[:16]


def _build_locked(out: str, objdir: str, hipcc: str, force: bool, verbose: bool, debug_hooks: bool) -> str:
    want = sources_hash()
    if not force and library_stamp(out) == want:
        return out
    flags = ["-O3", "--offload-arch=gfx950", "-fPIC"] + (["-DVD_DBG_HOOKS=1"] if debug_hooks else [])
    jobs, objs = [], []
    for src in SOURCES:
        obj = os.path.join(objdir, os.path.basename(src) + ".o")
        side = obj + ".srchash"
        objs.append(obj)
        key = _file_hash(src, HEADER, *CSRC_HEADERS)
        have = open(side).read().strip() if os.path.exists(side) and os.path.exists(obj) else None
        if force or have != key:
            if os.path.exists(side):
                os.remove(side)
            cmd = [hipcc] + flags + ["-c", src, "-o", obj]
            if verbose:
                print(" ".join(cmd))
            jobs.append((cmd, subprocess.Popen(cmd), side, key))
    for cmd, pr, side, key in jobs:
        if pr.wait() != 0:
            raise subprocess.CalledProcessError(pr.returncode, cmd)
        with open(side, "w") as f:
            f.write(key)
    stamp_obj = os.path.join(objdir, "stamp.cpp.o")
    cmd = [hipcc, "-O2", "-fPIC", "-DVD_SOURCES_HASH=\"%s%s\"" % (STAMP_PREFIX, want), "-c", STAMP_SOURCE, "-o", stamp_obj]
    subprocess.run(cmd, check=True)
    tmp = out + ".tmp.%d" % os.getpid()
    cmd = [hipcc, "--offload-arch=gfx950", "-shared", "-fPIC", "-o", tmp] + objs + [stamp_obj, "-ldl"]
    if verbose:
        print(" ".join(cmd))
    subprocess.run(cmd, check=True)
    os.replace(tmp, out)
    return out


STAMP_PREFIX = "VD_SOURCES_HASH="


def library_stamp(path: str = None) -> Optional[str]:
    path = path or LIB_PATH
    if not os.path.exists(path):
        return None
    import mmap
    with open(path, "rb") as f:
        with mmap.mmap(f.fileno(), 0, access=mmap.ACCESS_READ) as m:
            i = m.find(STAMP_PREFIX.encode())
            if i < 0:
                return None
            return m[i + len(STAMP_PREFIX):i + len(STAMP_PREFIX) + 16].decode("ascii", "replace")


def sources_hash() -> str:
    import hashlib
    h = hashlib.sha256()
    for path in sorted(SOURCES) + [HEADER] + CSRC_HEADERS:
        with open(path, "rb") as f:
            h.update(f.read())
    return h.hexdigest()[:16]


_lib: Optional[ctypes.CDLL] = None


def lib() -> ctypes.CDLL:
    global _lib
    if _lib is None:
        path = os.environ.get("VD_LIB_PATH", LIB_PATH)
        if os.environ.get("VD_LIB_VARIANT") == "dbg":
            path = build(debug_hooks=True)
        if not os.path.exists(path):
            raise RuntimeError(
                "libvd_hip.so not found at %s -- run `python -c 'import __graft_entry__ as g; g.build()'` "
                "(there is no CPU or eager fallback for the HIP path)" % path)
        if "VD_LIB_PATH" not in os.environ and os.environ.get("VD_LIB_VARIANT") != "dbg":
            want = sources_hash()
            if library_stamp(path) != want:
                try:
                    build()
                except (OSError, subprocess.CalledProcessError) as e:
                    raise RuntimeError("libvd_hip.so at %s was built from other sources (stamp %s, checkout %s) and could not be "
                                       "rebuilt: %s" % (path, library_stamp(path), want, e))
                if library_stamp(path) != want:
                    raise RuntimeError("libvd_hip.so at %s carries stamp %s, the checkout's kernel sources hash to %s"
                                       % (path, library_stamp(path), want))
        L = ctypes.CDLL(path)
        for name in EXPORTS:
            if not hasattr(L, name):
                if "VD_LIB_PATH" in os.environ:
                    continue
                raise RuntimeError("libvd_hip.so does not export %s" % name)
            getattr(L, name).restype = {"vd_program_info": ctypes.c_int64, "vd_program_free": None, "vd_blob_free": None, "vd_embed_free": None, "vd_train_free": None, "vd_comm_free": None, "vd_train_workspace_bytes": ctypes.c_int64, "vd_bias_grad_pooled_scratch_floats": ctypes.c_int64,
                                        "vd_embed_num_features": ctypes.c_int64, "vd_embed_workspace_bytes": ctypes.c_int64,
                                        "vd_embed_argmax_bytes": ctypes.c_int64, "vd_embed_backward_workspace_bytes": ctypes.c_int64,
                                        "vd_coreset_workspace_bytes": ctypes.c_int64}.get(name, ctypes.c_int)
        if L.vd_abi_version() != 5:
            raise RuntimeError("libvd_hip.so ABI version mismatch")
        if hasattr(L, "vd_sources_hash"):
            L.vd_sources_hash.restype = ctypes.c_char_p
        _lib = L
    return _lib


# ... 64 lines not shown
```

Baseline: 31.05.

## Fuse SGD update with pix2rows packing and add clip-order gather/scatter in conv

```diff
diff --git a/include/vd_hip.h b/include/vd_hip.h
--- a/include/vd_hip.h
+++ b/include/vd_hip.h
@@ -66,6 +66,8 @@
     int32_t src_planes, src_rows;
     int32_t pair_flip;
     uint32_t* range_stats;
+    const int64_t* clip_order;
+    const int64_t* out_clip_index;
 } VdConvParams;
 
 int vd_abi_version(void);
@@ -106,6 +108,8 @@
 
 int vd_sgd_momentum(float* x, float* buf, const float* g, int64_t n, float lr, float momentum, int first,
                     void* stream);
+int vd_sgd_momentum_pix2rows(float* x, float* buf, const float* g, int64_t nclips, int T, int H, int W, float lr, float momentum,
+                             int first, void* out_hi, void* out_lo, int prec, void* stream);
 
 int vd_hallucinator_fwd(const float* stat, const float* dyn, const int64_t* sidx, const int64_t* didx,
                         const float* w, const float* b, int n, int T, int H, int W, float* out, void* stream);
diff --git a/video_distillation_amd/csrc/aux_kernels.hip b/video_distillation_amd/csrc/aux_kernels.hip
--- a/video_distillation_amd/csrc/aux_kernels.hip
+++ b/video_distillation_amd/csrc/aux_kernels.hip
@@ -534,6 +534,116 @@
     if (blocks > 8192) blocks = 8192;
     hipLaunchKernelGGL(sgd_momentum_kernel, dim3((unsigned)blocks), dim3(bs), 0, reinterpret_cast<hipStream_t>(stream),
                        x, buf, g, n, lr, momentum, first);
+    return (int)hipGetLastError();
+}
+
+__global__ void sgd_momentum_pix2rows_kernel(float* __restrict__ x, float* __restrict__ buf, const float* __restrict__ g,
+                                             int64_t nchunks, int W, int cpr, float lr, float mu, int first,
+                                             uint4* __restrict__ hi, uint4* __restrict__ lo, int prec) {
+    const int64_t i = (int64_t)blockIdx.x * blockDim.x + threadIdx.x;
+    if (i >= nchunks) return;
+    const int j = (int)(i % cpr);
+    const int64_t base = (i / cpr) * W;
+    const int w0 = 8 * j - 3;
+    uint16_t h16[8], l16[8];
+#pragma unroll
+    for (int k = 0; k < 8; ++k) {
+#pragma clang fp contract(off)
+        const int ww = w0 + k;
+        float v = 0.f;
+        if (ww >= 0 && ww < W) {
+            const int64_t e = base + ww;
+            const float gv = g[e];
+            const float prev = buf[e] * mu;
+            const float b = first ? gv : prev + gv;
+            buf[e] = b;
+            const float step = lr * b;
+            v = x[e] - step;
+            x[e] = v;
+        }
+        split16p(prec, v, h16[k], l16[k]);
+    }
+    uint4 vh, vl;
+    vh.x = h16[0] | ((uint32_t)h16[1] << 16); vh.y = h16[2] | ((uint32_t)h16[3] << 16);
+    vh.z = h16[4] | ((uint32_t)h16[5] << 16); vh.w = h16[6] | ((uint32_t)h16[7] << 16);
+    hi[i] = vh;
+    if (lo != nullptr) {
+        vl.x = l16[0] | ((uint32_t)l16[1] << 16); vl.y = l16[2] | ((uint32_t)l16[3] << 16);
+        vl.z = l16[4] | ((uint32_t)l16[5] << 16); vl.w = l16[6] | ((uint32_t)l16[7] << 16);
+        lo[i] = vl;
+    }
+}
+
+__global__ void sgd_momentum_pix2rows_vec_kernel(float* __restrict__ x, float* __restrict__ buf, const float* __restrict__ g,
+                                                 int64_t nrows, int W, int cpr, int rpw, float lr, float mu, int first,
+                                                 uint4* __restrict__ hi, uint4* __restrict__ lo, int prec) {
+    const int lane = threadIdx.x & 63;
+    const int64_t wave = ((int64_t)blockIdx.x * blockDim.x + threadIdx.x) >> 6;
+    const int rr = lane / cpr, j = lane - rr * cpr;
+    const int64_t row = wave * rpw + rr;
+    const bool active = rr < rpw && row < nrows;
+    float nv[8];
+#pragma unroll
+    for (int q = 0; q < 2; ++q) {
+#pragma clang fp contract(off)
+        const int wq = 8 * j - 4 + 4 * q;
+        float4 xn = make_float4(0.f, 0.f, 0.f, 0.f);
+        if (active && wq >= 0 && wq < W) {
+            const int64_t e = row * W + wq;
+            const float4 gv = *reinterpret_cast<const float4*>(g + e);
+            const float4 xv = *reinterpret_cast<const float4*>(x + e);
+            float4 b = gv;
+            if (!first) {
+                const float4 bv = *reinterpret_cast<const float4*>(buf + e);
+                const float p0 = bv.x * mu, p1 = bv.y * mu, p2 = bv.z * mu, p3 = bv.w * mu;
+                b.x = p0 + gv.x; b.y = p1 + gv.y; b.z = p2 + gv.z; b.w = p3 + gv.w;
+            }
+            *reinterpret_cast<float4*>(buf + e) = b;
+            const float s0 = lr * b.x, s1 = lr * b.y, s2 = lr * b.z, s3 = lr * b.w;
+            xn.x = xv.x - s0; xn.y = xv.y - s1; xn.z = xv.z - s2; xn.w = xv.w - s3;
+            *reinterpret_cast<float4*>(x + e) = xn;
+        }
+        nv[4 * q] = xn.x; nv[4 * q + 1] = xn.y; nv[4 * q + 2] = xn.z; nv[4 * q + 3] = xn.w;
+    }
+    const float nxt = __shfl_down(nv[0], 1, 64);
+    if (!active) return;
+    uint16_t h16[8], l16[8];
+#pragma unroll
+    for (int k = 0; k < 7; ++k) split16p(prec, nv[k + 1], h16[k], l16[k]);
+    split16p(prec, (j + 1 < cpr) ? nxt : 0.f, h16[7], l16[7]);
+    const int64_t i = row * cpr + j;
+    uint4 vh, vl;
+    vh.x = h16[0] | ((uint32_t)h16[1] << 16); vh.y = h16[2] | ((uint32_t)h16[3] << 16);
+    vh.z = h16[4] | ((uint32_t)h16[5] << 16); vh.w = h16[6] | ((uint32_t)h16[7] << 16);
+    hi[i] = vh;
+    if (lo != nullptr) {
+        vl.x = l16[0] | ((uint32_t)l16[1] << 16); vl.y = l16[2] | ((uint32_t)l16[3] << 16);
+        vl.z = l16[4] | ((uint32_t)l16[5] << 16); vl.w = l16[6] | ((uint32_t)l16[7] << 16);
+        lo[i] = vl;
+    }
+}
+
+extern "C" int vd_sgd_momentum_pix2rows(float* x, float* buf, const float* g, int64_t nclips, int T, int H, int W, float lr,
+                                        float momentum, int first, void* out_hi, void* out_lo, int prec, void* stream) {
+    if (nclips < 0 || T < 0 || H < 0 || W < 0 || prec < VD_PREC_BF16 || prec > VD_PREC_F16X3) return -1;
+    const int cpr = ((W + 8) + 7) / 8;
+    const int64_t nchunks = nclips * T * 3 * H * cpr;
+    if (nchunks <= 0) return 0;
+    if (x == nullptr || buf == nullptr || g == nullptr || out_hi == nullptr) return -1;
+    const int bs = 256;
+    if ((nchunks + bs - 1) / bs > 0x7fffffff) return -2;
+    const auto al16 = [](const void* q) { return (reinterpret_cast<uintptr_t>(q) & 15) == 0; };
+    if ((W & 3) == 0 && cpr <= 64 && al16(x) && al16(buf) && al16(g)) {
+        const int rpw = 64 / cpr;
+        const int64_t nrows = nclips * T * 3 * H, nwaves = (nrows + rpw - 1) / rpw, blocks = (nwaves + 3) / 4;
+        if (blocks > 0x7fffffff) return -2;
+        hipLaunchKernelGGL(sgd_momentum_pix2rows_vec_kernel, dim3((unsigned)blocks), dim3(bs), 0, reinterpret_cast<hipStream_t>(stream),
+                           x, buf, g, nrows, W, cpr, rpw, lr, momentum, first, (uint4*)out_hi, (uint4*)out_lo, prec);
+        return (int)hipGetLastError();
+    }
+    hipLaunchKernelGGL(sgd_momentum_pix2rows_kernel, dim3((unsigned)((nchunks + bs - 1) / bs)), dim3(bs), 0,
+                       reinterpret_cast<hipStream_t>(stream), x, buf, g, nchunks, W, cpr, lr, momentum, first, (uint4*)out_hi,
+                       (uint4*)out_lo, prec);
     return (int)hipGetLastError();
 }
 
diff --git a/video_distillation_amd/csrc/conv_mfma.hip b/video_distillation_amd/csrc/conv_mfma.hip
--- a/video_distillation_amd/csrc/conv_mfma.hip
+++ b/video_distillation_amd/csrc/conv_mfma.hip
@@ -188,6 +188,7 @@
     int* lds_tap = reinterpret_cast<int*>(smem + LPL * plane_bytes);
     int* lds_otab = lds_tap + 2 * p.S;
     int* lds_skip = lds_otab + (p.MW * MTW + BAL) * 4;
+    int64_t* lds_orow = reinterpret_cast<int64_t*>(smem + LPL * plane_bytes + (((2 * p.S + (p.MW * MTW + BAL) * 4 + (p.S >> 2)) * 4 + 7) & ~7));
     const bool one_type = (p.ntypes == 1);
     const uint32_t* zslot = reinterpret_cast<const uint32_t*>(p.zero_slot);
     const uint32_t* src = reinterpret_cast<const uint32_t*>(p.src);
@@ -234,6 +235,18 @@
         }
     }
     const int clip0 = grp * p.ncl;
+    if constexpr (C8) {
+        if (p.epi == VD_EPI_POS_FEAT && p.out_clip_index != nullptr) {
+            __syncthreads();
+            if (tid < 16) {
+                const int32_t* brow = p.boxes + bi * 8;
+                const int o = (p.tables + (one_type ? p.tab_ofs[1] : brow[1]))[tid];
+                const int ci = o >= 0 ? o / (int)p.out_clip_stride : 0;
+                const bool ok = o >= 0 && clip0 + ci < p.nclips;
+                lds_orow[tid] = ok ? p.out_clip_index[clip0 + ci] * p.out_clip_stride + brow[3] + (o - ci * (int)p.out_clip_stride) : (int64_t)-1;
+            }
+        }
+    }
 
     const int32_t* gtab = p.gather + (int64_t)bi * p.gather_stride;
     constexpr bool HOIST = (TILES < 8);
@@ -267,7 +280,6 @@
     }
 #pragma unroll
     for (int u = 0; u < (HOIST ? LU : 1); ++u) asm volatile("" : "+v"(goff[u]));
-
     f32x16 acc[TILES];
 #pragma unroll
     for (int i = 0; i < TILES; ++i)
@@ -307,7 +319,14 @@
         for (int u = 0; u < DB; ++u) load_b(u, bqh[u], bql[u]);
         const uint32_t* csrc = src + (int64_t)clip0 * p.src_clip_stride4 + (int64_t)cc * p.src_chunk_stride4;
         if constexpr (TILES <= 4) {
-            if (p.clip_index != nullptr) csrc = src + p.clip_index[clip0] * (int64_t)p.src_clip_stride4;
+            if constexpr (!X3) {
+                if (p.clip_index != nullptr || p.clip_order != nullptr) {
+                    const int64_t co = p.clip_order != nullptr ? p.clip_order[clip0] : (int64_t)clip0;
+                    csrc = src + (p.clip_index != nullptr ? p.clip_index[co] : co) * (int64_t)p.src_clip_stride4;
+                }
+            } else {
+                if (p.clip_index != nullptr) csrc = src + p.clip_index[clip0] * (int64_t)p.src_clip_stride4;
+            }
         }
         if constexpr (SO) {
             if (p.src_split_cc > 0 && cc >= p.src_split_cc)
@@ -726,6 +745,12 @@
     const int64_t out_base = (int64_t)clip0 * p.out_clip_stride + out_rel;
     const float asc = (PREC == VD_PREC_F16X3 && p.w_box_stride == 0) ? 1.f / (float)(1 << VD_F16X3_WSHIFT) : 1.f;
 
+    auto clip_of = [&](int o) {
+        int ci = 0;
+#pragma unroll 1
+        for (int64_t t = p.out_clip_stride; t <= (int64_t)0x7fffffff && ci + 1 < p.ncl && o >= (int)t; t += p.out_clip_stride) ++ci;
+        return ci;
+    };
     if (p.epi == VD_EPI_ROWS) {
         float* dst = reinterpret_cast<float*>(p.dst);
         if constexpr (EXT) { if (p.atomic) dst += (int64_t)box[5] * p.replica_stride; }
@@ -775,6 +800,11 @@
                 if (p.relu) m = fmaxf(m, 0.f);
                 const int row = (k & 3) + 8 * (k >> 2) + 4 * half;
                 const int o = lds_otab[row >> 1];
+                if (p.out_clip_index != nullptr) {
+                    const int64_t ob = lds_orow[row >> 1];
+                    if (ob >= 0 && n_ok) dstf[ob + (int64_t)n * p.n_stride] = m;
+                    continue;
+                }
                 const int64_t idx = out_base + o + (int64_t)n * p.n_stride;
                 if (o >= 0 && n_ok && idx < out_total) dstf[idx] = m;
             }
@@ -899,6 +929,14 @@
                 const uint8_t ab = (uint8_t)(av[st] | (mx > 0.f ? 0 : 0x80));
                 if (feat) {
                     const uint32_t idx = (uint32_t)base + chan;
+                    if constexpr (X3 && !EXT && !SQ && MTW <= 4) {
+                        if (p.out_clip_index != nullptr) {
+                            const int ci = clip_of(base);
+                            reinterpret_cast<float*>(p.dst)[p.out_clip_index[clip0 + ci] * p.out_clip_stride + out_rel +
+                                                            (base - ci * (int)p.out_clip_stride) + chan] = mx;
+                            continue;
+                        }
+                    }
                     dstf[idx] = mx;
                     if (amx) amx[idx] = ab;
                 } else {
@@ -1057,11 +1095,13 @@
     typedef const int64_t __attribute__((address_space(4))) * clong_p;
     const cint_p c_boxes = (cint_p)(uintptr_t)p.boxes;
     const clong_p c_index = (clong_p)(uintptr_t)p.clip_index;
+    const clong_p c_order = (clong_p)(uintptr_t)p.clip_order;
     auto prep_rows = [&](int b) {
         const int clip0 = b / p.nbox, bi = b - clip0 * p.nbox;
         const cint_p box = c_boxes + bi * 8;
         const int b6 = box[6], b7 = box[7];
-        const int64_t ci = p.clip_index != nullptr ? c_index[clip0] : (int64_t)clip0;
+        const int64_t co = p.clip_order != nullptr ? c_order[clip0] : (int64_t)clip0;
+        const int64_t ci = p.clip_index != nullptr ? c_index[co] : co;
         rs_f0 = b6 >> 16; rs_h0 = (int)(int16_t)(b6 & 0xFFFF); rs_w0 = b7;
         rs_base = reinterpret_cast<const char*>(src + ci * p.src_clip_stride4 + ((int64_t)rs_f0 * p.src_rows + rs_h0) * row4 + rs_w0);
     };
@@ -1319,7 +1359,7 @@
     const VdConvParams& p = *pp;
     if (p.NT != 2 || p.MW != 2 || p.MTW != 4 || (p.NTW != 0 && p.NTW != 1) || p.S != 32 || p.CC != 1 || p.ncl != 1 ||
         p.ntypes != 1 || p.epi != VD_EPI_POOL_CL || p.pool_t != 1 || p.argmax != nullptr || !p.relu ||
-        8 * 1024 > p.lds_plane_bytes || p.src_planes <= 0 || p.src_rows <= 0 || p.type_desc == nullptr)
+        8 * 1024 > p.lds_plane_bytes || p.src_planes <= 0 || p.src_rows <= 0 || p.type_desc == nullptr || p.out_clip_index != nullptr)
         return -2;
     hipStream_t st = reinterpret_cast<hipStream_t>(stream);
     VdConvParams q = p;
@@ -1337,7 +1377,7 @@
     const int64_t total = (int64_t)groups * p.nbox;
     if (total <= 0) return 0;
     size_t lds = (size_t)((X3 && !SQ) ? 2 : 1) * p.lds_plane_bytes +
-                 (size_t)(2 * p.S + (p.MW * MTW + BAL) * 4 + (PREC == VD_PREC_F16C8 ? p.S / 4 : 0)) * sizeof(int) + 16;
+                 (size_t)(2 * p.S + (p.MW * MTW + BAL) * 4 + (PREC == VD_PREC_F16C8 ? p.S / 4 + 34 : 0)) * sizeof(int) + 16;
     if (lds > 160 * 1024) return -3;
     if ((p.dbg & 0x100) && lds < 100 * 1024) lds = 100 * 1024;
     auto kern = conv_mfma_kernel<PREC, MTW, SO, NTW, BAL, SQ>;
@@ -1376,7 +1416,12 @@
     if (wgw < 1 || wgw > 4 || p.lds_plane_bytes % 16 != 0) return -2;
     if (p.ncl * 65536 <= 0 || p.S <= 0 || p.CC <= 0) return -2;
     if (p.MTW * ntw < 8 && (p.gather_stride >> 6) > (int64_t)wgw * (p.MTW * ntw <= 4 ? 14 : 17)) return -2;
-    if (p.clip_index != nullptr && (p.ncl != 1 || p.CC != 1 || p.MTW * ntw > 4)) return -2;
+    if ((p.clip_index != nullptr || p.clip_order != nullptr) && (p.ncl != 1 || p.CC != 1 || p.MTW * ntw > 4)) return -2;
+    if (p.clip_order != nullptr && p.prec > VD_PREC_F16) return -2;
+    if (p.out_clip_index != nullptr && (p.prec < VD_PREC_BF16X3 || (p.epi != VD_EPI_POOL_FEAT && p.epi != VD_EPI_POS_FEAT) ||
+                                        p.argmax != nullptr || p.select || p.atomic || p.src_split_cc > 0 || p.MTW > 4 || p.CC == 1 ||
+                                        (p.w_box_stride != 0 && p.prec != VD_PREC_F16C8) || p.out_clip_stride <= 0 || p.out_clip_stride > 0x7fffffff))
+        return -2;
     if (p.prec == VD_PREC_F16C8) {
         if (ntw != 1 || p.MTW != 4 || p.S % 4 != 0 || (p.epi != VD_EPI_POOL_FEAT && p.epi != VD_EPI_POS_FEAT) || p.out_scale == nullptr ||
             p.select || p.atomic || p.src_split_cc > 0 || p.emit_lo != 0)
@@ -1499,7 +1544,7 @@
         const int wgw = p.NT * p.MW;
         if (wgw < 1 || wgw > 4 || p.lds_plane_bytes % 16 != 0 || p.ncl * 65536 <= 0 || p.S <= 0 || p.CC <= 0) return -2;
         if (p.MTW < 8 && (p.gather_stride >> 6) > (int64_t)wgw * (p.MTW <= 4 ? 14 : 17)) return -2;
-        if (p.clip_index != nullptr || p.emit_lo != 0 || p.w_box_stride != 0 || p.MTW == 5) return -2;
+        if (p.clip_index != nullptr || p.clip_order != nullptr || p.out_clip_index != nullptr || p.emit_lo != 0 || p.w_box_stride != 0 || p.MTW == 5) return -2;
         so = so || p.atomic || p.select || p.src_split_cc > 0;
     }
     if (so) {
diff --git a/video_distillation_amd/distill.py b/video_distillation_amd/distill.py
--- a/video_distillation_amd/distill.py
+++ b/video_distillation_amd/distill.py
@@ -281,6 +281,8 @@
                 if not hasattr(self, "_seg_perm"):
                     self._seg_perm = {}
                 self._seg_perm[key] = perm
+            if os.environ.get("VD_CLIP_ORDER", "1") == "1" and self.eng_real.supports_clip_order(rows is not None):
+                return self.eng_real.forward_sets(pool, index, rows=rows, order=perm)
             f = self.eng_real.forward_sets(pool, index[perm], rows=rows)
             out = torch.empty_like(f)
             out[perm] = f
@@ -309,8 +311,14 @@
                                          hip.stream_ptr(self.device)), "vd_group_sum")
         return out
 
+    def sgd_rows(self, x: torch.Tensor, buf: torch.Tensor, g: torch.Tensor, lr: float, mu: float, first: bool) -> None:
+        if os.environ.get("VD_SGD_ROWS", "1") == "1" and self.eng_syn.sgd_momentum_rows(x, buf, g.contiguous(), lr, mu, first):
+            return
+        self.sgd(x, buf, g, lr, mu, first)
+
     def sgd(self, x: torch.Tensor, buf: torch.Tensor, g: torch.Tensor, lr: float, mu: float, first: bool) -> None:
         hip = self.hip
+        self.eng_syn._rows_of = None
         hip.check(hip.lib().vd_sgd_momentum(hip.ptr(x), hip.ptr(buf), hip.ptr(g), ctypes.c_int64(x.numel()),
                                             ctypes.c_float(lr), ctypes.c_float(mu), int(first),
                                             hip.stream_ptr(self.device)), "vd_sgd_momentum")
@@ -536,7 +544,7 @@
         grad = be.embed_backward(handle, g_syn)
         if self.exchange == "allreduce":
             grad = self._allreduce_pixel_grad(grad)
-        be.sgd(self.image_syn, self.buf, grad, self.lr_img, self.momentum, first=(self.steps_done == 0))
+        getattr(be, "sgd_rows", be.sgd)(self.image_syn, self.buf, grad, self.lr_img, self.momentum, first=(self.steps_done == 0))
         self.steps_done += 1
         return loss_c.sum()
 
@@ -551,7 +559,7 @@
         grad = be.embed_backward(handle, g_syn)
         if self.exchange == "allreduce":
             grad = self._allreduce_pixel_grad(grad)
-        be.sgd(self.image_syn, self.buf, grad, self.lr_img, self.momentum, first=first)
+        getattr(be, "sgd_rows", be.sgd)(self.image_syn, self.buf, grad, self.lr_img, self.momentum, first=first)
 
     def _real_features(self, idx_t: torch.Tensor) -> torch.Tensor:
         be = self.be
diff --git a/video_distillation_amd/engine.py b/video_distillation_amd/engine.py
--- a/video_distillation_amd/engine.py
+++ b/video_distillation_amd/engine.py
@@ -111,8 +111,11 @@
     def run(self, src: torch.Tensor, src_plane_slots: int, bias: Optional[torch.Tensor], dst_ptr: int,
             dst_plane_stride: int, argmax: Optional[torch.Tensor], nclips: int, out_scale: Optional[torch.Tensor] = None,
             wpk: Optional[torch.Tensor] = None, w_plane_elems: int = 0, clip_index: Optional[torch.Tensor] = None,
-            group: Optional[int] = None, set_clips: int = 0, emit_lo: bool = False, launch: bool = True) -> None:
+            group: Optional[int] = None, set_clips: int = 0, emit_lo: bool = False, launch: bool = True,
+            clip_order: Optional[torch.Tensor] = None, out_clip_index: Optional[torch.Tensor] = None) -> None:
         p = self.params
+        p.clip_order = 0 if clip_order is None else clip_order.data_ptr()
+        p.out_clip_index = 0 if out_clip_index is None else out_clip_index.data_ptr()
         p.emit_lo = int(emit_lo)
         if int(emit_lo) == 2 and _RANGE_MONITOR:
             if self.range_stats is None:
@@ -330,6 +333,7 @@
         self._weights: Optional[List[torch.Tensor]] = None
         self._bwd_packed = False
         self._ws: Dict[str, torch.Tensor] = {}
+        self._rows_of: Optional[tuple] = None
         self.profile = None
 
     def _buf(self, name: str, shape, dtype) -> torch.Tensor:
@@ -403,6 +407,7 @@
         assert group is None or 0 <= group < getattr(self, "_dither", 0), "set_weights(dither=G) first"
         g = self.geo
         assert x.dim() == 5 and tuple(x.shape[1:]) == (g.frames, g.channel, g.height, g.width), x.shape
+        rows_current = index is None and rows is None and self._rows_are_current(x)
         x = x.detach().to(torch.float32).contiguous()
         B = x.shape[0] if index is None else int(index.numel())
         if index is not None:
@@ -425,9 +430,11 @@
                 slots0 = self._buf("slots0", (self.planes, n_slots0, 8), torch.int16)
                 lo = slots0[1] if self.planes == 2 else None
                 xin = x[c0:] if index is None else x
-                hip.check(L.vd_pix2rows(hip.ptr(xin), hip.ptr(None if index is None else index[c0:]),
-                                         ctypes.c_int64(nb), g.frames, g.height, g.width,
-                                         hip.ptr(slots0[0]), hip.ptr(lo), self.prec, st), "vd_pix2rows")
+                if not rows_current:
+                    self._rows_of = None
+                    hip.check(L.vd_pix2rows(hip.ptr(xin), hip.ptr(None if index is None else index[c0:]),
+                                             ctypes.c_int64(nb), g.frames, g.height, g.width,
+                                             hip.ptr(slots0[0]), hip.ptr(lo), self.prec, st), "vd_pix2rows")
             n1, n2 = nb * per1, nb * per2
             hilo = self.fwd2x is not None
             assert not (hilo and keep), "last_hilo engines have no kept-arg-max forward"
@@ -459,9 +466,36 @@
             return feats, saved
         return feats
 
-    def forward_sets(self, x: torch.Tensor, index: torch.Tensor, rows: Optional[torch.Tensor] = None) -> torch.Tensor:
+    def _rows_are_current(self, x: torch.Tensor) -> bool:
+        tok = self._rows_of
+        return bool(tok is not None and tok[0]() is x and tok[1:] == (x.data_ptr(), tuple(x.shape), x._version)
+                    and x.shape[0] <= self.chunk)
+
+    def sgd_momentum_rows(self, x: torch.Tensor, buf: torch.Tensor, grad: torch.Tensor, lr: float, mu: float, first: bool) -> bool:
+        g = self.geo
+        if not (x.dim() == 5 and tuple(x.shape[1:]) == (g.frames, g.channel, g.height, g.width) and 0 < x.shape[0] <= self.chunk
+                and x.dtype == torch.float32 and x.is_contiguous() and x.device == self.device):
+            return False
+        assert buf.shape == x.shape and grad.shape == x.shape and buf.is_contiguous() and grad.is_contiguous()
+        assert buf.dtype == torch.float32 and grad.dtype == torch.float32
+        nb = int(x.shape[0])
+        n_slots0 = nb * g.frames * 3 * g.height * (P.pix_row_pitch(g.width) // 8)
+        slots0 = self._buf("slots0", (self.planes, n_slots0, 8), torch.int16)
+        lo = slots0[1] if self.planes == 2 else None
+        self._rows_of = None
+        hip.check(hip.lib().vd_sgd_momentum_pix2rows(hip.ptr(x), hip.ptr(buf), hip.ptr(grad), ctypes.c_int64(nb), g.frames, g.height,
+                                                     g.width, ctypes.c_float(lr), ctypes.c_float(mu), int(first), hip.ptr(slots0[0]),
+                                                     hip.ptr(lo), self.prec, hip.stream_ptr(self.device)), "vd_sgd_momentum_pix2rows")
+        import weakref
+        self._rows_of = (weakref.ref(x), x.data_ptr(), tuple(x.shape), x._version)
+        return True
+
+    def forward_sets(self, x: torch.Tensor, index: torch.Tensor, rows: Optional[torch.Tensor] = None,
+                     order: Optional[torch.Tensor] = None) -> torch.Tensor:
         G = getattr(self, "_dither", 0)
         B = int(index.numel())
+        if order is not None and not self.supports_clip_order(rows is not None):
+            raise ValueError("forward_sets(order=) needs resident rows, the register-resident-B first level and a hi+lo last level")
         assert G >= 2 and B % G == 0 and self.planes == 1, "set_weights(dither=G) on a single-pass engine first"
         g = self.geo
         per = B // G
@@ -478,12 +512,14 @@
         if rows is None:
             n_slots0 = B * g.frames * 3 * g.height * (rowp // 8)
             slots0 = self._buf("slots0", (1, n_slots0, 8), torch.int16)
+            self._rows_of = None
             hip.check(hip.lib().vd_pix2rows(hip.ptr(x.detach().to(torch.float32).contiguous()), hip.ptr(index), ctypes.c_int64(B),
                                             g.frames, g.height, g.width, hip.ptr(slots0[0]), hip.ptr(None), self.prec,
                                             hip.stream_ptr(self.device)), "vd_pix2rows")
         if self.fwd[0].breg_ok:
             if rows is not None:
-                self.fwd[0].run(rows, int(rows.shape[1]), w[1], act1.data_ptr(), n1, None, B, clip_index=index, set_clips=per)
+                self.fwd[0].run(rows, int(rows.shape[1]), w[1], act1.data_ptr(), n1, None, B, clip_index=index, set_clips=per,
+                                clip_order=order)
             else:
                 self.fwd[0].run(slots0, n_slots0, w[1], act1.data_ptr(), n1, None, B, set_clips=per)
         else:
@@ -501,7 +537,8 @@
             if li == 2 and hilo:
                 if os.environ.get("VD_L2_X2_SIM") == "act":
                     src[1].zero_()
-                self.fwd2x.run(src, n_src, w[5], dst_ptr, 0, None, B, out_scale=self.c8_scales if self.last_c8 else None)
+                self.fwd2x.run(src, n_src, w[5], dst_ptr, 0, None, B, out_scale=self.c8_scales if self.last_c8 else None,
+                               out_clip_index=order)
             elif per % self.fwd[li].plan.ncl == 0:
                 self.fwd[li].run(src, n_src, w[2 * li + 1], dst_ptr, n_dst, None, B, set_clips=per,
                                  emit_lo=(2 if self.last_c8 else 1) if (li == 1 and hilo) else 0)
@@ -510,6 +547,10 @@
                     self.fwd[li].run(src[:, s * per * per_src:], n_src, w[2 * li + 1], dst_ptr + s * per * per_dst_bytes, n_dst, None,
                                      per, group=s, emit_lo=(2 if self.last_c8 else 1) if (li == 1 and hilo) else 0)
         return feats
+
+    def supports_clip_order(self, resident_rows: bool) -> bool:
+        return bool(resident_rows and self.fwd[0].breg_ok and self.fwd2x is not None
+                    and self.fwd2x.plan.MTW <= 4 and self.fwd2x.plan.CC > 1)
 
     def backward(self, saved, g_feat: torch.Tensor) -> torch.Tensor:
         self._pack_bwd()
diff --git a/video_distillation_amd/hip.py b/video_distillation_amd/hip.py
--- a/video_distillation_amd/hip.py
+++ b/video_distillation_amd/hip.py
@@ -28,7 +28,7 @@
            "vd_bias_grad_pooled_scratch_floats", "vd_bias_grad_pooled_ordered", "vd_standardize_ordered", "vd_head_train_bwd_ordered",
            "vd_set_deterministic", "vd_get_deterministic", "vd_pack_weights_c8", "vd_pack_weights_multi",
            "vd_split_scaled", "vd_scale_combine", "vd_sources_hash", "vd_coreset_workspace_bytes", "vd_coreset_select",
-           "vd_clips_sample")
+           "vd_clips_sample", "vd_sgd_momentum_pix2rows")
 F16X3_WSHIFT = 8
 
 
@@ -50,6 +50,7 @@
         ("out_chunk_stride", ctypes.c_int32), ("out_t_stride", ctypes.c_int32),
         ("lds_plane_bytes", ctypes.c_int32), ("prec", ctypes.c_int32), ("dbg", ctypes.c_int32), ("ntypes", ctypes.c_int32), ("tab_ofs", ctypes.c_int32 * 3), ("atomic", ctypes.c_int32), ("select", ctypes.c_int32), ("src_split_cc", ctypes.c_int32), ("src_split_off4", ctypes.c_int64), ("NTW", ctypes.c_int32), ("clip_index", ctypes.c_void_p), ("mt_valid", ctypes.c_int32), ("persist", ctypes.c_int32), ("stamps", ctypes.c_void_p),
         ("w_set_clips", ctypes.c_int32), ("replica_stride", ctypes.c_int32), ("emit_lo", ctypes.c_int32), ("src_planes", ctypes.c_int32), ("src_rows", ctypes.c_int32), ("pair_flip", ctypes.c_int32), ("range_stats", ctypes.c_void_p),
+        ("clip_order", ctypes.c_void_p), ("out_clip_index", ctypes.c_void_p),
     ]
 
 
```

Measured after the change: 30.96. No clear change (-0.3%).
